# fgvieira/ngsLD

Measured on AMD Instinct MI355X. Metric: SNP-pair EM-LD computations/sec @ n_ind=500, higher is better.
Workload: dtype f64

## Files before the change

include/ngsld.h:

```cpp
#ifndef NGSLD_H
#define NGSLD_H

#include <stddef.h>
#include <stdint.h>

#ifdef __cplusplus
extern "C" {
#endif

typedef struct ngsld_ctx ngsld_ctx;

enum {
  NGSLD_OK = 0,
  NGSLD_ERR_INVALID = -1,
  NGSLD_ERR_DEVICE = -2,
  NGSLD_ERR_NOMEM = -3,
  NGSLD_ERR_NAN = -4,
  NGSLD_ERR_MAF_RANGE = -5,
  NGSLD_ERR_SINK = -6,
  NGSLD_ERR_UNSUPPORTED = -7
};

typedef struct {
  uint64_t max_kb_dist;
  uint64_t max_snp_dist;
  double min_maf;
  int32_t ignore_miss_data;
  int32_t extend_out;
  double rnd_sample;
  uint64_t seed;
  uint64_t first_row;
} ngsld_params;

typedef struct {
  double r2_ExpG;
  double D;
  double Dp;
  double r2;
} ngsld_rec_std;

typedef struct {
  double hap[4];
  uint32_t n_ind_data;
  uint32_t n_iter;
} ngsld_rec_ext;

typedef struct {
  uint32_t s1, s2_begin, count, reserved;
  uint64_t mask;
  uint64_t first_record;
} ngsld_item;

typedef struct {
  uint64_t s1_begin, s1_end;
  uint64_t n_pairs;
  uint64_t n_items;
  const ngsld_item *items;
  const ngsld_rec_std *std;
  const ngsld_rec_ext *ext;
  const char *text;
  uint64_t text_len;
} ngsld_batch;

typedef int (*ngsld_sink_fn)(void *user, const ngsld_batch *batch);

typedef int (*ngsld_read_sites_fn)(void *user, uint64_t site_begin, uint64_t n_sites, double *dst);

const char *ngsld_version(void);

int ngsld_create(int device, ngsld_ctx **ctx);
void ngsld_destroy(ngsld_ctx *ctx);
const char *ngsld_last_error(const ngsld_ctx *ctx);

int ngsld_set_geno_raw(ngsld_ctx *ctx, const double *gl_raw, uint64_t n_sites, uint64_t n_ind, int log_scale,
                       int ignore_miss_data, int on_device);
typedef struct {
  int32_t log_scale;
  int32_t ignore_miss_data;
  int32_t on_device;
  int32_t text_semantics;
  int32_t call_geno;
  int32_t per_individual_only;
  double N_thresh;
  double call_thresh;
} ngsld_geno_opts;
int ngsld_set_geno_raw_opts(ngsld_ctx *ctx, const double *gl_raw, uint64_t n_sites, uint64_t n_ind,
                            const ngsld_geno_opts *opts);
int ngsld_set_geno_lkl(ngsld_ctx *ctx, const double *geno_lkl, const double *maf, uint64_t n_sites, uint64_t n_ind,
                       int on_device);
int ngsld_get_maf(ngsld_ctx *ctx, double *maf_out);
int ngsld_set_pos_dist(ngsld_ctx *ctx, const double *pos_dist);

int ngsld_plan(ngsld_ctx *ctx, const ngsld_params *params, uint64_t *n_pairs);
int ngsld_plan_rows(ngsld_ctx *ctx, const uint64_t **row_off, const uint32_t **row_end);

int ngsld_run(ngsld_ctx *ctx, uint64_t s1_begin, uint64_t s1_end, ngsld_sink_fn sink, void *user);

int ngsld_set_text_output(ngsld_ctx *ctx, const char *const *labels, int enable);

int ngsld_reserve_text_buffers(ngsld_ctx *ctx, uint64_t bytes_per_row);

int ngsld_set_replay_source(ngsld_ctx *ctx, ngsld_read_sites_fn read, void *user);
int ngsld_set_replay_matrix(ngsld_ctx *ctx, const double *values);
int ngsld_set_replay(ngsld_ctx *ctx, int enable);
int ngsld_replay_stats(ngsld_ctx *ctx, uint64_t *pairs, uint64_t *sites);

int ngsld_set_exact_store(ngsld_ctx *ctx, int mode);
typedef struct {
  uint64_t pairs_flagged;
  uint64_t pairs_replayed;
  uint64_t pairs_on_device;
  uint64_t pairs_on_host;
  uint64_t sites_reevaluated;
  int32_t exact_store;
  int32_t text_rows_patched;
  double exact_store_build_s;
  uint64_t sites_degenerate;
} ngsld_replay_stats_t;
int ngsld_replay_info(ngsld_ctx *ctx, ngsld_replay_stats_t *out);

int ngsld_run_device(ngsld_ctx *ctx, uint64_t s1_begin, uint64_t s1_end, void *d_std, void *d_ext, void *hip_stream);
int ngsld_finish_device(ngsld_ctx *ctx);

int ngsld_last_kernel_time(ngsld_ctx *ctx, double *total_ms, uint64_t *n_launches, uint64_t *n_pairs);

const char *ngsld_pair_kernel(const ngsld_ctx *ctx);
int ngsld_describe_dispatch(uint64_t n_ind, int ignore_miss_data, char *buf, size_t buf_len);

int ngsld_set_tuning(ngsld_ctx *ctx, uint32_t pairs_per_item, uint64_t batch_pairs);

int ngsld_selftest(ngsld_ctx *ctx);

int ngsld_selftest_format(ngsld_ctx *ctx, uint64_t n, const ngsld_rec_std *std, const ngsld_rec_ext *ext, const double *dist,
                          const double *maf1, const double *maf2, char *text, uint64_t text_cap, uint64_t *row_len,
                          int32_t *needs_host);
int ngsld_selftest_printed(ngsld_ctx *ctx, uint64_t n, const double *x, int32_t precision, int32_t weight_type,
                           double min_weight, int64_t *micro, int32_t *micro_ok, int64_t *label, int32_t *label_rc);

typedef struct {
  uint64_t row_begin, row_end;
  uint64_t site_end;
} ngsld_slab;

int ngsld_window_ends(const double *pos_dist, uint64_t n_sites, const ngsld_params *params, uint32_t *row_end);

int ngsld_plan_slabs(const double *pos_dist, uint64_t n_sites, const ngsld_params *params, uint64_t max_slab_sites,
                     ngsld_slab *slabs, uint64_t cap, uint64_t *n_slabs);

uint64_t ngsld_slab_sites_for_budget(uint64_t n_ind, uint64_t budget_bytes);
uint64_t ngsld_sites_for_budget(uint64_t n_ind, uint64_t budget_bytes, int matrix_copies);

int ngsld_streamed_replay_info(ngsld_replay_stats_t *out);

int ngsld_set_memory_budget(int device, uint64_t bytes);

int ngsld_device_memory(int device, uint64_t *free_bytes, uint64_t *total_bytes);


int ngsld_run_streamed(int device, uint64_t n_sites, uint64_t n_ind, const double *pos_dist,
                       const ngsld_params *params, const ngsld_geno_opts *opts, uint64_t max_slab_sites,
                       ngsld_read_sites_fn read, void *read_user, double *maf_out, ngsld_sink_fn sink,
                       void *sink_user, uint64_t *n_pairs, uint64_t *n_slabs, char *err, size_t errlen);

int ngsld_run_streamed_text(int device, uint64_t n_sites, uint64_t n_ind, const double *pos_dist,
                            const ngsld_params *params, const ngsld_geno_opts *opts, uint64_t max_slab_sites,
                            ngsld_read_sites_fn read, void *read_user, double *maf_out, ngsld_sink_fn sink,
                            void *sink_user, uint64_t *n_pairs, uint64_t *n_slabs, char *err, size_t errlen,
                            const char *const *labels, int text_output);


int ngsld_plan_parts(const double *pos_dist, uint64_t n_sites, const ngsld_params *params, int n_parts, ngsld_slab *parts);

typedef int (*ngsld_multi_sink_fn)(void *user, int part, const ngsld_batch *batch);

int ngsld_run_multi(const int *devices, int n_devices, uint64_t n_sites, uint64_t n_ind, const double *pos_dist,
                    const ngsld_params *params, const ngsld_geno_opts *opts, const double *gl_raw,
                    ngsld_read_sites_fn read, void *read_user, double *maf_out, ngsld_multi_sink_fn sink, void *sink_user,
                    const char *const *labels, int text_output, uint64_t *pairs_per_part, char *err, size_t errlen);

enum { NGSLD_DIST_NONE = 0, NGSLD_DIST_UPLOAD = 1, NGSLD_DIST_PEER_COPY = 2, NGSLD_DIST_RCCL = 3 };
int ngsld_multi_last_distribution(void);

int ngsld_rccl_selftest(int device, uint64_t bytes, char *err, size_t errlen);

typedef struct {
  uint32_t struct_size;
  int32_t field;
  double max_kb_dist;
  double min_weight;
  int32_t weight_type;
  int32_t keep_heavy;
  int32_t precision;
  int32_t reserved;
  const char *const *subset;
  uint64_t n_subset;
} ngsld_prune_params;

typedef struct {
  uint32_t struct_size;
  uint32_t reserved;
  uint64_t pairs;
  uint64_t nodes, edges;
  uint64_t kept, excluded;
  uint64_t rounds;
  uint64_t host_nodes, host_edges, host_steps;
  double pairs_ms, edges_ms, graph_ms, rounds_ms, host_ms, total_ms;
} ngsld_prune_stats;

int ngsld_prune(ngsld_ctx *ctx, const ngsld_prune_params *params, const char *const *labels, uint8_t *site_state,
                ngsld_prune_stats *stats);

typedef struct {
  uint32_t struct_size;
  uint32_t fields;
  double bin_size;
  double max_kb_dist;
  double min_maf;
} ngsld_decay_params;

typedef struct {
  uint32_t struct_size;
  uint32_t lds;
  uint64_t pairs;
  uint64_t pairs_counted;
  uint64_t bins;
  uint64_t bin_slots;
  uint64_t chunks;
  double pairs_ms, bin_ms, total_ms;
} ngsld_decay_stats;

int ngsld_decay(ngsld_ctx *ctx, const ngsld_decay_params *params, ngsld_decay_stats *stats);
int ngsld_decay_bins(ngsld_ctx *ctx, uint64_t cap, double *dist, uint64_t *count, double *mean, uint64_t *n_bins);

typedef struct {
  uint32_t struct_size;
  uint32_t fields;
  const char *chr;
  uint64_t start, end;
} ngsld_blocks_params;

typedef struct {
  uint32_t struct_size;
  uint32_t reserved;
  uint64_t members, sites;
  uint64_t pairs, pairs_in_region;
  uint64_t cells_na, host_rows, chunks;
  double pairs_ms, scatter_ms, format_ms, total_ms;
} ngsld_blocks_stats;

int ngsld_blocks(ngsld_ctx *ctx, const ngsld_blocks_params *params, const char *const *labels, ngsld_blocks_stats *stats);
int ngsld_blocks_sites(ngsld_ctx *ctx, uint64_t cap, uint64_t *site, uint64_t *n_sites);
int ngsld_blocks_matrix(ngsld_ctx *ctx, int field, double *values, uint8_t *present);
typedef int (*ngsld_text_fn)(void *user, const char *text, uint64_t len);
int ngsld_blocks_text(ngsld_ctx *ctx, int field, ngsld_text_fn sink, void *user, ngsld_blocks_stats *stats);

typedef struct {
  uint32_t struct_size;
  uint32_t fields;
  double max_kb_dist;
  double min_maf;
  double linked_min;
  int32_t abs_value;
  int32_t reserved;
} ngsld_site_ld_params;

typedef struct {
  uint32_t struct_size;
  uint32_t lds;
  uint64_t pairs;
  uint64_t pairs_counted;
  uint64_t sites_with_pairs;
  uint64_t chunks;
  double pairs_ms, site_ms, total_ms;
} ngsld_site_ld_stats;

int ngsld_site_ld(ngsld_ctx *ctx, const ngsld_site_ld_params *params, ngsld_site_ld_stats *stats);
int ngsld_site_ld_get(ngsld_ctx *ctx, int field, uint64_t *n, int64_t *sum_micro, int64_t *max_micro, uint64_t *linked,
                      double *mean);

// ... 127 lines not shown
```

ngsld_amd/capi.py:

```python
from __future__ import annotations

import ctypes as C
import os
import subprocess

import numpy as np

PKG_DIR = os.path.dirname(os.path.abspath(__file__))
REPO_DIR = os.path.dirname(PKG_DIR)
LIB_PATH = os.environ.get("NGSLD_LIB") or os.path.join(PKG_DIR, "libngsld.so")
CLI_PATH = os.path.join(PKG_DIR, "bin", "ngsLD")

OK, ERR_INVALID, ERR_DEVICE, ERR_NOMEM, ERR_NAN, ERR_MAF_RANGE, ERR_SINK, ERR_UNSUPPORTED = 0, -1, -2, -3, -4, -5, -6, -7


class Params(C.Structure):
    _fields_ = [("max_kb_dist", C.c_uint64), ("max_snp_dist", C.c_uint64), ("min_maf", C.c_double),
                ("ignore_miss_data", C.c_int32), ("extend_out", C.c_int32), ("rnd_sample", C.c_double),
                ("seed", C.c_uint64), ("first_row", C.c_uint64)]


class GenoOpts(C.Structure):
    _fields_ = [("log_scale", C.c_int32), ("ignore_miss_data", C.c_int32), ("on_device", C.c_int32),
                ("text_semantics", C.c_int32), ("call_geno", C.c_int32), ("per_individual_only", C.c_int32),
                ("N_thresh", C.c_double), ("call_thresh", C.c_double)]


REC_STD = np.dtype([("r2_ExpG", "<f8"), ("D", "<f8"), ("Dp", "<f8"), ("r2", "<f8")])
REC_EXT = np.dtype([("hap", "<f8", (4,)), ("n_ind_data", "<u4"), ("n_iter", "<u4")])


ITEM = np.dtype([("s1", "<u4"), ("s2_begin", "<u4"), ("count", "<u4"), ("reserved", "<u4"), ("mask", "<u8"),
                 ("first_record", "<u8")])


class Batch(C.Structure):
    _fields_ = [("s1_begin", C.c_uint64), ("s1_end", C.c_uint64), ("n_pairs", C.c_uint64), ("n_items", C.c_uint64),
                ("items", C.c_void_p), ("std", C.c_void_p), ("ext", C.c_void_p), ("text", C.c_void_p),
                ("text_len", C.c_uint64)]


def items_to_pairs(items: np.ndarray) -> tuple[np.ndarray, np.ndarray]:
    if len(items) == 0:
        return np.zeros(0, dtype=np.uint64), np.zeros(0, dtype=np.uint64)
    bits = (items["mask"][:, None] >> np.arange(64, dtype=np.uint64)[None, :]) & np.uint64(1)
    bits &= (np.arange(64)[None, :] < items["count"][:, None]).astype(np.uint64)
    idx, c = np.nonzero(bits)
    return items["s1"][idx].astype(np.uint64), (items["s2_begin"][idx].astype(np.uint64) + c.astype(np.uint64))


def items_from_pairs(s1: np.ndarray, s2: np.ndarray, span: int = 64) -> np.ndarray:
    s1, s2 = np.asarray(s1, dtype=np.int64), np.asarray(s2, dtype=np.int64)
    chunk = (s2 - s1 - 1) // span
    key = s1 * (1 << 32) + chunk
    uniq, first, inv = np.unique(key, return_index=True, return_inverse=True)
    items = np.zeros(len(uniq), dtype=ITEM)
    items["s1"] = s1[first]
    items["s2_begin"] = s1[first] + 1 + chunk[first] * span
    items["first_record"] = first
    np.bitwise_or.at(items["mask"], inv, np.uint64(1) << (s2 - items["s2_begin"][inv]).astype(np.uint64))
    last = np.zeros(len(uniq), dtype=np.int64)
    np.maximum.at(last, inv, s2 - items["s2_begin"][inv].astype(np.int64))
    items["count"] = last + 1
    return items


SINK_FN = C.CFUNCTYPE(C.c_int, C.c_void_p, C.POINTER(Batch))
MULTI_SINK_FN = C.CFUNCTYPE(C.c_int, C.c_void_p, C.c_int, C.POINTER(Batch))
READ_FN = C.CFUNCTYPE(C.c_int, C.c_void_p, C.c_uint64, C.c_uint64, C.c_void_p)
SLAB = np.dtype([("row_begin", "<u8"), ("row_end", "<u8"), ("site_end", "<u8")])

SYMBOLS = [
    "ngsld_version", "ngsld_create", "ngsld_destroy", "ngsld_last_error", "ngsld_set_geno_raw",
    "ngsld_set_geno_raw_opts", "ngsld_set_geno_lkl",
    "ngsld_get_maf", "ngsld_set_pos_dist", "ngsld_plan", "ngsld_plan_rows", "ngsld_run", "ngsld_run_device", "ngsld_set_text_output",
    "ngsld_set_replay_source", "ngsld_set_replay_matrix", "ngsld_set_replay", "ngsld_replay_stats", "ngsld_finish_device",
    "ngsld_set_exact_store", "ngsld_replay_info",
    "ngsld_plan_parts", "ngsld_run_multi", "ngsld_multi_last_distribution", "ngsld_rccl_selftest",
    "ngsld_last_kernel_time", "ngsld_pair_kernel", "ngsld_describe_dispatch", "ngsld_set_tuning", "ngsld_selftest", "ngsld_selftest_format",
    "ngsld_selftest_printed", "ngsld_reserve_text_buffers",
    "ngsld_window_ends", "ngsld_plan_slabs", "ngsld_slab_sites_for_budget", "ngsld_sites_for_budget", "ngsld_streamed_replay_info", "ngsld_set_memory_budget", "ngsld_device_memory", "ngsld_run_streamed", "ngsld_run_streamed_text",
    "ngsld_host_read_geno_bin_range",
    "ngsld_host_set_threads", "ngsld_host_read_pos", "ngsld_host_pos_dist", "ngsld_host_label", "ngsld_host_free_pos", "ngsld_host_pos_slice",
    "ngsld_host_geno_size_ok", "ngsld_host_read_geno_bin", "ngsld_host_read_geno_text", "ngsld_host_format_header", "ngsld_host_format_pair",
    "ngsld_host_format_double", "ngsld_host_write_batch", "ngsld_host_replay_pair", "ngsld_host_missing_call_log",
    "ngsld_host_gz_open", "ngsld_host_gz_close",
    "ngsld_prune", "ngsld_host_prune_graph", "ngsld_host_prune_label",
    "ngsld_decay", "ngsld_decay_bins", "ngsld_host_decay_fit",
    "ngsld_blocks", "ngsld_blocks_sites", "ngsld_blocks_matrix", "ngsld_blocks_text",
    "ngsld_site_ld", "ngsld_site_ld_get",
    "ngsld_clusters", "ngsld_clusters_sites", "ngsld_clusters_table",
    "ngsld_grid", "ngsld_grid_cells", "ngsld_grid_chromosomes", "ngsld_grid_get",
    "ngsld_linked_pairs",
    "ngsld_scan", "ngsld_scan_get",
]


class ReplayStats(C.Structure):
    _fields_ = [("pairs_flagged", C.c_uint64), ("pairs_replayed", C.c_uint64), ("pairs_on_device", C.c_uint64),
                ("pairs_on_host", C.c_uint64), ("sites_reevaluated", C.c_uint64), ("exact_store", C.c_int32),
                ("text_rows_patched", C.c_int32), ("exact_store_build_s", C.c_double), ("sites_degenerate", C.c_uint64)]


class PruneParams(C.Structure):
    _fields_ = [("struct_size", C.c_uint32), ("field", C.c_int32), ("max_kb_dist", C.c_double), ("min_weight", C.c_double),
                ("weight_type", C.c_int32), ("keep_heavy", C.c_int32), ("precision", C.c_int32), ("reserved", C.c_int32),
                ("subset", C.POINTER(C.c_char_p)), ("n_subset", C.c_uint64)]


class PruneStats(C.Structure):
    _fields_ = [("struct_size", C.c_uint32), ("reserved", C.c_uint32), ("pairs", C.c_uint64), ("nodes", C.c_uint64),
                ("edges", C.c_uint64), ("kept", C.c_uint64), ("excluded", C.c_uint64), ("rounds", C.c_uint64),
                ("host_nodes", C.c_uint64), ("host_edges", C.c_uint64), ("host_steps", C.c_uint64),
                ("pairs_ms", C.c_double), ("edges_ms", C.c_double), ("graph_ms", C.c_double), ("rounds_ms", C.c_double),
                ("host_ms", C.c_double), ("total_ms", C.c_double)]


class DecayParams(C.Structure):
    _fields_ = [("struct_size", C.c_uint32), ("fields", C.c_uint32), ("bin_size", C.c_double), ("max_kb_dist", C.c_double),
                ("min_maf", C.c_double)]


class DecayStats(C.Structure):
    _fields_ = [("struct_size", C.c_uint32), ("lds", C.c_uint32), ("pairs", C.c_uint64), ("pairs_counted", C.c_uint64),
                ("bins", C.c_uint64), ("bin_slots", C.c_uint64), ("chunks", C.c_uint64), ("pairs_ms", C.c_double),
                ("bin_ms", C.c_double), ("total_ms", C.c_double)]


class BlocksParams(C.Structure):
    _fields_ = [("struct_size", C.c_uint32), ("fields", C.c_uint32), ("chr", C.c_char_p), ("start", C.c_uint64),
                ("end", C.c_uint64)]


class BlocksStats(C.Structure):
    _fields_ = [("struct_size", C.c_uint32), ("reserved", C.c_uint32), ("members", C.c_uint64), ("sites", C.c_uint64),
                ("pairs", C.c_uint64), ("pairs_in_region", C.c_uint64), ("cells_na", C.c_uint64), ("host_rows", C.c_uint64),
                ("chunks", C.c_uint64), ("pairs_ms", C.c_double), ("scatter_ms", C.c_double), ("format_ms", C.c_double),
                ("total_ms", C.c_double)]


class SiteLdParams(C.Structure):
    _fields_ = [("struct_size", C.c_uint32), ("fields", C.c_uint32), ("max_kb_dist", C.c_double), ("min_maf", C.c_double),
                ("linked_min", C.c_double), ("abs_value", C.c_int32), ("reserved", C.c_int32)]


class SiteLdStats(C.Structure):
    _fields_ = [("struct_size", C.c_uint32), ("lds", C.c_uint32), ("pairs", C.c_uint64), ("pairs_counted", C.c_uint64),
                ("sites_with_pairs", C.c_uint64), ("chunks", C.c_uint64), ("pairs_ms", C.c_double), ("site_ms", C.c_double),
                ("total_ms", C.c_double)]


class ClustersParams(C.Structure):
    _fields_ = [("struct_size", C.c_uint32), ("field", C.c_int32), ("max_kb_dist", C.c_double), ("min_maf", C.c_double),
                ("min_weight", C.c_double), ("abs_value", C.c_int32), ("reserved", C.c_int32)]


class ClustersStats(C.Structure):
    _fields_ = [("struct_size", C.c_uint32), ("reserved", C.c_uint32), ("pairs", C.c_uint64), ("nodes", C.c_uint64),
                ("edges", C.c_uint64), ("clusters", C.c_uint64), ("clusters_multi", C.c_uint64), ("largest", C.c_uint64),
                ("chunks", C.c_uint64), ("union_launches", C.c_uint64), ("pairs_ms", C.c_double), ("union_ms", C.c_double),
                ("finish_ms", C.c_double), ("total_ms", C.c_double)]


class GridParams(C.Structure):
    _fields_ = [("struct_size", C.c_uint32), ("fields", C.c_uint32), ("bin_size", C.c_uint64), ("max_kb_dist", C.c_double),
                ("min_maf", C.c_double), ("linked_min", C.c_double), ("abs_value", C.c_int32), ("reserved", C.c_int32)]


class GridStats(C.Structure):
    _fields_ = [("struct_size", C.c_uint32), ("lds", C.c_uint32), ("pairs", C.c_uint64), ("pairs_counted", C.c_uint64),
                ("cells", C.c_uint64), ("bins", C.c_uint64), ("band", C.c_uint64), ("chunks", C.c_uint64),
                ("pairs_ms", C.c_double), ("grid_ms", C.c_double), ("total_ms", C.c_double)]


class LinkedParams(C.Structure):
    _fields_ = [("struct_size", C.c_uint32), ("field", C.c_int32), ("min_weight", C.c_double), ("max_kb_dist", C.c_double),
                ("min_maf", C.c_double), ("abs_value", C.c_int32), ("want", C.c_int32)]


class ScanParams(C.Structure):
    _fields_ = [("struct_size", C.c_uint32), ("fields", C.c_uint32), ("half_window", C.c_uint64), ("max_kb_dist", C.c_double),
                ("min_maf", C.c_double), ("reserved", C.c_uint64)]


class ScanStats(C.Structure):
    _fields_ = [("struct_size", C.c_uint32), ("reserved", C.c_uint32), ("pairs", C.c_uint64), ("pairs_counted", C.c_uint64),
                ("largest_window", C.c_uint64), ("chunks", C.c_uint64), ("pairs_ms", C.c_double), ("scan_ms", C.c_double),
                ("total_ms", C.c_double)]


class LinkedBatch(C.Structure):
    _fields_ = [("n", C.c_uint64), ("s1", C.c_void_p), ("s2", C.c_void_p), ("std", C.c_void_p), ("ext", C.c_void_p),
                ("text", C.c_void_p), ("text_len", C.c_uint64)]


class LinkedStats(C.Structure):
    _fields_ = [("struct_size", C.c_uint32), ("reserved", C.c_uint32), ("pairs", C.c_uint64), ("rows", C.c_uint64),
                ("text_bytes", C.c_uint64), ("host_rows", C.c_uint64), ("chunks", C.c_uint64), ("pairs_ms", C.c_double),
                ("kernel_ms", C.c_double), ("total_ms", C.c_double), ("count_ms", C.c_double), ("scan_ms", C.c_double),
                ("write_ms", C.c_double)]


LINKED_RECORDS, LINKED_TEXT = 1, 2
LINKED_FN = C.CFUNCTYPE(C.c_int, C.c_void_p, C.POINTER(LinkedBatch))
TEXT_FN = C.CFUNCTYPE(C.c_int, C.c_void_p, C.c_void_p, C.c_uint64)


class DecayFitResult(C.Structure):
    _fields_ = [("rate", C.c_double), ("ld_max", C.c_double), ("ld_min", C.c_double), ("sse", C.c_double),
                ("n_bins", C.c_uint64)]


DECAY_FIELDS = ("r2_ExpG", "D", "Dp", "r2")


class NgsldError(RuntimeError):
    def __init__(self, code: int, msg: str):
        super().__init__(f"ngsld error {code}: {msg}")
        self.code = code
        self.msg = msg


def build(force: bool = False, jobs: int = 8) -> None:
    csrc = os.path.join(PKG_DIR, "csrc")
    if force:
        subprocess.check_call(["make", "-s", "-C", csrc, "clean"])
    subprocess.check_call(["make", "-s", f"-j{jobs}", "-C", csrc, "all"])


_lib = None


def lib() -> C.CDLL:
    global _lib
    if _lib is None:
        if not os.path.exists(LIB_PATH):
            raise FileNotFoundError(f"{LIB_PATH} is missing: run ngsld_amd.capi.build() (or make -C ngsld_amd/csrc); "
                                    "there is no fallback implementation")
        L = C.CDLL(LIB_PATH)
        vp, u64, dbl = C.c_void_p, C.c_uint64, C.c_double
        L.ngsld_version.restype = C.c_char_p
        L.ngsld_create.argtypes = [C.c_int, C.POINTER(vp)]
        L.ngsld_destroy.argtypes = [vp]
        L.ngsld_destroy.restype = None
        L.ngsld_last_error.argtypes = [vp]
        L.ngsld_last_error.restype = C.c_char_p
        L.ngsld_set_geno_raw.argtypes = [vp, vp, u64, u64, C.c_int, C.c_int, C.c_int]
        L.ngsld_set_geno_raw_opts.argtypes = [vp, vp, u64, u64, C.POINTER(GenoOpts)]
        L.ngsld_set_geno_lkl.argtypes = [vp, vp, vp, u64, u64, C.c_int]
        L.ngsld_get_maf.argtypes = [vp, vp]
        L.ngsld_set_pos_dist.argtypes = [vp, vp]
        L.ngsld_plan.argtypes = [vp, C.POINTER(Params), C.POINTER(u64)]
        L.ngsld_plan_rows.argtypes = [vp, C.POINTER(C.POINTER(C.c_uint64)), C.POINTER(C.POINTER(C.c_uint32))]
        L.ngsld_run.argtypes = [vp, u64, u64, SINK_FN, vp]
        L.ngsld_run_device.argtypes = [vp, u64, u64, vp, vp, vp]
        if hasattr(L, "ngsld_set_replay_source"):
            L.ngsld_set_replay_source.argtypes = [vp, READ_FN, vp]
            if hasattr(L, "ngsld_set_replay_matrix"):
                L.ngsld_set_replay_matrix.argtypes = [vp, vp]
            L.ngsld_set_replay.argtypes = [vp, C.c_int]
            L.ngsld_replay_stats.argtypes = [vp, C.POINTER(u64), C.POINTER(u64)]
        if hasattr(L, "ngsld_replay_info"):
            L.ngsld_set_exact_store.argtypes = [vp, C.c_int]
            L.ngsld_replay_info.argtypes = [vp, C.POINTER(ReplayStats)]
            L.ngsld_finish_device.argtypes = [vp]
        if hasattr(L, "ngsld_set_text_output"):
            L.ngsld_set_text_output.argtypes = [vp, C.POINTER(C.c_char_p), C.c_int]
        L.ngsld_last_kernel_time.argtypes = [vp, C.POINTER(dbl), C.POINTER(u64), C.POINTER(u64)]
        L.ngsld_set_tuning.argtypes = [vp, C.c_uint32, u64]
        if hasattr(L, "ngsld_pair_kernel"):
            L.ngsld_pair_kernel.argtypes = [vp]
            L.ngsld_pair_kernel.restype = C.c_char_p
        L.ngsld_selftest.argtypes = [vp]
        if hasattr(L, "ngsld_selftest_format"):
            L.ngsld_selftest_format.argtypes = [vp, u64, vp, vp, vp, vp, vp, C.c_char_p, u64, vp, C.POINTER(C.c_int32)]
            L.ngsld_selftest_printed.argtypes = [vp, u64, vp, C.c_int32, C.c_int32, dbl, vp, vp, vp, vp]
        L.ngsld_window_ends.argtypes = [vp, u64, C.POINTER(Params), vp]
        L.ngsld_plan_slabs.argtypes = [vp, u64, C.POINTER(Params), u64, vp, u64, C.POINTER(u64)]
        L.ngsld_slab_sites_for_budget.argtypes = [u64, u64]
        L.ngsld_slab_sites_for_budget.restype = u64
        if hasattr(L, "ngsld_sites_for_budget"):
            L.ngsld_sites_for_budget.argtypes = [u64, u64, C.c_int]
            L.ngsld_sites_for_budget.restype = u64
        L.ngsld_device_memory.argtypes = [C.c_int, C.POINTER(u64), C.POINTER(u64)]
        L.ngsld_run_streamed.argtypes = [C.c_int, u64, u64, vp, C.POINTER(Params), C.POINTER(GenoOpts), u64, READ_FN, vp,
                                         vp, SINK_FN, vp, C.POINTER(u64), C.POINTER(u64), C.c_char_p, C.c_size_t]
        if hasattr(L, "ngsld_run_multi"):
            L.ngsld_plan_parts.argtypes = [vp, u64, C.POINTER(Params), C.c_int, vp]
            L.ngsld_run_multi.argtypes = [C.POINTER(C.c_int), C.c_int, u64, u64, vp, C.POINTER(Params), C.POINTER(GenoOpts),
                                          vp, READ_FN, vp, vp, MULTI_SINK_FN, vp, C.POINTER(C.c_char_p), C.c_int,
                                          C.POINTER(u64), C.c_char_p, C.c_size_t]
        if hasattr(L, "ngsld_multi_last_distribution"):
            L.ngsld_multi_last_distribution.argtypes = []
        if hasattr(L, "ngsld_rccl_selftest"):
            L.ngsld_rccl_selftest.argtypes = [C.c_int, u64, C.c_char_p, C.c_size_t]
        L.ngsld_host_read_geno_bin_range.argtypes = [C.c_char_p, u64, u64, u64, vp, C.c_char_p, C.c_size_t]
        L.ngsld_host_set_threads.argtypes = [C.c_int]
        L.ngsld_host_set_threads.restype = None
        L.ngsld_host_read_pos.argtypes = [C.c_char_p, C.c_int, u64, C.POINTER(vp), C.c_char_p, C.c_size_t]
        L.ngsld_host_pos_dist.argtypes = [vp]
        L.ngsld_host_pos_dist.restype = C.POINTER(dbl)
        L.ngsld_host_label.argtypes = [vp, u64]
        L.ngsld_host_label.restype = C.c_char_p
        L.ngsld_host_free_pos.argtypes = [vp]
        L.ngsld_host_free_pos.restype = None
        L.ngsld_host_pos_slice.argtypes = [vp, u64, u64]
        L.ngsld_host_pos_slice.restype = vp
        L.ngsld_host_geno_size_ok.argtypes = [u64, u64, u64]
        L.ngsld_host_read_geno_bin.argtypes = [C.c_char_p, u64, u64, vp, C.c_char_p, C.c_size_t]
        L.ngsld_host_read_geno_text.argtypes = [C.c_char_p, C.c_int, C.c_int, u64, u64, vp, C.POINTER(C.c_int),
                                                C.c_char_p, C.c_size_t]
        L.ngsld_host_format_header.argtypes = [C.c_char_p, C.c_size_t, C.c_int]
        L.ngsld_host_format_header.restype = C.c_size_t
        L.ngsld_host_format_pair.argtypes = [C.c_char_p, C.c_size_t, C.c_char_p, C.c_char_p, dbl, vp, vp, dbl, dbl]
        L.ngsld_host_format_pair.restype = C.c_size_t
        L.ngsld_host_format_double.argtypes = [C.c_char_p, C.c_size_t, dbl, C.c_int]
        L.ngsld_host_format_double.restype = C.c_size_t
        L.ngsld_host_write_batch.argtypes = [C.POINTER(Batch), vp, vp, vp, C.c_int, C.c_int]
        L.ngsld_host_replay_pair.argtypes = [vp, vp, u64, C.POINTER(GenoOpts), vp, vp, vp]
        if hasattr(L, "ngsld_host_gz_open"):
            L.ngsld_host_gz_open.argtypes = [C.c_char_p, C.c_int, C.POINTER(vp), C.POINTER(C.c_int)]
            L.ngsld_host_gz_close.argtypes = [vp]
        if hasattr(L, "ngsld_prune"):
            L.ngsld_prune.argtypes = [vp, C.POINTER(PruneParams), C.POINTER(C.c_char_p), vp, C.POINTER(PruneStats)]
            L.ngsld_host_prune_graph.argtypes = [u64, vp, u64, vp, vp, vp, C.c_int, vp, C.POINTER(u64)]
            L.ngsld_host_prune_label.argtypes = [dbl, C.c_int, C.c_char, C.POINTER(C.c_int64)]
        if hasattr(L, "ngsld_decay"):
            L.ngsld_decay.argtypes = [vp, C.POINTER(DecayParams), C.POINTER(DecayStats)]
            L.ngsld_decay_bins.argtypes = [vp, u64, vp, vp, vp, C.POINTER(u64)]
            L.ngsld_host_decay_fit.argtypes = [u64, vp, vp, C.c_int, dbl, dbl, C.POINTER(DecayFitResult)]
        if hasattr(L, "ngsld_blocks"):
            L.ngsld_blocks.argtypes = [vp, C.POINTER(BlocksParams), C.POINTER(C.c_char_p), C.POINTER(BlocksStats)]
            L.ngsld_blocks_sites.argtypes = [vp, u64, vp, C.POINTER(u64)]
            L.ngsld_blocks_matrix.argtypes = [vp, C.c_int, vp, vp]
            L.ngsld_blocks_text.argtypes = [vp, C.c_int, TEXT_FN, vp, C.POINTER(BlocksStats)]
        if hasattr(L, "ngsld_site_ld"):
            L.ngsld_site_ld.argtypes = [vp, C.POINTER(SiteLdParams), C.POINTER(SiteLdStats)]
            L.ngsld_site_ld_get.argtypes = [vp, C.c_int, vp, vp, vp, vp, vp]
        if hasattr(L, "ngsld_clusters"):
            L.ngsld_clusters.argtypes = [vp, C.POINTER(ClustersParams), C.POINTER(ClustersStats)]
            L.ngsld_clusters_sites.argtypes = [vp, vp]
            L.ngsld_clusters_table.argtypes = [vp, u64, u64, vp, vp, vp, vp, vp, vp, vp, vp, vp, C.POINTER(u64)]
        if hasattr(L, "ngsld_grid"):
            L.ngsld_grid.argtypes = [vp, C.POINTER(GridParams), C.POINTER(C.c_char_p), C.POINTER(GridStats)]
            L.ngsld_grid_cells.argtypes = [vp, u64, vp, vp, vp, vp, C.POINTER(u64)]
            L.ngsld_grid_chromosomes.argtypes = [vp, u64, C.POINTER(C.c_char_p), C.POINTER(u64)]
            L.ngsld_grid_get.argtypes = [vp, C.c_int, u64, vp, vp, vp, vp]
        if hasattr(L, "ngsld_linked_pairs"):
            L.ngsld_linked_pairs.argtypes = [vp, C.POINTER(LinkedParams), C.POINTER(C.c_char_p), LINKED_FN, vp, C.POINTER(LinkedStats)]
        if hasattr(L, "ngsld_scan"):
            L.ngsld_scan.argtypes = [vp, C.POINTER(ScanParams), C.POINTER(ScanStats)]
            L.ngsld_scan_get.argtypes = [vp, C.c_int, vp, vp, vp, vp, vp, vp, vp, vp, vp, vp]
        _lib = L
    return _lib


def prune_label(x: float, prec: int = 4, weight_type: str = "a") -> int | None:
    out = C.c_int64()
    rc = lib().ngsld_host_prune_label(float(x), prec, weight_type.encode(), C.byref(out))
    if rc == ERR_INVALID:
        return None
    if rc != OK:
        raise NgsldError(rc, "label out of range")
    return out.value


def decay_fit(dist, values, field: str = "r2", n_ind: float = 0, recomb_rate: float = 1.0) -> dict:
    d = np.ascontiguousarray(dist, dtype=np.float64)
    v = np.ascontiguousarray(values, dtype=np.float64)
    if d.shape != v.shape or d.ndim != 1:
        raise ValueError("dist and values must be 1-D arrays of one length")
    if field not in DECAY_FIELDS:
        raise ValueError(f"field must be one of {DECAY_FIELDS}")
    out = DecayFitResult()
    rc = lib().ngsld_host_decay_fit(len(d), d.ctypes.data, v.ctypes.data, 4 + DECAY_FIELDS.index(field), float(n_ind),
                                    float(recomb_rate), C.byref(out))
    if rc != OK:
        raise NgsldError(rc, f"ngsld_host_decay_fit refused the {field} fit")
    return {k: getattr(out, k) for k, _ in DecayFitResult._fields_}


def prune_graph(n_nodes: int, a, b, label, keep_heavy: bool = False, rank=None) -> tuple[np.ndarray, int]:
    a = np.ascontiguousarray(a, dtype=np.uint32)
    b = np.ascontiguousarray(b, dtype=np.uint32)
    lab = np.ascontiguousarray(label, dtype=np.int64)
    rk = None if rank is None else np.ascontiguousarray(rank, dtype=np.uint64)
    excl = np.zeros(max(n_nodes, 1), dtype=np.uint8)
    steps = C.c_uint64()
    rc = lib().ngsld_host_prune_graph(n_nodes, None if rk is None else rk.ctypes.data, len(a), a.ctypes.data, b.ctypes.data,
                                      lab.ctypes.data, int(keep_heavy), excl.ctypes.data, C.byref(steps))
    if rc != OK:
        raise NgsldError(rc, "ngsld_host_prune_graph failed")
    return excl[:n_nodes].astype(bool), steps.value


def read_pos(path: str, header: bool, n_sites: int) -> tuple[np.ndarray, list[str]]:
    L = lib()
    h = C.c_void_p()
    err = C.create_string_buffer(512)
    rc = L.ngsld_host_read_pos(path.encode(), int(header), n_sites, C.byref(h), err, len(err))
    if rc != OK:
        raise NgsldError(rc, err.value.decode())
    try:
        pd = np.ctypeslib.as_array(L.ngsld_host_pos_dist(h), shape=(n_sites,)).copy()
        labels = [L.ngsld_host_label(h, s).decode() for s in range(n_sites)]
    finally:
        L.ngsld_host_free_pos(h)
    return pd, labels


def read_geno_bin(path: str, n_ind: int, n_sites: int) -> np.ndarray:
    L = lib()
    out = np.empty((n_sites, n_ind, 3), dtype=np.float64)
    err = C.create_string_buffer(512)
    rc = L.ngsld_host_read_geno_bin(path.encode(), n_ind, n_sites, out.ctypes.data, err, len(err))
    if rc != OK:
        raise NgsldError(rc, err.value.decode())
    return out


def read_geno_bin_range(path: str, n_ind: int, site_begin: int, n_sites: int) -> np.ndarray:
    L = lib()
    out = np.empty((n_sites, n_ind, 3), dtype=np.float64)
    err = C.create_string_buffer(512)
    rc = L.ngsld_host_read_geno_bin_range(path.encode(), n_ind, site_begin, n_sites, out.ctypes.data, err, len(err))
# ... 431 lines not shown
        a, b = C.c_uint64(), C.c_uint64()
        self._check(self._L.ngsld_replay_stats(self._h, C.byref(a), C.byref(b)))
        return a.value, b.value

    def set_exact_store(self, mode: int) -> None:
        self._check(self._L.ngsld_set_exact_store(self._h, int(mode)))

    def replay_info(self) -> dict:
        st = ReplayStats()
        self._check(self._L.ngsld_replay_info(self._h, C.byref(st)))
        return {k: getattr(st, k) for k, _ in ReplayStats._fields_}

    def finish_device(self) -> None:
        self._check(self._L.ngsld_finish_device(self._h))

    def maf(self) -> np.ndarray:
        out = np.empty(self.n_sites, dtype=np.float64)
        self._check(self._L.ngsld_get_maf(self._h, out.ctypes.data))
        return out

    def set_pos_dist(self, pos_dist: np.ndarray | None) -> None:
        if pos_dist is None:
            self._check(self._L.ngsld_set_pos_dist(self._h, None))
        else:
            pd = np.ascontiguousarray(pos_dist, dtype=np.float64)
            assert pd.shape[0] == self.n_sites
            self._check(self._L.ngsld_set_pos_dist(self._h, pd.ctypes.data))

    def set_tuning(self, pairs_per_item: int = 0, batch_pairs: int = 0) -> None:
        self._check(self._L.ngsld_set_tuning(self._h, pairs_per_item, batch_pairs))

    def plan(self, max_kb_dist: int = 0, max_snp_dist: int = 0, min_maf: float = 0.0, ignore_miss_data: bool = False,
             extend_out: bool = True, rnd_sample: float = 1.0, seed: int = 0, first_row: int = 0) -> int:
        p = Params(max_kb_dist, max_snp_dist, min_maf, int(ignore_miss_data), int(extend_out), rnd_sample, seed,
                   first_row)
        n = C.c_uint64()
        self._check(self._L.ngsld_plan(self._h, C.byref(p), C.byref(n)))
        self.extend_out = extend_out
        return n.value

    def plan_rows(self) -> tuple[np.ndarray, np.ndarray]:
        ro, re = C.POINTER(C.c_uint64)(), C.POINTER(C.c_uint32)()
        self._check(self._L.ngsld_plan_rows(self._h, C.byref(ro), C.byref(re)))
        return (np.ctypeslib.as_array(ro, shape=(self.n_sites + 1,)).copy(),
                np.ctypeslib.as_array(re, shape=(self.n_sites,)).copy())

    def run(self, s1_begin: int = 0, s1_end: int | None = None):
        s1_end = self.n_sites if s1_end is None else s1_end
        s1s, s2s, stds, exts = [], [], [], []

        def sink(_user, bp):
            b = bp.contents
            n = b.n_pairs
            if n:
                stds.append(np.frombuffer(C.string_at(b.std, n * REC_STD.itemsize), dtype=REC_STD).copy())
                if b.ext:
                    exts.append(np.frombuffer(C.string_at(b.ext, n * REC_EXT.itemsize), dtype=REC_EXT).copy())
            items = np.frombuffer(C.string_at(b.items, b.n_items * ITEM.itemsize), dtype=ITEM) if b.n_items else \
                np.zeros(0, dtype=ITEM)
            a, bb = items_to_pairs(items)
            assert len(a) == n
            if len(items):
                assert np.array_equal(items["first_record"], np.concatenate([[0], np.cumsum(
                    [bin(int(m)).count("1") for m in items["mask"]])[:-1]]).astype(np.uint64))
            s1s.append(a)
            s2s.append(bb)
            return 0

        cb = SINK_FN(sink)
        self._check(self._L.ngsld_run(self._h, s1_begin, s1_end, cb, None))
        cat = lambda xs, dt: np.concatenate(xs) if xs else np.zeros(0, dtype=dt)
        return (cat(s1s, np.uint64), cat(s2s, np.uint64), cat(stds, REC_STD),
                cat(exts, REC_EXT) if self.extend_out else None)

    def items(self, s1_begin: int = 0, s1_end: int | None = None) -> np.ndarray:
        s1_end = self.n_sites if s1_end is None else s1_end
        got = []

        def sink(_user, bp):
            b = bp.contents
            if b.n_items:
                got.append(np.frombuffer(C.string_at(b.items, b.n_items * ITEM.itemsize), dtype=ITEM).copy())
            return 0

        self.set_text_output(None, False)
        self._check(self._L.ngsld_run(self._h, s1_begin, s1_end, SINK_FN(sink), None))
        return np.concatenate(got) if got else np.zeros(0, dtype=ITEM)

    def run_to_fd(self, s1_begin: int, s1_end: int, fd: int, pos_handle, pos_dist: np.ndarray | None, maf: np.ndarray,
                  n_threads: int) -> int:
        maf = np.ascontiguousarray(maf, dtype=np.float64)
        pd_ptr = None if pos_dist is None else np.ascontiguousarray(pos_dist, dtype=np.float64).ctypes.data
        total, rc_box = [0], [0]

        libc = C.CDLL(None, use_errno=True)
        libc.write.argtypes = [C.c_int, C.c_void_p, C.c_size_t]
        libc.write.restype = C.c_ssize_t

        def sink(_user, bp):
            b = bp.contents
            total[0] += b.n_pairs
            if b.text:
                off = 0
                while off < b.text_len:
                    w = libc.write(fd, b.text + off, min(b.text_len - off, 1 << 30))
                    if w <= 0:
                        return 1
                    off += w
                return 0
            rc_box[0] = self._L.ngsld_host_write_batch(bp, pos_handle, pd_ptr, maf.ctypes.data, n_threads, fd)
            return 0 if rc_box[0] == OK else 1

        self._check(self._L.ngsld_run(self._h, s1_begin, s1_end, SINK_FN(sink), None))
        return total[0]

    def set_text_output(self, labels: list[str] | None, enable: bool = True) -> None:
        arr = None
        if labels is not None:
            arr = (C.c_char_p * len(labels))(*[l.encode() for l in labels])
        self._check(self._L.ngsld_set_text_output(self._h, arr, int(enable)))

    def run_text(self, s1_begin: int = 0, s1_end: int | None = None) -> tuple[bytes, int]:
        s1_end = self.n_sites if s1_end is None else s1_end
        parts, fallbacks = [], [0]

        def sink(_user, bp):
            b = bp.contents
            if b.text:
                parts.append(C.string_at(b.text, b.text_len))
            else:
                fallbacks[0] += 1
            return 0

        self._check(self._L.ngsld_run(self._h, s1_begin, s1_end, SINK_FN(sink), None))
        return b"".join(parts), fallbacks[0]

    def run_discard(self, s1_begin: int = 0, s1_end: int | None = None) -> int:
        s1_end = self.n_sites if s1_end is None else s1_end
        total = [0]

        def sink(_user, bp):
            total[0] += bp.contents.n_pairs
            return 0

        self._check(self._L.ngsld_run(self._h, s1_begin, s1_end, SINK_FN(sink), None))
        return total[0]

    def run_device(self, s1_begin: int, s1_end: int, d_std: int, d_ext: int | None, stream: int | None = None) -> None:
        self._check(self._L.ngsld_run_device(self._h, s1_begin, s1_end, d_std, d_ext, stream))

    def pair_kernel(self) -> str:
        return self._L.ngsld_pair_kernel(self._h).decode()

    def last_kernel_time(self) -> tuple[float, int, int]:
        ms, nl, npairs = C.c_double(), C.c_uint64(), C.c_uint64()
        self._check(self._L.ngsld_last_kernel_time(self._h, C.byref(ms), C.byref(nl), C.byref(npairs)))
        return ms.value, nl.value, npairs.value

    def prune(self, labels: list[str] | None, field: int = 7, max_kb_dist: float = float("inf"), min_weight: float = 0.0,
              weight_type: str = "a", keep_heavy: bool = False, subset: list[str] | None = None,
              precision: int = 4) -> tuple[np.ndarray, dict]:
        arr = None if labels is None else (C.c_char_p * len(labels))(*[l.encode() for l in labels])
        sub = None if subset is None else (C.c_char_p * max(len(subset), 1))(*[l.encode() for l in subset])
        p = PruneParams(C.sizeof(PruneParams), field, float(max_kb_dist), float(min_weight), ord(weight_type), int(keep_heavy),
                        precision, 0, sub, 0 if subset is None else len(subset))
        st = PruneStats()
        st.struct_size = C.sizeof(PruneStats)
        state = np.zeros(max(self.n_sites, 1), dtype=np.uint8)
        self._check(self._L.ngsld_prune(self._h, C.byref(p), arr, state.ctypes.data, C.byref(st)))
        return state[:self.n_sites], {k: getattr(st, k) for k, _ in PruneStats._fields_ if k not in ("struct_size", "reserved")}

    def decay(self, ld=("r2",), bin_size: float = 250, max_kb_dist: float = float("inf"),
              min_maf: float = 0.0) -> tuple[dict, dict]:
        ld = (ld,) if isinstance(ld, str) else tuple(ld)
        bad = [f for f in ld if f not in DECAY_FIELDS]
        if bad or not ld:
            raise ValueError(f"ld must name some of {DECAY_FIELDS}: {bad}")
        mask = sum(1 << DECAY_FIELDS.index(f) for f in set(ld))
        names = [f for k, f in enumerate(DECAY_FIELDS) if (mask >> k) & 1]
        p = DecayParams(C.sizeof(DecayParams), mask, float(bin_size), float(max_kb_dist), float(min_maf))
        st = DecayStats()
        st.struct_size = C.sizeof(DecayStats)
        self._check(self._L.ngsld_decay(self._h, C.byref(p), C.byref(st)))
        nb = st.bins
        dist = np.zeros(max(nb, 1))
        cnt = np.zeros(max(nb, 1), dtype=np.uint64)
        mean = np.zeros((max(nb, 1), len(names)))
        got = C.c_uint64()
        self._check(self._L.ngsld_decay_bins(self._h, nb, dist.ctypes.data, cnt.ctypes.data, mean.ctypes.data, C.byref(got)))
        assert got.value == nb
        bins = {"dist": dist[:nb], "n": cnt[:nb]}
        for k, f in enumerate(names):
            bins[f] = mean[:nb, k].copy()
        return bins, {k: getattr(st, k) for k, _ in DecayStats._fields_ if k != "struct_size"}

    def site_ld(self, ld=("r2",), max_kb_dist: float = float("inf"), min_maf: float = 0.0, linked_min: float = 0.5,
                abs_value: bool = True) -> tuple[dict, dict]:
        ld = (ld,) if isinstance(ld, str) else tuple(ld)
        bad = [f for f in ld if f not in DECAY_FIELDS]
        if bad or not ld:
            raise ValueError(f"ld must name some of {DECAY_FIELDS}: {bad}")
        mask = sum(1 << DECAY_FIELDS.index(f) for f in set(ld))
        p = SiteLdParams(C.sizeof(SiteLdParams), mask, float(max_kb_dist), float(min_maf), float(linked_min), int(bool(abs_value)), 0)
        st = SiteLdStats()
        st.struct_size = C.sizeof(SiteLdStats)
        self._check(self._L.ngsld_site_ld(self._h, C.byref(p), C.byref(st)))
        m = max(self.n_sites, 1)
        sites = {"n": np.zeros(m, dtype=np.uint64)}
        for k, f in enumerate(DECAY_FIELDS):
            if not (mask >> k) & 1:
                continue
            sites[f"sum_{f}"], sites[f"max_{f}"] = np.zeros(m, dtype=np.int64), np.zeros(m, dtype=np.int64)
            sites[f"linked_{f}"], sites[f"mean_{f}"] = np.zeros(m, dtype=np.uint64), np.zeros(m)
            self._check(self._L.ngsld_site_ld_get(self._h, 4 + k, sites["n"].ctypes.data, sites[f"sum_{f}"].ctypes.data,
                                                  sites[f"max_{f}"].ctypes.data, sites[f"linked_{f}"].ctypes.data,
                                                  sites[f"mean_{f}"].ctypes.data))
        sites = {k: v[:self.n_sites] for k, v in sites.items()}
        return sites, {k: getattr(st, k) for k, _ in SiteLdStats._fields_ if k != "struct_size"}

    def scan(self, half_window: int, ld=("r2",), max_kb_dist: float = float("inf"), min_maf: float = 0.0) -> tuple[dict, dict]:
        ld = (ld,) if isinstance(ld, str) else tuple(ld)
        bad = [f for f in ld if f not in DECAY_FIELDS]
        if bad or not ld:
            raise ValueError(f"ld must name some of {DECAY_FIELDS}: {bad}")
        if not 0 <= int(half_window) < 2 ** 64:
            raise ValueError("half_window must be a non-negative integer")
        mask = sum(1 << DECAY_FIELDS.index(f) for f in set(ld))
        p = ScanParams(C.sizeof(ScanParams), mask, int(half_window), float(max_kb_dist), float(min_maf), 0)
        st = ScanStats()
        st.struct_size = C.sizeof(ScanStats)
        self._check(self._L.ngsld_scan(self._h, C.byref(p), C.byref(st)))
        m = max(self.n_sites, 1)
        win = {"win_first": np.zeros(m, dtype=np.uint32), "win_last": np.zeros(m, dtype=np.uint32)}
        for cl in ("ll", "rr", "lr"):
            win[f"n_{cl}"] = np.zeros(m, dtype=np.uint64)
        for k, f in enumerate(DECAY_FIELDS):
            if not (mask >> k) & 1:
                continue
            for cl in ("ll", "rr", "lr"):
                win[f"sum_{cl}_{f}"] = np.zeros(m, dtype=np.int64)
            win[f"zns_{f}"], win[f"omega_{f}"] = np.zeros(m), np.zeros(m)
            self._check(self._L.ngsld_scan_get(self._h, 4 + k, win["win_first"].ctypes.data, win["win_last"].ctypes.data,
                                               win["n_ll"].ctypes.data, win["n_rr"].ctypes.data, win["n_lr"].ctypes.data,
                                               win[f"sum_ll_{f}"].ctypes.data, win[f"sum_rr_{f}"].ctypes.data,
                                               win[f"sum_lr_{f}"].ctypes.data, win[f"zns_{f}"].ctypes.data,
                                               win[f"omega_{f}"].ctypes.data))
        win = {k: v[:self.n_sites] for k, v in win.items()}
        return win, {k: getattr(st, k) for k, _ in ScanStats._fields_ if k not in ("struct_size", "reserved")}

    def clusters(self, field: int = 7, min_weight: float = 0.5, max_kb_dist: float = float("inf"), min_maf: float = 0.0,
                 abs_value: bool = True, min_size: int = 2) -> tuple[np.ndarray, dict, dict]:
        p = ClustersParams(C.sizeof(ClustersParams), int(field), float(max_kb_dist), float(min_maf), float(min_weight),
                           int(bool(abs_value)), 0)
        st = ClustersStats()
        st.struct_size = C.sizeof(ClustersStats)
        self._check(self._L.ngsld_clusters(self._h, C.byref(p), C.byref(st)))
        ids = np.zeros(max(self.n_sites, 1), dtype=np.uint32)
        self._check(self._L.ngsld_clusters_sites(self._h, ids.ctypes.data))
        rows = C.c_uint64(0)
        self._check(self._L.ngsld_clusters_table(self._h, int(min_size), 0, None, None, None, None, None, None, None, None, None,
                                                 C.byref(rows)))
        m = max(int(rows.value), 1)
        kinds = dict(id=np.uint32, size=np.uint32, first=np.uint32, last=np.uint32, span=np.uint64, edges=np.uint64, sum=np.int64,
                     mean=np.float64, density=np.float64)
        table = {k: np.zeros(m, dtype=t) for k, t in kinds.items()}
        self._check(self._L.ngsld_clusters_table(self._h, int(min_size), m, *(table[k].ctypes.data for k in kinds), C.byref(rows)))
        table = {k: v[:int(rows.value)] for k, v in table.items()}
        return ids[:self.n_sites], table, {k: getattr(st, k) for k, _ in ClustersStats._fields_ if k not in ("struct_size", "reserved")}

    def grid(self, labels: list[str] | None, bin_size: int, ld=("r2",), max_kb_dist: float = float("inf"), min_maf: float = 0.0,
             linked_min: float = 0.5, abs_value: bool = True) -> tuple[dict, dict]:
        ld = (ld,) if isinstance(ld, str) else tuple(ld)
        bad = [f for f in ld if f not in DECAY_FIELDS]
        if bad or not ld:
            raise ValueError(f"ld must name some of {DECAY_FIELDS}: {bad}")
        mask = sum(1 << DECAY_FIELDS.index(f) for f in set(ld))
        arr = None if labels is None else (C.c_char_p * max(len(labels), 1))(*[l.encode() for l in labels])
        p = GridParams(C.sizeof(GridParams), mask, int(bin_size), float(max_kb_dist), float(min_maf), float(linked_min),
                       int(bool(abs_value)), 0)
        st = GridStats()
        st.struct_size = C.sizeof(GridStats)
        self._check(self._L.ngsld_grid(self._h, C.byref(p), arr, C.byref(st)))
        nc = int(st.cells)
        m = max(nc, 1)
        n_chr = C.c_uint64(0)
        self._check(self._L.ngsld_grid_chromosomes(self._h, 0, None, C.byref(n_chr)))
        names = (C.c_char_p * max(int(n_chr.value), 1))()
        self._check(self._L.ngsld_grid_chromosomes(self._h, int(n_chr.value), names, None))
        names = np.array([names[k].decode() for k in range(int(n_chr.value))] or [""])
        idx, b1, b2 = np.zeros(m, dtype=np.uint32), np.zeros(m, dtype=np.uint64), np.zeros(m, dtype=np.uint64)
        cells = {"n": np.zeros(m, dtype=np.uint64)}
        got = C.c_uint64(0)
        self._check(self._L.ngsld_grid_cells(self._h, m, idx.ctypes.data, b1.ctypes.data, b2.ctypes.data, cells["n"].ctypes.data,
                                             C.byref(got)))
        assert got.value == nc
        cells = {"chr": names[idx], "bin1": b1 * np.uint64(int(bin_size)), "bin2": b2 * np.uint64(int(bin_size)), **cells}
        for k, f in enumerate(DECAY_FIELDS):
            if not (mask >> k) & 1:
                continue
            cells[f"sum_{f}"], cells[f"max_{f}"] = np.zeros(m, dtype=np.int64), np.zeros(m, dtype=np.int64)
            cells[f"linked_{f}"], cells[f"mean_{f}"] = np.zeros(m, dtype=np.uint64), np.zeros(m)
            self._check(self._L.ngsld_grid_get(self._h, 4 + k, m, cells[f"sum_{f}"].ctypes.data, cells[f"max_{f}"].ctypes.data,
                                               cells[f"linked_{f}"].ctypes.data, cells[f"mean_{f}"].ctypes.data))
        cells = {k: v[:nc] for k, v in cells.items()}
        return cells, {k: getattr(st, k) for k, _ in GridStats._fields_ if k != "struct_size"}

# ... 82 lines not shown
```

ngsld_amd/csrc/engine.h:

```cpp
#pragma once

#include "knobs.h"

#include <hip/hip_runtime.h>
#include <sched.h>
#include <dlfcn.h>
#include <sys/mman.h>

#include <algorithm>
#include <atomic>
#include <chrono>
#include <cmath>
#include <condition_variable>
#include <functional>
#include <cstdio>
#include <cstdlib>
#include <cstring>
#include <limits>
#include <mutex>
#include <new>
#include <string>
#include <thread>
#include <unordered_map>
#include <vector>
// ... 60 lines not shown
    if (count == 0) return hipSuccess;
    hipError_t e = hipMalloc((void **)&p, count * sizeof(T));
    if (e == hipSuccess) n = count;
    return e;
  }
  void release() {
    if (p) (void)hipFree(p);
    p = nullptr;
    n = 0;
  }
};

template <typename T>
struct PinBuf {
  T *p = nullptr;
  size_t n = 0;
  void *map_base = nullptr;
  size_t map_len = 0;
  PinBuf() = default;
  PinBuf(const PinBuf &) = delete;
  PinBuf &operator=(const PinBuf &) = delete;
  ~PinBuf() { release(); }
  hipError_t resize(size_t count) {
    if (count <= n && p != nullptr) return hipSuccess;
    release();
    if (count == 0) return hipSuccess;
    const size_t huge = (size_t)2 << 20, want = count * sizeof(T);
    static const bool use_register = [] {
      const char *e = std::getenv("NGSLD_PIN_REGISTER");
      return e != nullptr && std::strcmp(e, "1") == 0;
    }();
    if (use_register && want >= huge) {
      const size_t bytes = (want + huge - 1) / huge * huge, len = bytes + huge;
      void *m = mmap(nullptr, len, PROT_READ | PROT_WRITE, MAP_PRIVATE | MAP_ANONYMOUS, -1, 0);
      if (m != MAP_FAILED) {
        void *q = reinterpret_cast<void *>((reinterpret_cast<uintptr_t>(m) + huge - 1) / huge * huge);
        (void)madvise(q, bytes, MADV_HUGEPAGE);
        if (madvise(q, bytes, MADV_DONTFORK) == 0 && hipHostRegister(q, bytes, hipHostRegisterMapped) == hipSuccess) {
          p = static_cast<T *>(q);
          n = count;
          map_base = m;
          map_len = len;
          return hipSuccess;
        }
        (void)hipGetLastError();
        (void)munmap(m, len);
      }
    }
    hipError_t e = hipHostMalloc((void **)&p, want, hipHostMallocDefault);
    if (e == hipSuccess) n = count;
    return e;
  }
  void release() {
    if (p && map_base) {
      (void)hipHostUnregister(p);
      (void)munmap(map_base, map_len);
    } else if (p) {
      (void)hipHostFree(p);
    }
    p = nullptr;
    n = 0;
    map_base = nullptr;
    map_len = 0;
  }
};
class ReplayPool {
 public:
  ~ReplayPool() {
    {
      std::lock_guard<std::mutex> lk(mu_);
      stop_ = true;
    }
    cv_.notify_all();
    for (auto &t : threads_) t.join();
  }
  template <typename F>
  void run(int T, F &&fn) {
    if (T <= 1) {
      fn(0);
      return;
    }
    while ((int)threads_.size() < T - 1) {
      const int id = (int)threads_.size() + 1;
      threads_.emplace_back([this, id] { loop(id); });
    }
    {
      std::lock_guard<std::mutex> lk(mu_);
      job_ = [&fn](int t) { fn(t); };
      n_ = T;
      left_ = T - 1;
      ++epoch_;
    }
    cv_.notify_all();
    fn(0);
    std::unique_lock<std::mutex> lk(mu_);
    done_.wait(lk, [this] { return left_ == 0; });
    job_ = nullptr;
  }

 private:
  void loop(int id) {
    uint64_t seen = 0;
    for (;;) {
      std::function<void(int)> job;
      {
        std::unique_lock<std::mutex> lk(mu_);
        cv_.wait(lk, [&] { return stop_ || epoch_ != seen; });
        if (stop_) return;
        seen = epoch_;
        if (id >= n_) continue;
        job = job_;
      }
      job(id);
      std::lock_guard<std::mutex> lk(mu_);
      if (--left_ == 0) done_.notify_all();
    }
  }
  std::vector<std::thread> threads_;
  std::mutex mu_;
  std::condition_variable cv_, done_;
  std::function<void(int)> job_;
  int n_ = 0, left_ = 0;
  uint64_t epoch_ = 0;
  bool stop_ = false;
};

}
}

using namespace ngsld;
using namespace ngsld::eng;

#include "exact_store.h"

struct FlagRow {
  uint64_t rec, off;
  uint32_t len, s1, s2, pad;
};
constexpr uint32_t kFlagRowsCap = 1024;

struct ngsld_ctx {
  int device = 0;
  hipStream_t stream = nullptr, stream2 = nullptr, copy_stream = nullptr;
  hipStream_t text_stream = nullptr;
  hipEvent_t ev_scan_done[3] = {nullptr, nullptr, nullptr};
  std::string err;

  uint64_t n_sites = 0, n_ind = 0;
  uint32_t np = 0;
  PairConfig cfg{};
  bool have_geno = false;
  DevBuf<double> d_planes, d_maf, d_mean, d_rsx, d_sc4;
  DevBuf<double> d_dose_sum;
  bool first_step_on = true;
  static constexpr int kMomentStreams = 4;
  DevBuf<double> d_moments[kMomentStreams];
  hipStream_t moments_stream[kMomentStreams] = {nullptr, nullptr, nullptr, nullptr};
  hipEvent_t moments_done[kMomentStreams] = {nullptr, nullptr, nullptr, nullptr};
  int moments_used = 0;
  DevBuf<int> d_status;
  std::vector<double> h_maf, h_pos_dist;
  DevBuf<uint64_t> d_hard_masks;
  DevBuf<double> d_hard_u;
  DevBuf<int> d_all_hard, d_odd_missing;
  int h_odd_missing = 0;
  bool missing_canonical = false;
  int h_all_hard = 0, h_prep_status = 0;
  uint32_t mask_words = 0;
  DevBuf<uint8_t> d_skip;
  DevBuf<uint32_t> d_skip_count;
  uint32_t h_skip_count = 0;
  bool skip_on = true;
  bool skip_kernels = false;

  bool planned = false;
  ngsld_params params{};
  std::vector<uint64_t> h_row_off, h_item_off;
  std::vector<uint32_t> h_row_end;
  std::vector<uint8_t> h_keep;
  std::vector<Item> h_items;
  std::vector<uint64_t> h_run_off;
  uint64_t run_len = 0;
  std::vector<uint64_t> run_ends;
  int n_cus = 256;
  DevBuf<Run> d_runs;
  DevBuf<uint64_t> d_row_off, d_item_off, d_row_seed, d_row_count;
  DevBuf<uint32_t> d_row_end;
  DevBuf<uint8_t> d_keep;
  DevBuf<Item> d_items;
  uint64_t n_items = 0;

  int kernel_choice = kChooseAuto;
  uint32_t pairs_per_item = 16;
  uint64_t batch_pairs = 1ull << 23;
  bool batch_pairs_set = false;

  static constexpr int kSlots = 3;
  DevBuf<ngsld_rec_std> d_std[kSlots];
  DevBuf<ngsld_rec_ext> d_ext[kSlots];
  PinBuf<ngsld_rec_std> h_std[kSlots];
  PinBuf<ngsld_rec_ext> h_ext[kSlots];
  hipEvent_t ev_kernel_done[kSlots] = {nullptr, nullptr, nullptr}, ev_copy_done[kSlots] = {nullptr, nullptr, nullptr};
  bool run_direct = true, run_taper = true;
  int run_streams = 1;
  bool timed_overlap = false;

  bool text_mode = false, have_labels = false;
  uint64_t max_label = 6;
  DevBuf<char> d_labels, d_text[kSlots], d_scan_tmp, d_scan_tmp_b;
  DevBuf<uint64_t> d_label_off, d_lens[kSlots], d_offs[kSlots], d_text_meta[kSlots];
  DevBuf<double> d_cum;
  DevBuf<uint32_t> d_infc;
  PinBuf<char> h_text[kSlots];
  PinBuf<uint64_t> h_text_meta[kSlots];
  std::thread reserve_thread;

  bool replay_on = true;
  ngsld_read_sites_fn replay_read = nullptr;
  void *replay_user = nullptr;
  const double *replay_matrix = nullptr;
  std::mutex replay_mu;
  hipStream_t replay_stream = nullptr;
  std::mutex replay_stream_mu;
  ngsld_geno_opts gopts{};
  bool normalised = false;
  DevBuf<uint32_t> d_flags[kSlots], d_flags_dev;
  PinBuf<uint32_t> h_flags[kSlots], h_flags_dev;
  PinBuf<uint32_t> h_flag_bits;
  PinBuf<FlagRow> h_flag_rows[kSlots];
  uint32_t flag_cap[kSlots] = {0, 0, 0}, flag_cap_dev = 0;
  bool replay_device = true;
  uint64_t replayed_on_device = 0;
  uint64_t text_rows_patched = 0;
  ExactStore store;
  int exact_mode = 1;
  struct LaneScratch {
    DevBuf<ReplayEntry> list;
    DevBuf<uint64_t> keys_a, keys_b;
    DevBuf<uint32_t> vals_a, vals_b;
    DevBuf<char> temp;
    size_t temp_bytes = 0;
    void release() { list.release(); keys_a.release(); keys_b.release(); vals_a.release(); vals_b.release(); temp.release(); }
    bool reserve(uint64_t list_cap, uint64_t n_sites) {
      temp_bytes = replay_sort_temp_bytes(list_cap, (uint32_t)n_sites);
      if (list.resize(list_cap) == hipSuccess && keys_a.resize(list_cap) == hipSuccess && keys_b.resize(list_cap) == hipSuccess &&
          vals_a.resize(list_cap) == hipSuccess && vals_b.resize(list_cap) == hipSuccess && temp.resize(temp_bytes ? temp_bytes : 1) == hipSuccess)
        return true;
      (void)hipGetLastError();
      release();
      return false;
    }
  } lane_scratch[kSlots], lane_scratch_dev;
  uint64_t host_replayed_total = 0;
  uint64_t flagged_pairs = 0;
  bool slot_dev_applied[kSlots] = {false, false, false};
  PinBuf<double> h_site_stage;
  DevBuf<uint64_t> d_patch_idx;
  DevBuf<ngsld_rec_std> d_patch_std;
  DevBuf<ngsld_rec_ext> d_patch_ext;
  DevBuf<char> d_scan_tmp2;
  DevBuf<uint32_t> d_patch_s1, d_patch_s2;
  uint64_t replayed_pairs = 0, replayed_sites = 0;
  int replay_threads = 0;
  ReplayPool replay_pool;
  struct {
    bool pending = false;
    uint64_t s1_begin = 0, s1_end = 0;
    ngsld_rec_std *d_std = nullptr;
    ngsld_rec_ext *d_ext = nullptr;
    hipStream_t st = nullptr;
    bool dev_applied = false;
  } dev_run;
  bool dev_run_flag_text = false;
  DevBuf<ngsld_rec_std> d_group_std[2];
  DevBuf<ngsld_rec_ext> d_group_ext[2];
  DevBuf<uint64_t> d_group_lens, d_group_offs, d_group_meta, d_group_first;
  DevBuf<int> d_group_needs;
  DevBuf<char> d_group_text;
  PinBuf<uint64_t> h_group_bounds;
  PinBuf<int> h_group_needs;

  std::vector<std::pair<hipEvent_t, hipEvent_t>> ev_pool;
  size_t ev_used = 0;
  hipStream_t timed_stream = nullptr;
  uint64_t timed_pairs = 0;

  uint32_t decay_fields = 0;
  std::vector<double> decay_dist, decay_mean;
  std::vector<uint64_t> decay_count;

  uint32_t site_fields = 0;
  std::vector<uint64_t> site_n, site_linked;
  std::vector<int64_t> site_sum, site_max;
  std::vector<double> site_mean;
  void clear_sites() {
    site_fields = 0;
    site_n.clear();
    site_linked.clear();
    site_sum.clear();
    site_max.clear();
    site_mean.clear();
  }

  struct Clusters {
    bool valid = false;
    std::vector<uint32_t> id, size, first, last;
    std::vector<uint64_t> span, edges;
    std::vector<int64_t> sum;
    std::vector<double> mean, density;
  } clusters;
  void clear_clusters() { clusters = Clusters(); }

  struct Grid {
    uint32_t fields = 0;
    std::vector<std::string> chr_name;
    std::vector<uint32_t> chr;
    std::vector<uint64_t> b1, b2, n, linked;
    std::vector<int64_t> sum, max;
    std::vector<double> mean;
  } grid;
  void clear_grid() { grid = Grid(); }

  struct Scan {
    uint32_t fields = 0;
    std::vector<uint32_t> first, last;
    std::vector<uint64_t> n;
    std::vector<int64_t> sum;
    std::vector<double> zns, omega;
  } scan;
  void clear_scan() { scan = Scan(); }

  uint32_t blocks_fields = 0;
  uint64_t blocks_members = 0;
  DevBuf<double> d_blocks_val;
  DevBuf<uint8_t> d_blocks_present;
  DevBuf<uint32_t> d_blocks_col;
  std::vector<uint64_t> blocks_site;
  std::vector<std::string> blocks_label;
  DevBuf<char> d_blocks_label;
  DevBuf<uint64_t> d_blocks_label_off;
  void clear_blocks() {
    clear_sites();
    clear_clusters();
    clear_grid();
    clear_scan();
    blocks_fields = 0;
    blocks_members = 0;
    d_blocks_val.release();
    d_blocks_present.release();
    d_blocks_col.release();
    d_blocks_label.release();
    d_blocks_label_off.release();
    blocks_site.clear();
    blocks_label.clear();
  }
};

namespace ngsld {
namespace eng {


inline int fail(ngsld_ctx *c, int code, const std::string &msg) {
  if (c) c->err = msg;
  return code;
}

inline int hip_fail(ngsld_ctx *c, hipError_t e, const char *what) {
  return fail(c, e == hipErrorOutOfMemory ? NGSLD_ERR_NOMEM : NGSLD_ERR_DEVICE,
              std::string(what) + ": " + hipGetErrorString(e));
}

#define HIP_TRY(c, call)                                \
  do {                                                  \
    hipError_t e_ = (call);                             \
    if (e_ != hipSuccess) return hip_fail(c, e_, #call); \
  } while (0)

#define RC_TRY(call)                     \
  do {                                   \
    const int rc_ = (call);              \
    if (rc_ != NGSLD_OK) return rc_;     \
  } while (0)

inline int caught(ngsld_ctx *c, bool nomem) {
  if (c) {
    (void)hipSetDevice(c->device);
    (void)hipDeviceSynchronize();
    c->planned = false;
  }
  return nomem ? fail(c, NGSLD_ERR_NOMEM, "out of host memory") : fail(c, NGSLD_ERR_INVALID, "unexpected C++ exception");
}
#define NGSLD_CATCH(ctx)                                        \
  catch (const std::bad_alloc &) { return caught(ctx, true); }  \
  catch (...) { return caught(ctx, false); }

inline int check_status(ngsld_ctx *c) {
  int status = 0;
  HIP_TRY(c, hipMemcpy(&status, c->d_status.p, sizeof(int), hipMemcpyDeviceToHost));
  if (status == NGSLD_ERR_MAF_RANGE) return fail(c, NGSLD_ERR_MAF_RANGE, "invalid allele frequencies");
  return NGSLD_OK;
}

constexpr uint64_t kTextBatchPairs = 1ull << 19;

inline uint32_t flag_cap_for(uint64_t n) { return (uint32_t)std::min<uint64_t>(1ull << 20, std::max<uint64_t>(4096, n / 256)); }
inline size_t flag_head_bytes(uint32_t cap) { return (size_t)flag_head_words(cap) * sizeof(uint32_t); }
inline size_t flag_bitmap_words(uint64_t n) { return (size_t)((n + 31) / 32); }
inline size_t flag_words(uint64_t n, uint32_t cap) { return (size_t)flag_head_words(cap) + 2 * flag_bitmap_words(n); }

void plan_rows(const std::vector<double> &pos_dist, const std::vector<double> &maf, const ngsld_params &p, uint64_t n,
               std::vector<uint32_t> &row_end);
int build_runs(ngsld_ctx *c, uint64_t run_len, const std::vector<uint64_t> &launch_ends);

inline uint64_t rows_within(const std::vector<uint64_t> &off, uint64_t r0, uint64_t end, uint64_t target) {
  uint64_t r1 = r0 + 1;
  while (r1 < end && off[r1 + 1] - off[r0] <= target) ++r1;
  return r1;
}
hipError_t timed_launch(ngsld_ctx *c, const PairArgs &a, hipStream_t stream);
PairArgs make_args(ngsld_ctx *c, uint64_t r0, uint64_t r1, ngsld_rec_std *d_std, ngsld_rec_ext *d_ext,
                   uint32_t *d_flags = nullptr, uint32_t flag_cap = 0, uint64_t flag_n = 0);

bool dist_prefix(const ngsld_ctx *c, std::vector<double> &cum, std::vector<uint32_t> &infc);

inline unsigned blocks_for(uint64_t threads, unsigned per_block = 256) { return (unsigned)((threads + per_block - 1) / per_block); }
inline double ms_since(std::chrono::steady_clock::time_point t0) {
  return std::chrono::duration<double, std::milli>(std::chrono::steady_clock::now() - t0).count();
}
template <class P, class S>
int check_struct_sizes(ngsld_ctx *c, const P *p, const char *p_name, const S *stats, const char *s_name) {
  if (p == nullptr || p->struct_size != sizeof(P))
    return fail(c, NGSLD_ERR_INVALID, std::string(p_name) + ": struct_size must be sizeof(" + p_name + ")");
  if (stats != nullptr && stats->struct_size < sizeof(uint32_t)) return fail(c, NGSLD_ERR_INVALID, std::string(s_name) + ": struct_size not set");
  return NGSLD_OK;
}
template <class S>
void copy_stats(S *out, const S &s) {
  if (out == nullptr) return;
  const uint32_t want = out->struct_size;
  std::memcpy(out, &s, std::min<size_t>(want, sizeof(S)));
  out->struct_size = want;
}
inline int field_list(uint32_t mask, int field[4]) {
  int ns = 0;
  for (int f = 0; f < 4; ++f)
    if ((mask >> f) & 1u) field[ns++] = f;
  return ns;
}

int send_flag_rows(ngsld_ctx *c, const uint32_t *d_flags, uint32_t cap, bool dev_applied, const uint64_t *d_offs, const uint64_t *d_lens,
                   uint64_t n_records, uint64_t base, FlagRow *h_rows, hipStream_t st);
int replay_pairs_on_host(ngsld_ctx *c, const uint32_t *s1, const uint32_t *s2, size_t n, ngsld_rec_std *out_std, ngsld_rec_ext *out_ext);
unsigned usable_threads();
hipStream_t replay_stream_of(ngsld_ctx *c);
int ensure_host_items(ngsld_ctx *c);
int fetch_replay_site(ngsld_ctx *c, uint64_t s, std::vector<double> &tmp, ReplaySite *out);
int flagged_records(ngsld_ctx *c, const uint32_t *h_head, const uint32_t *d_flags, uint32_t cap, uint64_t n,
                    std::vector<uint64_t> &recs, bool dev_applied = false);
bool room_for(uint64_t need_bytes, uint64_t device_margin, uint64_t budget_margin);
bool lkl_device_eligible(const ngsld_ctx *c);
bool lkl_device_ready(const ngsld_ctx *c);
int reserve_device_run(ngsld_ctx *c, uint64_t n_records);
inline uint64_t exact_sites_needed(const ngsld_ctx *c, uint64_t r0, uint64_t r1) {
  uint64_t need = r1;
  for (uint64_t r = r0; r < r1 && r < c->h_row_end.size(); ++r) need = std::max<uint64_t>(need, c->h_row_end[r]);
  return std::min<uint64_t>(need, c->n_sites);
}
struct ReplayLaunch {
  uint32_t *d_flags;
  uint32_t cap;
  uint64_t out_base, n;
  ngsld_rec_std *d_std;
  ngsld_rec_ext *d_ext;
  hipStream_t st;
  bool flag_text;
  int slot;
};
int try_device_replay_lkl(ngsld_ctx *c, const ReplayLaunch &l, bool *applied, uint64_t need_sites);
int device_replay_lkl(ngsld_ctx *c, const ReplayLaunch &l);
int device_replay(ngsld_ctx *c, const ReplayLaunch &l);
int replay_flagged(ngsld_ctx *c, const std::vector<uint64_t> &recs, uint64_t base, ngsld_rec_std *h_std,
                   ngsld_rec_ext *h_ext, ngsld_rec_std *d_std, ngsld_rec_ext *d_ext, hipStream_t st,
                   std::vector<uint32_t> *sites1 = nullptr, std::vector<uint32_t> *sites2 = nullptr);
int reset_flags(ngsld_ctx *c, DevBuf<uint32_t> &buf, uint64_t n, uint32_t cap, hipStream_t stream);
int send_flag_head(ngsld_ctx *c, const uint32_t *d_flags, uint32_t *h_head, uint32_t cap, hipStream_t st, bool with_list = true);
int finish_device_run(ngsld_ctx *c);

}
}
```

ngsld_amd/csrc/engine.hip:

```cpp
#include "engine.h"

#include <atomic>

namespace ngsld {
namespace eng {

thread_local std::string g_create_error;

int set_geno_common(ngsld_ctx *c, const double *gl, const double *maf, uint64_t n_sites, uint64_t n_ind,
                    const ngsld_geno_opts &o, bool normalised) {
  if (c == nullptr) return NGSLD_ERR_INVALID;
  const int log_scale = o.log_scale, ignore_miss = o.ignore_miss_data, on_device = o.on_device;
  Range range_("ngsld:set_geno (upload + per-site prep)");
  if (o.call_geno && o.N_thresh > o.call_thresh)
    return fail(c, NGSLD_ERR_INVALID, "missing data threshold must be smaller than calling genotype threshold!");
  if (gl == nullptr || n_sites == 0 || n_ind == 0) return fail(c, NGSLD_ERR_INVALID, "empty genotype matrix");
  if (normalised && maf == nullptr) return fail(c, NGSLD_ERR_INVALID, "maf missing");
  if (n_sites >= 0xffffffffull) return fail(c, NGSLD_ERR_UNSUPPORTED, "n_sites must be below 2^32 - 1");
  PairConfig cfg;
  if (!pair_config(n_ind, &cfg, c->kernel_choice, ignore_miss != 0))
    return fail(c, NGSLD_ERR_UNSUPPORTED, "n_ind is outside the supported range");
  HIP_TRY(c, hipSetDevice(c->device));
  (void)hipGetLastError();
  {
    const int rcp = finish_device_run(c);
    if (rcp != NGSLD_OK) return rcp;
  }
  c->store.reset();
  c->have_geno = false;
  c->planned = false;
  c->clear_blocks();
  c->text_mode = false;
  c->replay_read = nullptr;
  c->replay_user = nullptr;
  c->replay_matrix = nullptr;
  c->host_replayed_total = 0;
  for (int k = 0; k < 2; ++k) {
    c->d_group_std[k].release();
    c->d_group_ext[k].release();
  }
  c->d_group_lens.release();
  c->d_group_offs.release();
  c->d_group_text.release();
  c->gopts = o;
  c->normalised = normalised;
  c->n_sites = n_sites;
  c->n_ind = n_ind;
  c->cfg = cfg;
  c->np = cfg.np;
  const bool trace = std::getenv("NGSLD_TRACE") != nullptr;
  const auto t_0 = std::chrono::steady_clock::now();
  auto ms_since = [&]() { return std::chrono::duration<double, std::milli>(std::chrono::steady_clock::now() - t_0).count(); };
  const size_t plane_elems = (size_t)n_sites * 3 * c->np;
  HIP_TRY(c, c->d_planes.resize(plane_elems));
  HIP_TRY(c, c->d_maf.resize(n_sites));
  HIP_TRY(c, c->d_mean.resize(n_sites));
  HIP_TRY(c, c->d_rsx.resize(n_sites));
  HIP_TRY(c, c->d_sc4.resize(4 * n_sites));
  HIP_TRY(c, c->d_status.resize(1));
  HIP_TRY(c, hipMemsetAsync(c->d_status.p, 0, sizeof(int), c->stream));

  PrepArgs a{};
  a.planes = c->d_planes.p;
  a.site_stride = 3ull * c->np;
  a.np = c->np;
  a.n_ind = (uint32_t)n_ind;
  a.log_scale = log_scale;
  a.ignore_miss = ignore_miss;
  a.normalised_input = normalised ? 1 : 0;
  a.text_semantics = o.text_semantics;
  a.call_geno = o.call_geno;
  {
    const char *pe = test_knob("PREP_EXACT");
    a.exact_chain = (pe != nullptr && std::strcmp(pe, "0") != 0) ? 1 : 0;
  }
  a.N_thresh = o.N_thresh;
  a.call_thresh = o.call_thresh;
  a.maf = c->d_maf.p;
  a.mean_e = c->d_mean.p;
  a.rsx = c->d_rsx.p;
  a.status = c->d_status.p;
  c->missing_canonical = false;
  const bool look_for_odd_missing = o.text_semantics && log_scale && !o.call_geno && !normalised;
  if (look_for_odd_missing) {
    HIP_TRY(c, c->d_odd_missing.resize(1));
    HIP_TRY(c, hipMemsetAsync(c->d_odd_missing.p, 0, sizeof(int), c->stream));
    a.odd_missing = c->d_odd_missing.p;
    a.missing_canon = replay_missing_raw_text();
  }
  if (on_device) {
    a.raw = gl;
    a.maf_in = maf;
    a.site0 = 0;
    a.n_sites = n_sites;
    HIP_TRY(c, launch_prep(a, c->stream));
  } else {
    const uint64_t site_bytes = n_ind * 3 * sizeof(double);
    uint64_t stage_bytes = 64ull << 20;
    if (const char *e = test_knob("STAGE_BYTES")) stage_bytes = std::strtoull(e, nullptr, 10);
    uint64_t chunk = stage_bytes / site_bytes;
    if (chunk < 1) chunk = 1;
    if (chunk > n_sites) chunk = n_sites;
    DevBuf<double> stage[2], maf_stage[2];
    hipEvent_t prepped[2] = {nullptr, nullptr};
    for (int k = 0; k < 2; ++k) {
      HIP_TRY(c, stage[k].resize(chunk * n_ind * 3));
      if (normalised) HIP_TRY(c, maf_stage[k].resize(chunk));
      HIP_TRY(c, hipEventCreateWithFlags(&prepped[k], hipEventDisableTiming));
    }
    int rc = NGSLD_OK;
    uint64_t k = 0;
    if (trace) std::fprintf(stderr, "[trace] set_geno: device buffers + staging allocated at %.2f ms\n", ms_since());
    for (uint64_t s0 = 0; s0 < n_sites && rc == NGSLD_OK; s0 += chunk, ++k) {
      const int b = (int)(k & 1);
      const uint64_t m = std::min(chunk, n_sites - s0);
      hipError_t e = hipSuccess;
      if (k >= 2) e = hipEventSynchronize(prepped[b]);
      if (e == hipSuccess)
        e = hipMemcpyAsync(stage[b].p, gl + s0 * n_ind * 3, m * site_bytes, hipMemcpyHostToDevice, c->copy_stream);
      if (e == hipSuccess && normalised)
        e = hipMemcpyAsync(maf_stage[b].p, maf + s0, m * sizeof(double), hipMemcpyHostToDevice, c->copy_stream);
      if (e == hipSuccess) e = hipStreamSynchronize(c->copy_stream);
      if (trace) std::fprintf(stderr, "[trace] set_geno: chunk %llu (%llu sites) on the device at %.2f ms\n", (unsigned long long)k, (unsigned long long)m, ms_since());
      a.raw = stage[b].p;
      a.maf_in = normalised ? maf_stage[b].p : nullptr;
      a.site0 = s0;
      a.n_sites = m;
      if (e == hipSuccess) e = launch_prep(a, c->stream);
      if (e == hipSuccess) e = hipEventRecord(prepped[b], c->stream);
      if (e != hipSuccess) rc = hip_fail(c, e, "chunked genotype upload");
    }
    hipError_t e = hipStreamSynchronize(c->stream);
    if (trace) std::fprintf(stderr, "[trace] set_geno: last prep kernel done at %.2f ms\n", ms_since());
    for (int q = 0; q < 2; ++q) {
      stage[q].release();
      maf_stage[q].release();
      if (prepped[q]) (void)hipEventDestroy(prepped[q]);
    }
    if (trace) std::fprintf(stderr, "[trace] set_geno: staging buffers freed at %.2f ms\n", ms_since());
    if (rc != NGSLD_OK) return rc;
    if (e != hipSuccess) return hip_fail(c, e, "chunked genotype upload");
  }
  c->h_skip_count = 0;
  const bool look_for_skip = c->skip_on && c->replay_on && c->replay_device && c->exact_mode != 0;
  c->skip_kernels = cfg.kernel == kRun || (cfg.kernel == kMulti && cfg.form == 0 && cfg.waves == 2);
  if (look_for_skip) {
    HIP_TRY(c, c->d_skip.resize(n_sites));
    HIP_TRY(c, c->d_skip_count.resize(1));
    HIP_TRY(c, hipMemsetAsync(c->d_skip_count.p, 0, sizeof(uint32_t), c->stream));
    HIP_TRY(c, launch_site_skip(c->d_planes.p, 3ull * c->np, c->np, (uint32_t)n_ind, ignore_miss, c->d_maf.p, n_sites, c->d_skip.p,
                                c->d_skip_count.p, c->stream));
    HIP_TRY(c, hipMemcpyAsync(&c->h_skip_count, c->d_skip_count.p, sizeof(uint32_t), hipMemcpyDeviceToHost, c->stream));
  } else {
    c->d_skip.release();
  }
  HIP_TRY(c, launch_pack_scalars(c->d_maf.p, c->d_mean.p, c->d_rsx.p, c->d_skip.p, c->d_sc4.p, n_sites, c->stream));
  if (cfg.kernel == kRun && !ignore_miss && cfg.slots >= 2 && cfg.slots <= 8) {
    c->first_step_on = !test_knob_is("FIRST_STEP", "0");
    HIP_TRY(c, c->d_dose_sum.resize(n_sites));
    HIP_TRY(c, launch_site_dose(c->d_planes.p, 3ull * c->np, c->np, (uint32_t)n_ind, c->d_maf.p, c->d_skip.p, n_sites, c->d_dose_sum.p,
                                c->stream));
  } else {
    c->d_dose_sum.release();
  }
  int &all_hard = c->h_all_hard;
  all_hard = 0;
  const char *hk = test_knob("HARD_KERNEL");
  const bool try_hard = n_ind <= kHardMaxInd && !o.per_individual_only && !(hk != nullptr && std::strcmp(hk, "0") == 0);
  if (try_hard) {
    c->mask_words = (uint32_t)((n_ind + 63) / 64);
    HIP_TRY(c, c->d_hard_masks.resize((size_t)n_sites * 4 * c->mask_words));
    HIP_TRY(c, c->d_hard_u.resize(n_sites));
    HIP_TRY(c, c->d_all_hard.resize(1));
    all_hard = 1;
    HIP_TRY(c, hipMemcpyAsync(c->d_all_hard.p, &all_hard, sizeof(int), hipMemcpyHostToDevice, c->stream));
    HIP_TRY(c, launch_classify_hard(c->d_planes.p, 3ull * c->np, c->np, (uint32_t)n_ind, n_sites, c->d_hard_masks.p,
                                    c->d_hard_u.p, c->d_all_hard.p, c->stream));
    HIP_TRY(c, hipMemcpyAsync(&all_hard, c->d_all_hard.p, sizeof(int), hipMemcpyDeviceToHost, c->stream));
    if (trace) std::fprintf(stderr, "[trace] set_geno: called-genotype check enqueued at %.2f ms\n", ms_since());
  }
  c->h_maf.resize(n_sites);
  int &status = c->h_prep_status;
  status = 0;
  HIP_TRY(c, hipMemcpyAsync(c->h_maf.data(), c->d_maf.p, n_sites * sizeof(double), hipMemcpyDeviceToHost, c->stream));
  HIP_TRY(c, hipMemcpyAsync(&status, c->d_status.p, sizeof(int), hipMemcpyDeviceToHost, c->stream));
  c->h_odd_missing = 1;
  if (look_for_odd_missing)
    HIP_TRY(c, hipMemcpyAsync(&c->h_odd_missing, c->d_odd_missing.p, sizeof(int), hipMemcpyDeviceToHost, c->stream));
  HIP_TRY(c, hipStreamSynchronize(c->stream));
  c->missing_canonical = look_for_odd_missing && c->h_odd_missing == 0;
  if (trace) std::fprintf(stderr, "[trace] set_geno: scalars packed, called-genotype check, maf on the host at %.2f ms\n", ms_since());
  if (status == NGSLD_ERR_NAN) return fail(c, NGSLD_ERR_NAN, "NaN found! Is the file format correct?");
  if (try_hard && all_hard) {
    c->cfg.kernel = kHard;
    c->cfg.group = 16;
    c->cfg.slots = 1;
    c->cfg.waves = 1;
    c->d_dose_sum.release();
  } else {
    c->d_hard_masks.release();
    c->d_hard_u.release();
  }
  c->have_geno = true;
  return NGSLD_OK;
}
}
}

extern "C" {

const char *ngsld_version(void) { return "ngsld-amd 0.13.0 (gfx950; reference ngsLD 1.2.1)"; }

int ngsld_create(int device, ngsld_ctx **out) {
  if (out == nullptr) return NGSLD_ERR_INVALID;
  *out = nullptr;
  int n_dev = 0;
  hipError_t e = hipGetDeviceCount(&n_dev);
  if (e != hipSuccess || n_dev == 0) {
    g_create_error = std::string("no HIP device available (") + hipGetErrorString(e) +
                     "); this library has no CPU fallback";
    return NGSLD_ERR_DEVICE;
  }
  if (device < 0 || device >= n_dev) {
    g_create_error = "device index out of range";
    return NGSLD_ERR_INVALID;
  }
  hipDeviceProp_t prop;
  e = hipGetDeviceProperties(&prop, device);
  if (e != hipSuccess) {
    g_create_error = std::string("hipGetDeviceProperties: ") + hipGetErrorString(e);
    return NGSLD_ERR_DEVICE;
  }
  if (std::strncmp(prop.gcnArchName, "gfx950", 6) != 0) {
    g_create_error = std::string("device is ") + prop.gcnArchName + ", this build targets gfx950 (MI355X) only";
    return NGSLD_ERR_DEVICE;
  }
  ngsld_ctx *c = new (std::nothrow) ngsld_ctx();
  if (c == nullptr) return NGSLD_ERR_NOMEM;
  c->device = device;
  if (prop.multiProcessorCount > 0) c->n_cus = prop.multiProcessorCount;
  if (const char *k = std::getenv("NGSLD_PAIR_KERNEL")) {
    c->kernel_choice = std::strcmp(k, "multi") == 0 ? kChooseMulti
                       : (std::strcmp(k, "ab") == 0 ? kChooseAB
                          : (std::strcmp(k, "stream") == 0 ? kChoosePlainStream : (std::strcmp(k, "abm") == 0 ? kChooseABMulti
                                                               : (std::strcmp(k, "bres") == 0 ? kChooseResidentStream : kChooseAuto))));
  }
  if (const char *k = test_knob("BATCH_PAIRS")) {
    const uint64_t v = std::strtoull(k, nullptr, 10);
    if (v > 0) {
      c->batch_pairs = v;
      c->batch_pairs_set = true;
    }
  }
  if (const char *k = std::getenv("NGSLD_REPLAY")) c->replay_on = std::strcmp(k, "0") != 0;
  if (const char *k = std::getenv("NGSLD_REPLAY_THREADS")) c->replay_threads = std::atoi(k);
  if (const char *k = std::getenv("NGSLD_REPLAY_DEVICE")) c->replay_device = std::strcmp(k, "0") != 0;
  if (const char *k = std::getenv("NGSLD_REPLAY_SKIP")) c->skip_on = std::strcmp(k, "0") != 0;
  if (const char *k = std::getenv("NGSLD_EXACT_STORE")) c->exact_mode = std::max(0, std::min(2, std::atoi(k)));
  if (const char *k = test_knob("RUN_DIRECT")) c->run_direct = std::strcmp(k, "0") != 0;
  if (const char *k = test_knob("RUN_TAPER")) c->run_taper = std::strcmp(k, "0") != 0;
  if (const char *k = test_knob("RUN_STREAMS")) c->run_streams = std::atoi(k) >= 2 ? 2 : 1;
  if ((e = hipSetDevice(device)) != hipSuccess || (e = hipStreamCreate(&c->stream)) != hipSuccess ||
      (e = hipStreamCreate(&c->stream2)) != hipSuccess || (e = hipStreamCreate(&c->copy_stream)) != hipSuccess) {
    g_create_error = std::string("stream setup: ") + hipGetErrorString(e);
    delete c;
    return NGSLD_ERR_DEVICE;
  }
  for (int k = 0; k < ngsld_ctx::kSlots; ++k) {
    (void)hipEventCreateWithFlags(&c->ev_kernel_done[k], hipEventDisableTiming);
    (void)hipEventCreateWithFlags(&c->ev_copy_done[k], hipEventDisableTiming);
  }
  *out = c;
  return NGSLD_OK;
}

void ngsld_destroy(ngsld_ctx *c) {
  if (c == nullptr) return;
  if (c->reserve_thread.joinable()) c->reserve_thread.join();
  c->store.destroy();
  (void)hipSetDevice(c->device);
  (void)hipDeviceSynchronize();
  c->d_planes.release(); c->d_maf.release(); c->d_mean.release(); c->d_rsx.release(); c->d_sc4.release(); c->d_dose_sum.release(); c->d_runs.release(); c->d_skip.release(); c->d_skip_count.release();
  for (auto &b : c->d_moments) b.release();
  for (auto &e : c->moments_done)
    if (e) (void)hipEventDestroy(e);
  c->d_hard_masks.release(); c->d_hard_u.release(); c->d_all_hard.release();
  c->lane_scratch_dev.release();
  for (int k = 0; k < ngsld_ctx::kSlots; ++k) c->lane_scratch[k].release();
  c->d_labels.release(); c->d_scan_tmp.release(); c->d_scan_tmp_b.release(); c->d_label_off.release(); c->d_cum.release(); c->d_infc.release();
  for (int k = 0; k < ngsld_ctx::kSlots; ++k) {
    c->d_text[k].release(); c->d_lens[k].release(); c->d_offs[k].release(); c->d_text_meta[k].release();
    c->h_text[k].release(); c->h_text_meta[k].release();
  }
  c->d_status.release(); c->d_row_off.release(); c->d_item_off.release(); c->d_row_end.release();
  c->d_row_seed.release(); c->d_row_count.release(); c->d_keep.release(); c->d_items.release();
  for (int k = 0; k < ngsld_ctx::kSlots; ++k) {
    c->d_std[k].release(); c->d_ext[k].release(); c->h_std[k].release(); c->h_ext[k].release();
    if (c->ev_kernel_done[k]) (void)hipEventDestroy(c->ev_kernel_done[k]);
    if (c->ev_copy_done[k]) (void)hipEventDestroy(c->ev_copy_done[k]);
  }
  for (auto &ev : c->ev_pool) {
    (void)hipEventDestroy(ev.first);
    (void)hipEventDestroy(ev.second);
  }
  if (c->stream) (void)hipStreamDestroy(c->stream);
  if (c->stream2) (void)hipStreamDestroy(c->stream2);
  if (c->copy_stream) (void)hipStreamDestroy(c->copy_stream);
  if (c->text_stream) (void)hipStreamDestroy(c->text_stream);
  for (int k = 0; k < 3; ++k)
    if (c->ev_scan_done[k]) (void)hipEventDestroy(c->ev_scan_done[k]);
  if (c->replay_stream) (void)hipStreamDestroy(c->replay_stream);
  delete c;
}

const char *ngsld_last_error(const ngsld_ctx *c) { return c ? c->err.c_str() : g_create_error.c_str(); }

int ngsld_set_geno_raw(ngsld_ctx *c, const double *gl_raw, uint64_t n_sites, uint64_t n_ind, int log_scale,
                       int ignore_miss_data, int on_device) try {
  ngsld_geno_opts o{};
  o.log_scale = log_scale;
  o.ignore_miss_data = ignore_miss_data;
  o.on_device = on_device;
  return set_geno_common(c, gl_raw, nullptr, n_sites, n_ind, o, false);
} NGSLD_CATCH(c)

int ngsld_set_geno_raw_opts(ngsld_ctx *c, const double *gl_raw, uint64_t n_sites, uint64_t n_ind,
                            const ngsld_geno_opts *opts) try {
  if (opts == nullptr) return c ? fail(c, NGSLD_ERR_INVALID, "opts is NULL") : NGSLD_ERR_INVALID;
  return set_geno_common(c, gl_raw, nullptr, n_sites, n_ind, *opts, false);
} NGSLD_CATCH(c)

int ngsld_set_geno_lkl(ngsld_ctx *c, const double *geno_lkl, const double *maf, uint64_t n_sites, uint64_t n_ind,
                       int on_device) try {
  ngsld_geno_opts o{};
  o.on_device = on_device;
  return set_geno_common(c, geno_lkl, maf, n_sites, n_ind, o, true);
} NGSLD_CATCH(c)

int ngsld_get_maf(ngsld_ctx *c, double *maf_out) try {
  if (c == nullptr || maf_out == nullptr) return NGSLD_ERR_INVALID;
  if (!c->have_geno) return fail(c, NGSLD_ERR_INVALID, "no genotype data set");
  std::memcpy(maf_out, c->h_maf.data(), c->n_sites * sizeof(double));
  return NGSLD_OK;
} NGSLD_CATCH(c)

int ngsld_set_pos_dist(ngsld_ctx *c, const double *pos_dist) try {
  if (c == nullptr) return NGSLD_ERR_INVALID;
  if (!c->have_geno) return fail(c, NGSLD_ERR_INVALID, "set the genotype data before the positions");
  c->planned = false;
  c->clear_blocks();
  if (pos_dist == nullptr)
    c->h_pos_dist.assign(c->n_sites, std::numeric_limits<double>::infinity());
  else
    c->h_pos_dist.assign(pos_dist, pos_dist + c->n_sites);
  return NGSLD_OK;
} NGSLD_CATCH(c)
const char *ngsld_pair_kernel(const ngsld_ctx *c) {
  if (c == nullptr || !c->have_geno) return "";
  switch (effective_kernel(c->cfg, c->params.ignore_miss_data != 0)) {
    case kGroup: return "group";
    case kMulti: return c->cfg.form == 1 ? "multi-ab" : "multi";
    case kStream: return "stream";
    case kRun: return "run";
    case kHard: return "hard";
    case kRunAB: return "ab";
    default: return "";
  }
}

int ngsld_describe_dispatch(uint64_t n_ind, int ignore_miss_data, char *buf, size_t buf_len) {
  if (buf == nullptr || buf_len == 0) return NGSLD_ERR_INVALID;
  buf[0] = 0;
  PairConfig cfg;
  const bool masked = ignore_miss_data != 0;
  if (!pair_config(n_ind, &cfg, kChooseAuto, masked)) return NGSLD_ERR_UNSUPPORTED;
  const char *family = "";
  int slots = cfg.slots, waves = cfg.waves;
  switch (effective_kernel(cfg, masked)) {
    case kGroup: family = "group"; break;
    case kMulti:
      family = cfg.form == 1 ? "multi-ab" : "multi";
      if (cfg.form == 0) multi_shape(cfg, masked, &slots, &waves);
      break;
    case kStream: family = "stream"; break;
    case kRun: family = "run"; break;
    case kRunAB: family = "ab"; break;
    default: return NGSLD_ERR_UNSUPPORTED;
  }
  const int n = std::snprintf(buf, buf_len, "%s %dx%d lanes=%d np=%u", family, waves, slots, cfg.group, cfg.np);
  return (n < 0 || (size_t)n >= buf_len) ? NGSLD_ERR_INVALID : NGSLD_OK;
}

int ngsld_set_tuning(ngsld_ctx *c, uint32_t pairs_per_item, uint64_t batch_pairs) {
  if (c == nullptr) return NGSLD_ERR_INVALID;
  c->clear_blocks();
  if (pairs_per_item) {
    c->pairs_per_item = pairs_per_item;
    c->planned = false;
  }
  if (batch_pairs) {
    c->batch_pairs = batch_pairs;
    c->batch_pairs_set = true;
  }
  return NGSLD_OK;
}

int ngsld_selftest(ngsld_ctx *c) try {
  if (c == nullptr) return NGSLD_ERR_INVALID;
  HIP_TRY(c, hipSetDevice(c->device));
  (void)hipGetLastError();
  std::vector<double> in(320), out(71, 0.0);
  uint64_t st = 0x9E3779B97F4A7C15ull;
  for (auto &v : in) {
    st = st * 6364136223846793005ull + 1442695040888963407ull;
    v = (double)(st >> 11) / 9007199254740992.0 + 1e-3;
  }
  for (int l = 0; l < 64; ++l) in[256 + l] *= std::pow(10.0, -(l % 30));
  DevBuf<double> d_in, d_out;
  HIP_TRY(c, d_in.resize(in.size()));
  HIP_TRY(c, d_out.resize(out.size()));
  HIP_TRY(c, hipMemcpy(d_in.p, in.data(), in.size() * sizeof(double), hipMemcpyHostToDevice));
  HIP_TRY(c, launch_selftest(d_in.p, d_out.p, c->stream));
  HIP_TRY(c, hipStreamSynchronize(c->stream));
  HIP_TRY(c, hipMemcpy(out.data(), d_out.p, out.size() * sizeof(double), hipMemcpyDeviceToHost));
  d_in.release();
  d_out.release();
  for (int k = 0; k < 7; ++k) {
    const int v = k < 4 ? k : k - 4;
    const double got = k < 4 ? out[k] : out[68 + v];
    long double ref = 0;
    for (int l = 0; l < 64; ++l) ref += in[v * 64 + l];
    if (!(std::fabs((double)(got - ref)) <= 1e-14 * std::fabs((double)ref))) {
      char buf[160];
      std::snprintf(buf, sizeof(buf), "%s value %d: got %.17g expected %.17Lg", k < 4 ? "wave_sum4" : "wave_sum3", v, got, ref);
      return fail(c, NGSLD_ERR_DEVICE, buf);
    }
  }
  for (int l = 0; l < 64; ++l) {
    const double ref = 1.0 / in[256 + l];
    if (std::fabs(out[4 + l] - ref) > 4.5e-16 * ref) {
      char buf[160];
      std::snprintf(buf, sizeof(buf), "rcp_refined lane %d: got %.17g expected %.17g", l, out[4 + l], ref);
      return fail(c, NGSLD_ERR_DEVICE, buf);
    }
  }
  return NGSLD_OK;
} NGSLD_CATCH(c)

int ngsld_selftest_format(ngsld_ctx *c, uint64_t n, const ngsld_rec_std *std_rec, const ngsld_rec_ext *ext_rec, const double *dist,
                          const double *maf1, const double *maf2, char *text, uint64_t text_cap, uint64_t *row_len,
                          int32_t *needs_host) try {
  if (c == nullptr) return NGSLD_ERR_INVALID;
  if (n == 0 || n > (1ull << 24) || std_rec == nullptr || dist == nullptr || maf1 == nullptr || maf2 == nullptr ||
      text == nullptr || row_len == nullptr || needs_host == nullptr)
    return fail(c, NGSLD_ERR_INVALID, "ngsld_selftest_format: 1 <= n <= 2^24 rows and every pointer but ext set");
  HIP_TRY(c, hipSetDevice(c->device));
  (void)hipGetLastError();
  std::vector<ngsld_item> items(n);
  std::vector<double> cum(2 * n, 0.0), maf(2 * n);
  std::vector<uint32_t> infc(2 * n, 0);
  for (uint64_t i = 0; i < n; ++i) {
    items[i] = ngsld_item{(uint32_t)(2 * i), (uint32_t)(2 * i + 1), 1, 0, 1ull, i};
    if (dist[i] == std::numeric_limits<double>::infinity())
      infc[2 * i + 1] = 1;
    else
      cum[2 * i + 1] = dist[i];
    maf[2 * i] = maf1[i];
    maf[2 * i + 1] = maf2[i];
  }
  DevBuf<ngsld_item> d_items;
  DevBuf<ngsld_rec_std> d_std;
  DevBuf<ngsld_rec_ext> d_ext;
  DevBuf<double> d_cum, d_maf;
  DevBuf<uint32_t> d_infc;
  DevBuf<uint64_t> d_lens, d_offs, d_meta;
  DevBuf<int> d_host;
  DevBuf<char> d_text, d_tmp;
  const size_t tmp_bytes = text_scan_temp_bytes(n);
  HIP_TRY(c, d_items.resize(n));
  HIP_TRY(c, d_std.resize(n));
  if (ext_rec != nullptr) HIP_TRY(c, d_ext.resize(n));
  HIP_TRY(c, d_cum.resize(2 * n));
  HIP_TRY(c, d_maf.resize(2 * n));
  HIP_TRY(c, d_infc.resize(2 * n));
  HIP_TRY(c, d_lens.resize(n));
  HIP_TRY(c, d_offs.resize(n));
  HIP_TRY(c, d_meta.resize(2));
  HIP_TRY(c, d_host.resize(1));
  HIP_TRY(c, d_text.resize(text_cap ? text_cap : 1));
  HIP_TRY(c, d_tmp.resize(tmp_bytes ? tmp_bytes : 1));
  HIP_TRY(c, hipMemcpy(d_items.p, items.data(), n * sizeof(ngsld_item), hipMemcpyHostToDevice));
  HIP_TRY(c, hipMemcpy(d_std.p, std_rec, n * sizeof(ngsld_rec_std), hipMemcpyHostToDevice));
  if (ext_rec != nullptr) HIP_TRY(c, hipMemcpy(d_ext.p, ext_rec, n * sizeof(ngsld_rec_ext), hipMemcpyHostToDevice));
  HIP_TRY(c, hipMemcpy(d_cum.p, cum.data(), 2 * n * sizeof(double), hipMemcpyHostToDevice));
  HIP_TRY(c, hipMemcpy(d_maf.p, maf.data(), 2 * n * sizeof(double), hipMemcpyHostToDevice));
  HIP_TRY(c, hipMemcpy(d_infc.p, infc.data(), 2 * n * sizeof(uint32_t), hipMemcpyHostToDevice));
  HIP_TRY(c, hipMemset(d_meta.p, 0, 2 * sizeof(uint64_t)));
  HIP_TRY(c, hipMemset(d_host.p, 0, sizeof(int)));
  TextArgs t{};
  t.items = d_items.p;
  t.n_items = n;
  t.out_base = 0;
  t.n_pairs = n;
  t.std_rec = d_std.p;
  t.ext_rec = ext_rec != nullptr ? d_ext.p : nullptr;
  t.maf = d_maf.p;
  t.cum = d_cum.p;
  t.infc = d_infc.p;
  t.labels = nullptr;
  t.label_off = nullptr;
  t.lens = d_lens.p;
  t.offs = d_offs.p;
  t.text = d_text.p;
  t.text_cap = text_cap;
  t.overflow = d_meta.p + 1;
  t.needs_host = d_host.p;
  HIP_TRY(c, launch_text_lengths(t, c->stream));
  HIP_TRY(c, text_scan(d_tmp.p, tmp_bytes, d_lens.p, d_offs.p, n, d_meta.p, c->stream));
  if (text_cap > 0) HIP_TRY(c, launch_text_write(t, c->stream));
  HIP_TRY(c, hipStreamSynchronize(c->stream));
  uint64_t meta[2];
  int host = 0;
  HIP_TRY(c, hipMemcpy(meta, d_meta.p, sizeof(meta), hipMemcpyDeviceToHost));
  HIP_TRY(c, hipMemcpy(&host, d_host.p, sizeof(int), hipMemcpyDeviceToHost));
  HIP_TRY(c, hipMemcpy(row_len, d_lens.p, n * sizeof(uint64_t), hipMemcpyDeviceToHost));
  *needs_host = host;
  if (meta[0] > text_cap || meta[1] != 0)
    return fail(c, NGSLD_ERR_INVALID, "ngsld_selftest_format: the rows take " + std::to_string(meta[0]) + " bytes, text_cap is " +
                                          std::to_string(text_cap));
  HIP_TRY(c, hipMemcpy(text, d_text.p, meta[0], hipMemcpyDeviceToHost));
  return NGSLD_OK;
} NGSLD_CATCH(c)

uint64_t ngsld_slab_sites_for_budget(uint64_t n_ind, uint64_t budget_bytes) { return ngsld_sites_for_budget(n_ind, budget_bytes, 3); }

uint64_t ngsld_sites_for_budget(uint64_t n_ind, uint64_t budget_bytes, int matrix_copies) {
  PairConfig cfg, cfg_masked;
  if (!pair_config(n_ind, &cfg) || !pair_config(n_ind, &cfg_masked, kChooseAuto, true)) return 0;
  if (cfg_masked.np > cfg.np) cfg.np = cfg_masked.np;
  const uint64_t fixed = ((uint64_t)ngsld_ctx::kSlots * (1ull << 23) * (sizeof(ngsld_rec_std) + sizeof(ngsld_rec_ext))) + (768ull << 20);
  const uint64_t per_ctx = budget_bytes / 2;
  if (per_ctx <= fixed) return 0;
  const uint64_t copies = matrix_copies < 1 ? 1 : (matrix_copies > 3 ? 3 : (uint64_t)matrix_copies);
  return (per_ctx - fixed) / (24ull * copies * cfg.np + 64ull);
}

}

namespace ngsld {
namespace eng {
static std::atomic<uint64_t> g_mem_budget{0}, g_mem_base_free{0};
bool room_for(uint64_t need_bytes, uint64_t device_margin, uint64_t budget_margin) {
  size_t free_b = 0, total_b = 0;
  if (hipMemGetInfo(&free_b, &total_b) != hipSuccess) {
    (void)hipGetLastError();
    return false;
  }
  if ((uint64_t)free_b < need_bytes + device_margin) return false;
  const uint64_t budget = g_mem_budget.load();
  if (budget == 0) return true;
  const uint64_t base = g_mem_base_free.load(), used = base > (uint64_t)free_b ? base - (uint64_t)free_b : 0;
  return used + need_bytes + budget_margin <= budget;
}
}
}

extern "C" {

int ngsld_set_memory_budget(int device, uint64_t bytes) {
  uint64_t free_b = 0;
  if (ngsld_device_memory(device, &free_b, nullptr) != NGSLD_OK) return NGSLD_ERR_DEVICE;
  ngsld::eng::g_mem_base_free.store(free_b);
  ngsld::eng::g_mem_budget.store(bytes);
  return NGSLD_OK;
}

int ngsld_device_memory(int device, uint64_t *free_bytes, uint64_t *total_bytes) {
  if (hipSetDevice(device) != hipSuccess) {
    (void)hipGetLastError();
    return NGSLD_ERR_DEVICE;
  }
  size_t f = 0, t = 0;
  if (hipMemGetInfo(&f, &t) != hipSuccess) {
    (void)hipGetLastError();
    return NGSLD_ERR_DEVICE;
  }
  if (free_bytes) *free_bytes = f;
  if (total_bytes) *total_bytes = t;
  return NGSLD_OK;
}

}
```

ngsld_amd/csrc/engine_plan.hip:

```cpp
#include "engine.h"

namespace ngsld {
namespace eng {

void plan_rows(const std::vector<double> &pos_dist, const std::vector<double> &maf, const ngsld_params &p,
               uint64_t n, std::vector<uint32_t> &row_end) {
  row_end.assign(n, 0);
  const bool use_dist = p.max_kb_dist > 0;
  const double limit = (double)(p.max_kb_dist * 1000);
  bool exact = true;
  std::vector<double> cum;
  std::vector<uint32_t> seg;
  if (use_dist) {
    cum.assign(n, 0.0);
    seg.assign(n, 0);
    double run = 0.0;
    uint32_t sg = 0;
    for (uint64_t s = 0; s < n; ++s) {
      const double g = pos_dist[s];
      if (std::isinf(g) && g > 0) {
        if (s > 0) ++sg;
      } else if (s > 0) {
        if (!(g >= 1.0) || g != std::floor(g) || run + g > 9.0e15) exact = false;
        run += g;
      }
      cum[s] = run;
      seg[s] = sg;
    }
  }
  uint64_t e = 0;
  for (uint64_t s1 = 0; s1 < n; ++s1) {
    uint64_t end;
    if (maf[s1] < p.min_maf) {
      end = s1 + 1;
    } else if (!use_dist) {
      end = n;
    } else if (exact) {
      if (e < s1 + 1) e = s1 + 1;
      while (e < n && seg[e] == seg[s1] && !(limit < cum[e] - cum[s1])) ++e;
      end = e;
    } else {
      double dist = 0.0;
      end = s1 + 1;
      while (end < n) {
        dist += pos_dist[end];
        if (limit < dist) break;
        ++end;
      }
    }
    if (p.max_snp_dist > 0 && end > s1 + 1 + p.max_snp_dist) end = s1 + 1 + p.max_snp_dist;
    if (end > n) end = n;
    row_end[s1] = (uint32_t)end;
  }
}

int build_runs(ngsld_ctx *c, uint64_t run_len, const std::vector<uint64_t> &launch_ends) {
  run_len = std::max<uint64_t>(1, std::min<uint64_t>(run_len, kRunItems));
  if (c->run_len == run_len && c->run_ends == launch_ends) return NGSLD_OK;
  const uint64_t n = c->n_sites;
  uint64_t tail_len = std::max<uint64_t>(1, run_len / 8);
  uint64_t tail_pairs = (uint64_t)c->n_cus * run_len * item_span(c->cfg, c->pairs_per_item);
  if (const char *e = test_knob("TAIL_LEN")) tail_len = (uint64_t)std::max(0l, atol(e));
  if (const char *e = test_knob("TAIL_PAIRS")) tail_pairs = std::strtoull(e, nullptr, 10);
  std::vector<uint8_t> in_tail(n, 0);
  if (tail_len > 0 && tail_len < run_len) {
    uint64_t begin = 0;
    for (const uint64_t end : launch_ends) {
      if (end > n || end < begin) continue;
      for (uint64_t s1 = end; s1 > begin && c->h_row_off[end] - c->h_row_off[s1 - 1] <= tail_pairs; --s1) in_tail[s1 - 1] = 1;
      begin = end;
    }
  }
  std::vector<Run> runs;
  c->h_run_off.assign(n + 1, 0);
  for (uint64_t s1 = 0; s1 < n; ++s1) {
    const uint64_t i0 = c->h_item_off[s1], m = c->h_item_off[s1 + 1] - i0;
    const uint64_t len = in_tail[s1] ? tail_len : run_len;
    const uint64_t parts = (m + len - 1) / len;
    for (uint64_t q = 0; q < parts; ++q) {
      const uint64_t b = i0 + m * q / parts, e = i0 + m * (q + 1) / parts;
      runs.push_back(Run{(uint32_t)b, (uint32_t)(e - b)});
    }
    c->h_run_off[s1 + 1] = runs.size();
  }
  if (c->run_len != 0) HIP_TRY(c, hipDeviceSynchronize());
  HIP_TRY(c, c->d_runs.resize(runs.empty() ? 1 : runs.size()));
  if (!runs.empty())
    HIP_TRY(c, hipMemcpy(c->d_runs.p, runs.data(), runs.size() * sizeof(Run), hipMemcpyHostToDevice));
  c->run_len = run_len;
  c->run_ends = launch_ends;
  return NGSLD_OK;
}
}
}

extern "C" {

int ngsld_plan(ngsld_ctx *c, const ngsld_params *p, uint64_t *n_pairs) try {
  if (c == nullptr || p == nullptr) return NGSLD_ERR_INVALID;
  if (!c->have_geno) return fail(c, NGSLD_ERR_INVALID, "no genotype data set");
  if (c->h_pos_dist.size() != c->n_sites) {
    if (p->max_kb_dist > 0)
      return fail(c, NGSLD_ERR_INVALID, "position file necessary in order to filter by maximum distance!");
    c->h_pos_dist.assign(c->n_sites, std::numeric_limits<double>::infinity());
  }
  if (p->min_maf < 0 || p->min_maf > 1)
    return fail(c, NGSLD_ERR_INVALID, "minimum allele frequency must be in [0,1]!");
  HIP_TRY(c, hipSetDevice(c->device));
  (void)hipGetLastError();
  Range range_("ngsld:plan");
  {
    const int rcp = finish_device_run(c);
    if (rcp != NGSLD_OK) return rcp;
  }
  const uint64_t n = c->n_sites;
  c->params = *p;
  c->planned = false;
  c->clear_blocks();
  if (!(p->rnd_sample >= 0 && p->rnd_sample <= 1))
    return fail(c, NGSLD_ERR_INVALID, "proportion of comparisons to sample must be in ]0,1]!");
  const bool sampling = p->rnd_sample > 0 && p->rnd_sample < 1;
  c->replayed_sites = 0;
  if (c->replay_on && (c->replay_read != nullptr || c->replay_matrix != nullptr) && !c->normalised) {
    bool changed = false;
    std::vector<double> tmp;
    ReplaySite site;
    for (uint64_t s = 0; s < n; ++s) {
      const double m = c->h_maf[s], t = std::fabs(m) * 1e6;
      const bool tie = p->min_maf > 0 && std::fabs(m - p->min_maf) <= 1e-12;
      const bool edge = p->extend_out && std::fabs((t - std::floor(t)) - 0.5) < 1e-6;
      if (!tie && !edge) continue;
      const int rcs = fetch_replay_site(c, s, tmp, &site);
      if (rcs != NGSLD_OK) return fail(c, rcs, "the replay source callback failed");
      ++c->replayed_sites;
      if (site.maf != m && !(site.maf != site.maf && m != m)) {
        c->h_maf[s] = site.maf;
        changed = true;
      }
    }
    if (changed) {
      HIP_TRY(c, hipMemcpy(c->d_maf.p, c->h_maf.data(), n * sizeof(double), hipMemcpyHostToDevice));
      HIP_TRY(c, launch_pack_scalars(c->d_maf.p, c->d_mean.p, c->d_rsx.p, c->d_skip.p, c->d_sc4.p, n, c->stream));
      if (c->d_dose_sum.p != nullptr)
        HIP_TRY(c, launch_site_dose(c->d_planes.p, 3ull * c->np, c->np, (uint32_t)c->n_ind, c->d_maf.p, c->d_skip.p, n, c->d_dose_sum.p,
                                    c->stream));
    }
  }
  plan_rows(c->h_pos_dist, c->h_maf, *p, n, c->h_row_end);
  c->h_keep.resize(n);
  for (uint64_t s = 0; s < n; ++s) c->h_keep[s] = (c->h_maf[s] < p->min_maf) ? 0 : 1;
  const uint64_t ch = item_span(c->cfg, c->pairs_per_item);
  c->h_item_off.resize(n + 1);
  c->h_item_off[0] = 0;
  for (uint64_t s1 = 0; s1 < n; ++s1) {
    const uint64_t end = c->h_row_end[s1];
    const uint64_t span = end > s1 + 1 ? end - (s1 + 1) : 0;
    c->h_item_off[s1 + 1] = c->h_item_off[s1] + (span + ch - 1) / ch;
  }
  c->n_items = c->h_item_off[n];
  if (uses_runs(c->cfg.kernel)) {
    if (c->n_items > 0xffffffffull) return fail(c, NGSLD_ERR_UNSUPPORTED, "more than 2^32 work items in one plan");
    c->run_len = 0;
  }
  HIP_TRY(c, c->d_row_end.resize(n));
  HIP_TRY(c, c->d_keep.resize(n));
  HIP_TRY(c, c->d_row_off.resize(n + 1));
  HIP_TRY(c, c->d_item_off.resize(n + 1));
  HIP_TRY(c, c->d_row_count.resize(n));
  HIP_TRY(c, c->d_items.resize(c->n_items ? c->n_items : 1));
  HIP_TRY(c, hipMemcpyAsync(c->d_row_end.p, c->h_row_end.data(), n * sizeof(uint32_t), hipMemcpyHostToDevice, c->stream));
  HIP_TRY(c, hipMemcpyAsync(c->d_keep.p, c->h_keep.data(), n, hipMemcpyHostToDevice, c->stream));
  HIP_TRY(c, hipMemcpyAsync(c->d_item_off.p, c->h_item_off.data(), (n + 1) * sizeof(uint64_t), hipMemcpyHostToDevice, c->stream));
  std::vector<uint64_t> seeds;
  if (sampling) {
    seeds.resize(n);
    Taus master;
    master.set(p->seed);
    for (uint64_t k = 0; k < p->first_row; ++k) master.get();
    for (uint64_t s = 0; s < n; ++s) seeds[s] = master.row_seed();
    HIP_TRY(c, c->d_row_seed.resize(n));
    HIP_TRY(c, hipMemcpyAsync(c->d_row_seed.p, seeds.data(), n * sizeof(uint64_t), hipMemcpyHostToDevice, c->stream));
  }
  ItemArgs ia{};
  ia.row_end = c->d_row_end.p;
  ia.keep = c->d_keep.p;
  ia.row_seed = sampling ? c->d_row_seed.p : nullptr;
  ia.row_off = c->d_row_off.p;
  ia.item_off = c->d_item_off.p;
  ia.row_count = c->d_row_count.p;
  ia.items = c->d_items.p;
  ia.n_sites = (uint32_t)n;
  ia.span = (uint32_t)ch;
  ia.rnd_sample = p->rnd_sample;
  ia.count_only = 1;
  HIP_TRY(c, launch_items(ia, c->stream));
  std::vector<uint64_t> counts(n);
  HIP_TRY(c, hipMemcpyAsync(counts.data(), c->d_row_count.p, n * sizeof(uint64_t), hipMemcpyDeviceToHost, c->stream));
  HIP_TRY(c, hipStreamSynchronize(c->stream));
  c->h_row_off.resize(n + 1);
  c->h_row_off[0] = 0;
  for (uint64_t s1 = 0; s1 < n; ++s1) c->h_row_off[s1 + 1] = c->h_row_off[s1] + counts[s1];
  HIP_TRY(c, hipMemcpyAsync(c->d_row_off.p, c->h_row_off.data(), (n + 1) * sizeof(uint64_t), hipMemcpyHostToDevice, c->stream));
  ia.count_only = 0;
  HIP_TRY(c, launch_items(ia, c->stream));
  c->h_items.clear();
  HIP_TRY(c, hipStreamSynchronize(c->stream));
  if (uses_runs(c->cfg.kernel)) {
    const int rcr = build_runs(c, kRunItems, std::vector<uint64_t>{n});
    if (rcr != NGSLD_OK) return rcr;
  }
  c->planned = true;
  if (n_pairs) *n_pairs = c->h_row_off[n];
  return NGSLD_OK;
} NGSLD_CATCH(c)

int ngsld_plan_rows(ngsld_ctx *c, const uint64_t **row_off, const uint32_t **row_end) {
  if (c == nullptr) return NGSLD_ERR_INVALID;
  if (!c->planned) return fail(c, NGSLD_ERR_INVALID, "ngsld_plan has not been called");
  if (row_off) *row_off = c->h_row_off.data();
  if (row_end) *row_end = c->h_row_end.data();
  return NGSLD_OK;
}
int ngsld_window_ends(const double *pos_dist, uint64_t n_sites, const ngsld_params *p, uint32_t *row_end) try {
  if (p == nullptr || row_end == nullptr || n_sites == 0 || n_sites >= 0xffffffffull) return NGSLD_ERR_INVALID;
  std::vector<double> pd;
  if (pos_dist == nullptr)
    pd.assign(n_sites, std::numeric_limits<double>::infinity());
  else
    pd.assign(pos_dist, pos_dist + n_sites);
  ngsld_params q = *p;
  q.min_maf = 0.0;
  const std::vector<double> maf(n_sites, 0.5);
  std::vector<uint32_t> ends;
  plan_rows(pd, maf, q, n_sites, ends);
  std::memcpy(row_end, ends.data(), n_sites * sizeof(uint32_t));
  return NGSLD_OK;
} NGSLD_CATCH((ngsld_ctx *)nullptr)

}
```

ngsld_amd/csrc/engine_run.hip:

```cpp
#include "engine.h"
#include "../../include/ngsld_host.h"

namespace ngsld {
namespace eng {

static hipError_t launch_run_with_moments(ngsld_ctx *c, const PairArgs &a, hipStream_t stream) {
  const std::vector<uint64_t> &ro = c->h_row_off;
  const uint64_t total = ro[a.row1] - ro[a.row0];
  if (total == 0) return hipSuccess;
  uint64_t longest = 0;
  for (uint64_t r = a.row0; r < a.row1; ++r) longest = std::max(longest, ro[r + 1] - ro[r]);
  int k = 0;
  while (k < c->moments_used && c->moments_stream[k] != stream) ++k;
  if (k == c->moments_used) {
    if (k == ngsld_ctx::kMomentStreams) {
      k = ngsld_ctx::kMomentStreams - 1;
      const hipError_t e = hipEventSynchronize(c->moments_done[k]);
      if (e != hipSuccess) return e;
    } else {
      ++c->moments_used;
      const hipError_t e = hipEventCreateWithFlags(&c->moments_done[k], hipEventDisableTiming);
      if (e != hipSuccess) {
        --c->moments_used;
        return e;
      }
    }
    c->moments_stream[k] = stream;
  }
  DevBuf<double> &buf = c->d_moments[k];
  uint64_t want = total;
  if (const char *e = test_knob("MOMENTS_PAIRS")) want = std::min<uint64_t>(want, std::max<uint64_t>(1, std::strtoull(e, nullptr, 10)));
  want = std::max(want, longest);
  uint64_t cap = buf.n / 2;
  if (cap < want) {
    const uint64_t floor = std::max(std::max(longest, cap), std::min<uint64_t>(want, 1ull << 22));
    uint64_t grow = want;
    while (grow > floor && !room_for(grow * 16, 2ull << 30, 256ull << 20)) grow = std::max(floor, grow / 2);
    if (grow > cap) {
      const hipError_t e = buf.resize(2 * grow);
      if (e != hipSuccess) return e;
      cap = grow;
    }
  }
  cap = std::min(cap, want);
  const bool masked = false;
  for (uint64_t r0 = a.row0; r0 < a.row1;) {
    const uint64_t r1 = rows_within(ro, r0, a.row1, cap);
    if (ro[r1] > ro[r0]) {
      MomentArgs m{};
      m.planes = a.planes;
      m.site_stride = a.site_stride;
      m.np = a.np;
      m.n_ind = a.n_ind;
      m.maf = a.maf;
      m.n_sites = c->n_sites;
      m.items_all = a.items_all;
      m.item_off = a.item_off;
      m.row_end = c->d_row_end.p;
      m.row0 = (uint32_t)r0;
      m.row1 = (uint32_t)r1;
      m.dose = (a.dose_sum != nullptr && c->cfg.slots >= 2 && c->cfg.slots <= 8) ? 1 : 0;
      m.rec0 = ro[r0];
      m.out = buf.p;
      hipError_t e = launch_pair_moments(m, c->h_row_end.data(), stream);
      if (e != hipSuccess) return e;
      PairArgs b = a;
      b.row0 = (uint32_t)r0;
      b.row1 = (uint32_t)r1;
      b.items = c->d_items.p + c->h_item_off[r0];
      b.n_items = c->h_item_off[r1] - c->h_item_off[r0];
      b.runs = c->d_runs.p + c->h_run_off[r0];
      b.n_runs = c->h_run_off[r1] - c->h_run_off[r0];
      b.moments = reinterpret_cast<const double *>(reinterpret_cast<uintptr_t>(buf.p) - 16 * (ro[r0] - a.out_base));
      e = launch_pair_kernel(c->cfg, masked, b, stream);
      if (e != hipSuccess) return e;
    }
    r0 = r1;
  }
  return hipEventRecord(c->moments_done[k], stream);
}

hipError_t timed_launch(ngsld_ctx *c, const PairArgs &a, hipStream_t stream) {
  if (c->ev_used == c->ev_pool.size()) {
    hipEvent_t b, e;
    hipError_t r = hipEventCreate(&b);
    if (r != hipSuccess) return r;
    r = hipEventCreate(&e);
    if (r != hipSuccess) return r;
    c->ev_pool.emplace_back(b, e);
  }
  auto &ev = c->ev_pool[c->ev_used++];
  hipError_t r = hipEventRecord(ev.first, stream);
  if (r != hipSuccess) return r;
  if (c->cfg.kernel == kRun && c->params.ignore_miss_data == 0 && a.row1 > a.row0 && !test_knob_is("PAIR_MOMENTS", "0"))
    r = launch_run_with_moments(c, a, stream);
  else
    r = launch_pair_kernel(c->cfg, c->params.ignore_miss_data != 0, a, stream);
  if (r != hipSuccess) return r;
  return hipEventRecord(ev.second, stream);
}

PairArgs make_args(ngsld_ctx *c, uint64_t r0, uint64_t r1, ngsld_rec_std *d_std, ngsld_rec_ext *d_ext, uint32_t *d_flags,
                   uint32_t flag_cap, uint64_t flag_n) {
  PairArgs a{};
  a.flags = d_flags;
  a.flags_host = d_flags != nullptr ? d_flags + flag_head_words(flag_cap) + flag_bitmap_words(flag_n) : nullptr;
  a.flag_cap = flag_cap;
  a.flag_text = 1;
  a.pearson_on_device = lkl_device_eligible(c) ? 1 : 0;
  a.skip_degenerate = (d_flags != nullptr && c->h_skip_count > 0 && c->skip_on && lkl_device_eligible(c) && !c->store.failed()) ? 1 : 0;
  a.planes = c->d_planes.p;
  a.site_stride = 3ull * c->np;
  a.np = c->np;
  a.n_ind = (uint32_t)c->n_ind;
  a.inv_n = 1.0 / (double)c->n_ind;
  a.maf = c->d_maf.p;
  a.mean_e = c->d_mean.p;
  a.rsx = c->d_rsx.p;
  a.items = c->d_items.p + c->h_item_off[r0];
  a.n_items = c->h_item_off[r1] - c->h_item_off[r0];
  if (uses_runs(c->cfg.kernel)) {
    a.runs = c->d_runs.p + c->h_run_off[r0];
    a.n_runs = c->h_run_off[r1] - c->h_run_off[r0];
  }
  a.hard_masks = c->d_hard_masks.p;
  a.hard_u = c->d_hard_u.p;
  a.mask_words = c->mask_words;
  a.items_all = c->d_items.p;
  a.item_off = c->d_item_off.p;
  a.h_item_off = c->h_item_off.data();
  a.row0 = (uint32_t)r0;
  a.row1 = (uint32_t)r1;
  a.planes_bytes = c->n_sites * 3ull * c->np * sizeof(double);
  a.sc4 = c->d_sc4.p;
  a.dose_ok = c->cfg.kernel == kRun ? c->d_dose_sum.p : nullptr;
  a.dose_sum = c->first_step_on ? a.dose_ok : nullptr;
  a.out_base = c->h_row_off[r0];
  a.out_std = d_std;
  a.out_ext = d_ext;
  a.status = c->d_status.p;
  return a;
}
}
}

extern "C" {

int ngsld_set_text_output(ngsld_ctx *c, const char *const *labels, int enable) try {
  if (c == nullptr) return NGSLD_ERR_INVALID;
  if (!c->have_geno) return fail(c, NGSLD_ERR_INVALID, "set the genotype data before the labels");
  HIP_TRY(c, hipSetDevice(c->device));
  (void)hipGetLastError();
  c->text_mode = false;
  c->clear_blocks();
  if (!enable) return NGSLD_OK;
  c->have_labels = labels != nullptr;
  c->max_label = 6;
  if (labels != nullptr) {
    std::vector<uint64_t> off(c->n_sites + 1, 0);
    for (uint64_t s = 0; s < c->n_sites; ++s) {
      if (labels[s] == nullptr) return fail(c, NGSLD_ERR_INVALID, "a label is NULL");
      const uint64_t n = std::strlen(labels[s]);
      off[s + 1] = off[s] + n;
      c->max_label = std::max<uint64_t>(c->max_label, n);
    }
    std::vector<char> blob(off[c->n_sites] ? off[c->n_sites] : 1);
    for (uint64_t s = 0; s < c->n_sites; ++s) std::memcpy(blob.data() + off[s], labels[s], off[s + 1] - off[s]);
    HIP_TRY(c, c->d_labels.resize(blob.size()));
    HIP_TRY(c, c->d_label_off.resize(c->n_sites + 1));
    HIP_TRY(c, hipMemcpy(c->d_labels.p, blob.data(), blob.size(), hipMemcpyHostToDevice));
    HIP_TRY(c, hipMemcpy(c->d_label_off.p, off.data(), off.size() * sizeof(uint64_t), hipMemcpyHostToDevice));
  }
  c->text_mode = true;
  return NGSLD_OK;
} NGSLD_CATCH(c)

int ngsld_reserve_text_buffers(ngsld_ctx *c, uint64_t bytes_per_row) try {
  if (c == nullptr) return NGSLD_ERR_INVALID;
  if (c->reserve_thread.joinable()) c->reserve_thread.join();
  if (bytes_per_row == 0) return NGSLD_OK;
  const uint64_t bytes_per_batch = bytes_per_row * std::min<uint64_t>(c->batch_pairs, kTextBatchPairs);
  c->reserve_thread = std::thread([c, bytes_per_batch] {
    if (hipSetDevice(c->device) != hipSuccess) return;
    for (int k = 0; k < ngsld_ctx::kSlots; ++k) (void)c->h_text[k].resize(bytes_per_batch);
  });
  return NGSLD_OK;
} NGSLD_CATCH(c)
int ngsld_run_device(ngsld_ctx *c, uint64_t s1_begin, uint64_t s1_end, void *d_std, void *d_ext, void *hip_stream) try {
  if (c == nullptr) return NGSLD_ERR_INVALID;
  if (!c->planned) return fail(c, NGSLD_ERR_INVALID, "ngsld_plan has not been called");
  if (s1_begin > s1_end || s1_end > c->n_sites) return fail(c, NGSLD_ERR_INVALID, "row range out of bounds");
  if (d_std == nullptr) return fail(c, NGSLD_ERR_INVALID, "d_std is NULL");
  HIP_TRY(c, hipSetDevice(c->device));
  (void)hipGetLastError();
  Range range_("ngsld:run_device (pair kernels)");
  {
    const int rcp = finish_device_run(c);
    if (rcp != NGSLD_OK) return rcp;
  }
  hipStream_t st = hip_stream ? (hipStream_t)hip_stream : c->stream;
  c->ev_used = 0;
  c->timed_stream = st;
  c->timed_overlap = false;
  c->timed_pairs = c->h_row_off[s1_end] - c->h_row_off[s1_begin];
  c->replayed_pairs = 0;
  c->replayed_on_device = 0;
  c->flagged_pairs = 0;
// ... 833 lines not shown
```

ngsld_amd/csrc/exact_store.hip:

```cpp
#include "engine.h"

namespace ngsld {
namespace eng {

const double *ExactStore::planes(const ngsld_ctx *c) const { return alias_ ? c->d_planes.p : xplanes_.p; }
const double *ExactStore::maf(const ngsld_ctx *c) const { return alias_ ? c->d_maf.p : xmaf_.p; }

bool ExactStore::is_free(const ngsld_ctx *c) { return c->normalised || (c->replay_matrix == nullptr && c->replay_read == nullptr); }

bool ExactStore::wanted(const ngsld_ctx *c, uint64_t pending) const {
  if (!lkl_device_eligible(c) || failed_) return false;
  if (started() || is_free(c)) return pending > 0;
  if (c->exact_mode >= 2) return pending > 0;
  return c->host_replayed_total + pending > std::max<uint64_t>(4096, c->n_sites / 2);
}

bool ExactStore::alloc_lane_copy(ngsld_ctx *c) {
  xT_ready_ = false;
  const size_t elems = (size_t)c->n_sites * c->n_ind * 3;
  if (!room_for(elems * sizeof(double), 4ull << 30, 512ull << 20)) return false;
  std::vector<uint32_t> perm(c->n_sites);
  {
    uint32_t n_rare = 0;
    auto rare = [&](uint64_t s) {
// ... 21 lines not shown
  hipError_t e = launch_transpose_store(planes(c), 3ull * c->np, c->np, (uint32_t)c->n_ind, c->n_sites, xT_.p, xdepth_.p, xperm_.p, st);
  if (e == hipSuccess) e = hipStreamSynchronize(st);
  if (e != hipSuccess) return e;
  xT_ready_ = true;
  return hipSuccess;
}

__global__ __launch_bounds__(256) void store_chunk_kernel(const double *__restrict__ src, double *__restrict__ dst, uint64_t n,
                                                          const double *__restrict__ src_maf, double *__restrict__ dst_maf, uint64_t n_maf) {
  const uint64_t t = (uint64_t)blockIdx.x * blockDim.x + threadIdx.x, T = (uint64_t)gridDim.x * blockDim.x;
  const double2 *s2 = reinterpret_cast<const double2 *>(src);
  double2 *d2 = reinterpret_cast<double2 *>(dst);
  for (uint64_t i = t; i < n / 2; i += T) d2[i] = s2[i];
  if (t == 0 && (n & 1)) dst[n - 1] = src[n - 1];
  for (uint64_t i = t; i < n_maf; i += T) dst_maf[i] = src_maf[i];
}

struct ExactStore::Builder {
  ngsld_ctx *const c;
  ExactStore &s;
  Range range_{"ngsld:exact store (host libm -> device)"};
  const std::chrono::steady_clock::time_point t0 = std::chrono::steady_clock::now();
  const uint64_t n = c->n_sites, ni = c->n_ind, np = c->np, site_elems = 3 * np;
  uint64_t chunk = std::max<uint64_t>(1, (32ull << 20) / (site_elems * sizeof(double))), slow_us = 0;
  const int T = c->replay_threads > 0 ? c->replay_threads : (int)std::min<unsigned>(32u, usable_threads());
  hipEvent_t up[2] = {nullptr, nullptr};
  std::vector<double> raw_chunk;
  std::string msg;

  int hip(hipError_t e, const char *what) {
    if (e == hipSuccess) return NGSLD_OK;
    (void)hipGetLastError();
    return bad(NGSLD_ERR_DEVICE, (std::string(what) + ": " + hipGetErrorString(e)).c_str());
  }
  int bad(int rc, const char *text) { return msg = text, rc; }

  int setup() {
    if (const char *e = test_knob("EXACT_CHUNK_SITES")) chunk = std::max<uint64_t>(1, std::strtoull(e, nullptr, 10));
    if (const char *e = test_knob("EXACT_SLOW_US")) slow_us = std::strtoull(e, nullptr, 10);
    if (chunk > n) chunk = n;
    RC_TRY(hip(hipSetDevice(c->device), "exact store"));
    if (s.stream_ == nullptr) {
      int least = 0, greatest = 0;
      if (hipDeviceGetStreamPriorityRange(&least, &greatest) != hipSuccess) {
        (void)hipGetLastError();
        least = greatest = 0;
      }
      RC_TRY(hip(hipStreamCreateWithPriority(&s.stream_, hipStreamNonBlocking, greatest), "exact store stream"));
    }
    for (int k = 0; k < 2; ++k) {
      RC_TRY(hip(s.stage_[k].resize((size_t)chunk * (site_elems + 1)), "exact store staging"));
      RC_TRY(hip(hipEventCreateWithFlags(&up[k], hipEventDisableTiming), "exact store event"));
    }
    return NGSLD_OK;
  }

  int fetch_chunk(uint64_t s0, uint64_t m, const double **raw) {
    if (c->replay_matrix != nullptr) {
      *raw = c->replay_matrix + s0 * 3 * ni;
      return NGSLD_OK;
    }
    raw_chunk.resize((size_t)m * 3 * ni);
    std::lock_guard<std::mutex> g(c->replay_mu);
    if (c->replay_read(c->replay_user, s0, m, raw_chunk.data()) != 0) return bad(NGSLD_ERR_SINK, "the replay source callback failed");
    *raw = raw_chunk.data();
    return NGSLD_OK;
  }

  int compute_chunk(const double *raw, uint64_t m, int b) {
    double *stage = s.stage_[b].p, *stage_maf = stage + (size_t)chunk * site_elems;
    const int Tm = (int)std::min<uint64_t>((uint64_t)T, m);
    std::atomic<bool> good{true};
    s.pool_.run(Tm, [&](int t) {
      try {
        for (uint64_t k = m * (uint64_t)t / (uint64_t)Tm; k < m * (uint64_t)(t + 1) / (uint64_t)Tm; ++k)
          replay_site_planes(raw + k * 3 * ni, ni, c->gopts, np, stage + k * site_elems, &stage_maf[k]);
      } catch (...) {
        good = false;
      }
    });
    return good ? NGSLD_OK : bad(NGSLD_ERR_NOMEM, "out of host memory");
  }

  int upload_chunk(uint64_t s0, uint64_t m, int b) {
    double *stage_dev = nullptr;
    RC_TRY(hip(hipHostGetDevicePointer((void **)&stage_dev, s.stage_[b].p, 0), "exact store upload"));
    hipLaunchKernelGGL(store_chunk_kernel, dim3(512), dim3(256), 0, s.stream_, stage_dev, s.xplanes_.p + s0 * site_elems, (uint64_t)m * site_elems,
                       stage_dev + (size_t)chunk * site_elems, s.xmaf_.p + s0, (uint64_t)m);
    RC_TRY(hip(hipGetLastError(), "exact store upload"));
    if (s.xT_ready_.load())
      RC_TRY(hip(launch_transpose_store(s.xplanes_.p, site_elems, (uint32_t)np, (uint32_t)ni, n, s.xT_.p, s.xdepth_.p, s.xperm_.p, s.stream_, s0, s0 + m),
                 "exact store, individual-major copy"));
    return hip(hipEventRecord(up[b], s.stream_), "exact store upload");
  }

  int publish(int b, uint64_t end) {
    RC_TRY(hip(hipEventSynchronize(up[b]), "exact store upload"));
    s.frontier_.store(end);
    s.cv_.notify_all();
    return NGSLD_OK;
  }

  int chunks() try {
    RC_TRY(setup());
    uint64_t k = 0, prev_end = 0;
    for (uint64_t s0 = 0; s0 < n && !s.cancel_.load(); s0 += chunk, ++k) {
      const int b = (int)(k & 1);
      const uint64_t m = std::min(chunk, n - s0);
      const double *raw = nullptr;
      RC_TRY(fetch_chunk(s0, m, &raw));
      if (slow_us) std::this_thread::sleep_for(std::chrono::microseconds(slow_us));
      RC_TRY(compute_chunk(raw, m, b));
      RC_TRY(upload_chunk(s0, m, b));
      if (k >= 1) RC_TRY(publish(b ^ 1, prev_end));
      prev_end = s0 + m;
    }
    return NGSLD_OK;
  } catch (...) {
    return bad(NGSLD_ERR_NOMEM, "out of host memory");
  }

  void finish(int rc) {
    if (s.stream_ != nullptr) {
      const hipError_t e = hipStreamSynchronize(s.stream_);
      if (rc == NGSLD_OK) rc = hip(e, "exact store upload");
    }
    if (rc == NGSLD_OK && !s.cancel_.load()) {
      s.frontier_.store(n);
      s.cv_.notify_all();
    }
    for (auto &b : s.stage_) b.release();
    for (hipEvent_t e : up)
      if (e) (void)hipEventDestroy(e);
    const double secs = std::chrono::duration<double>(std::chrono::steady_clock::now() - t0).count();
    {
      std::lock_guard<std::mutex> g(s.mu_);
      s.rc_ = rc;
      s.msg_ = msg;
      s.build_s_ = secs;
      s.state_.store(rc == NGSLD_OK && !s.cancel_.load() ? 2 : -1);
    }
    s.cv_.notify_all();
    if (std::getenv("NGSLD_TRACE") != nullptr)
      std::fprintf(stderr, "[trace] exact store: %llu sites x %llu individuals through the host's libm in %.3f s (a thread of its own beside the run)\n",
                   (unsigned long long)n, (unsigned long long)ni, secs);
  }

  void run() { finish(chunks()); }
};

int ExactStore::start(ngsld_ctx *c) {
  if (state_.load() != 0 || failed_) return NGSLD_OK;
  HIP_TRY(c, hipSetDevice(c->device));
  if (is_free(c)) {
    alias_ = true;
    frontier_.store(c->n_sites);
    const hipError_t e = fill_lane_copy(c, replay_stream_of(c));
    if (e != hipSuccess) return hip_fail(c, e, "exact store, individual-major copy");
    failed_ = !xT_ready_.load() && replay_lkl_waves((uint32_t)c->n_ind) == 0;
    if (!failed_) state_.store(2);
    return NGSLD_OK;
  }
  const bool pretend = test_knob("EXACT_STORE_NO_ROOM") != nullptr;
  const bool no_room = !room_for((uint64_t)c->n_sites * (3ull * c->np + 1) * sizeof(double), 0, 256ull << 20);
  failed_ = pretend || no_room || xplanes_.resize((size_t)c->n_sites * 3 * c->np) != hipSuccess || xmaf_.resize(c->n_sites) != hipSuccess;
  if (failed_) (void)hipGetLastError();
  if (!failed_) {
    if (thread_.joinable()) thread_.join();
    alias_ = false;
    xT_ready_ = alloc_lane_copy(c);
    failed_ = !xT_ready_.load() && replay_lkl_waves((uint32_t)c->n_ind) == 0;
  }
  if (failed_) {
    xplanes_.release();
    xmaf_.release();
    return NGSLD_OK;
  }
  cancel_.store(false);
  frontier_.store(0);
  state_.store(1);
  try {
    thread_ = std::thread([this, c] { Builder{c, *this}.run(); });
  } catch (...) {
    state_.store(0);
    failed_ = true;
  }
  return NGSLD_OK;
}

int ExactStore::wait(ngsld_ctx *c, uint64_t need_sites, bool *have) {
  *have = false;
  if (failed_ || state_.load() == 0) return NGSLD_OK;
  const bool all = need_sites >= c->n_sites;
  {
    std::unique_lock<std::mutex> lk(mu_);
    while (state_.load() == 1 && (all || frontier_.load() < need_sites)) cv_.wait_for(lk, std::chrono::milliseconds(1));
    if (state_.load() == -1) {
      const int rc = rc_;
      const std::string msg = msg_;
      lk.unlock();
      stop();
      failed_ = true;
      return rc != NGSLD_OK ? fail(c, rc, msg.c_str()) : NGSLD_OK;
    }
  }
  if (state_.load() == 2 && thread_.joinable()) thread_.join();
  *have = true;
  return NGSLD_OK;
}

void ExactStore::wait_idle() {
  std::unique_lock<std::mutex> lk(mu_);
  while (state_.load() == 1) cv_.wait_for(lk, std::chrono::milliseconds(1));
}

void ExactStore::stop() {
  if (thread_.joinable()) {
    cancel_.store(true);
    thread_.join();
  }
  cancel_.store(false);
  state_.store(0);
  frontier_.store(0);
  rc_ = NGSLD_OK;
  msg_.clear();
  release_buffers();
}

void ExactStore::destroy() {
  stop();
  if (stream_) (void)hipStreamDestroy(stream_);
  stream_ = nullptr;
  for (auto &b : stage_) b.release();
}

}
}
```

ngsld_amd/csrc/ld_common.h:

```cpp
#pragma once

#include <hip/hip_runtime.h>
#include <stdint.h>

#include "../../include/ngsld.h"

namespace ngsld {

#ifndef NGSLD_PRIO_S
#define NGSLD_PRIO_S 0
#define NGSLD_PRIO_TREE 3
#define NGSLD_PRIO_R 1
#define NGSLD_PRIO_SERIAL 3
#endif
#ifndef NGSLD_SETPRIO
#define NGSLD_SETPRIO 1
#endif
#ifndef NGSLD_MASK_SLOTS
#define NGSLD_MASK_SLOTS 6
#endif
constexpr int kIterMax = 100;
constexpr double kEpsilon = 1e-5;

constexpr double kHapNoise = 0x1p-49;
// ... 30 lines not shown
  const Item *items;
  uint64_t n_items;
  const struct Run *runs;
  uint64_t n_runs;
  const Item *items_all;
  const double *sc4;
  uint64_t out_base;
  ngsld_rec_std *out_std;
  ngsld_rec_ext *out_ext;
  int *status;
  const uint64_t *hard_masks;
  const double *hard_u;
  uint32_t mask_words;
  uint32_t *flags;
  uint32_t *flags_host;
  uint32_t flag_cap;
  uint32_t flag_text;
  uint32_t pearson_on_device;
  uint32_t skip_degenerate;
  const uint64_t *item_off;
  const uint64_t *h_item_off;
  uint32_t row0, row1, tile_rows, tile_nk;
  uint64_t planes_bytes;
  const double *dose_sum;
  const double *dose_ok;
  const double *moments;
};

typedef unsigned u32x2 __attribute__((ext_vector_type(2)));

__device__ __forceinline__ double mk_double(unsigned lo, unsigned hi) { return __hiloint2double((int)hi, (int)lo); }

__device__ __forceinline__ double ref_nan(double v) { return v != v ? mk_double(0u, 0xfff80000u) : v; }

__device__ __forceinline__ double uniform(double v) {
  return mk_double((unsigned)__builtin_amdgcn_readfirstlane(__double2loint(v)),
                   (unsigned)__builtin_amdgcn_readfirstlane(__double2hiint(v)));
}

__device__ __forceinline__ double read_lane(double v, int lane) {
  return mk_double((unsigned)__builtin_amdgcn_readlane(__double2loint(v), lane),
                   (unsigned)__builtin_amdgcn_readlane(__double2hiint(v), lane));
}

__device__ __forceinline__ double fold32(double x, double y) {
  u32x2 l = __builtin_amdgcn_permlane32_swap((unsigned)__double2loint(x), (unsigned)__double2loint(y), false, false);
  u32x2 h = __builtin_amdgcn_permlane32_swap((unsigned)__double2hiint(x), (unsigned)__double2hiint(y), false, false);
  return mk_double(l[0], h[0]) + mk_double(l[1], h[1]);
}

__device__ __forceinline__ double fold16(double x, double y) {
  u32x2 l = __builtin_amdgcn_permlane16_swap((unsigned)__double2loint(x), (unsigned)__double2loint(y), false, false);
  u32x2 h = __builtin_amdgcn_permlane16_swap((unsigned)__double2hiint(x), (unsigned)__double2hiint(y), false, false);
  return mk_double(l[0], h[0]) + mk_double(l[1], h[1]);
}

template <int CTRL>
__device__ __forceinline__ double dpp_mov(double v) {
  int lo = __double2loint(v), hi = __double2hiint(v);
  lo = __builtin_amdgcn_update_dpp(0, lo, CTRL, 0xf, 0xf, true);
  hi = __builtin_amdgcn_update_dpp(0, hi, CTRL, 0xf, 0xf, true);
  return __hiloint2double(hi, lo);
}

__device__ __forceinline__ void wave_sum4(double &t0, double &t1, double &t2, double &t3) {
  double z01 = fold32(t0, t1);
  double z23 = fold32(t2, t3);
  double w = fold16(z01, z23);
  w += dpp_mov<0x128>(w);
  w += dpp_mov<0x124>(w);
  w += dpp_mov<0x4E>(w);
  w += dpp_mov<0xB1>(w);
  t0 = read_lane(w, 0);
  t2 = read_lane(w, 16);
  t1 = read_lane(w, 32);
  t3 = read_lane(w, 48);
}

template <int CTRL, int ROW_MASK>
__device__ __forceinline__ double dpp_mov_rows(double v) {
  int lo = __double2loint(v), hi = __double2hiint(v);
  lo = __builtin_amdgcn_update_dpp(0, lo, CTRL, ROW_MASK, 0xf, false);
  hi = __builtin_amdgcn_update_dpp(0, hi, CTRL, ROW_MASK, 0xf, false);
  return __hiloint2double(hi, lo);
}

__device__ __forceinline__ double wave_sum3_rows(double t1, double t2, double t3) {
  double z12 = fold32(t1, t2);
  double w = fold16(z12, t3);
  w += dpp_mov<0x128>(w);
  w += dpp_mov<0x124>(w);
  w += dpp_mov<0x4E>(w);
  w += dpp_mov<0xB1>(w);
  w += dpp_mov_rows<0x143, 0x8>(w);
  return w;
}
__device__ __forceinline__ void wave_sum3(double &t1, double &t2, double &t3) {
  double z12 = fold32(t1, t2);
  double w = fold16(z12, t3);
  w += dpp_mov<0x128>(w);
  w += dpp_mov<0x124>(w);
  w += dpp_mov<0x4E>(w);
  w += dpp_mov<0xB1>(w);
  t1 = read_lane(w, 0);
  t2 = read_lane(w, 32);
  int ulo, uhi;
  asm("; undefined" : "=v"(ulo), "=v"(uhi));
  const int lo = __builtin_amdgcn_update_dpp(ulo, __double2loint(w), 0x143, 0x8, 0xf, false);
  const int hi = __builtin_amdgcn_update_dpp(uhi, __double2hiint(w), 0x143, 0x8, 0xf, false);
  t3 = read_lane(w + __hiloint2double(hi, lo), 48);
}

__device__ __forceinline__ double wave_sum1_bcast(double v) {
  v += dpp_mov<0xB1>(v);
  v += dpp_mov<0x4E>(v);
  v += dpp_mov<0x124>(v);
  v += dpp_mov<0x128>(v);
  v += dpp_mov_rows<0x142, 0xa>(v);
  v += dpp_mov_rows<0x143, 0xc>(v);
  return read_lane(v, 63);
}

__device__ __forceinline__ double wave_sum1(double v) {
  double a = v, b = 0.0, c = 0.0, d = 0.0;
  wave_sum4(a, b, c, d);
  return a;
}

__device__ __forceinline__ double rcp_refined(double s) {
  const double r0 = __builtin_amdgcn_rcp(s);
  const double e = fma(-s, r0, 1.0);
  const double t = fma(e, e, e);
  return fma(r0, t, r0);
}

struct DoseWeights {
  double u0, u1, u2, u2x2;
};
__device__ __forceinline__ DoseWeights dose_weights(double m) {
  const double q = 1.0 - m;
  DoseWeights u;
  u.u0 = q * q;
  u.u1 = 2.0 * (m * q);
  u.u2 = m * m;
  u.u2x2 = 2.0 * u.u2;
  return u;
}
__device__ __forceinline__ void dose_terms(const DoseWeights &u, double a0, double a1, double a2, double &den, double &num) {
  const double t = u.u1 * a1;
  den = fma(u.u2, a2, fma(u.u0, a0, t));
  num = fma(u.u2x2, a2, t);
}

__device__ __forceinline__ void lds_barrier() {
  asm volatile("s_waitcnt lgkmcnt(0)" ::: "memory");
  __builtin_amdgcn_s_barrier();
  asm volatile("" ::: "memory");
}

typedef double dbl2 __attribute__((ext_vector_type(2)));
__device__ __forceinline__ uint32_t lds_addr(const void *p) {
  return (uint32_t)(uintptr_t)(__attribute__((address_space(3))) const char *)p;
}
__device__ __forceinline__ void lds_post(uint32_t addr, double v) {
  asm volatile("ds_write_b64 %0, %1" ::"v"(addr), "v"(v) : "memory");
}
__device__ __forceinline__ void lds_post2(uint32_t addr, double a, double b) {
  dbl2 v = {a, b};
  asm volatile("ds_write_b128 %0, %1" ::"v"(addr), "v"(v) : "memory");
}
template <int N>
__device__ __forceinline__ void lds_gather(uint32_t addr, dbl2 (&q)[N]) {
  static_assert(N == 2 || N == 3 || N == 4 || N == 6 || N == 8 || N == 12, "lds_gather: unsupported count");
  if constexpr (N == 2)
    asm volatile("ds_read_b128 %0, %2\n\tds_read_b128 %1, %2 offset:16\n\ts_waitcnt lgkmcnt(0)"
                 : "=&v"(q[0]), "=&v"(q[1]) : "v"(addr) : "memory");
  else if constexpr (N == 3)
    asm volatile("ds_read_b128 %0, %3\n\tds_read_b128 %1, %3 offset:16\n\tds_read_b128 %2, %3 offset:32\n\ts_waitcnt lgkmcnt(0)"
                 : "=&v"(q[0]), "=&v"(q[1]), "=&v"(q[2]) : "v"(addr) : "memory");
  else if constexpr (N == 4)
    asm volatile("ds_read_b128 %0, %4\n\tds_read_b128 %1, %4 offset:16\n\tds_read_b128 %2, %4 offset:32\n\t"
                 "ds_read_b128 %3, %4 offset:48\n\ts_waitcnt lgkmcnt(0)"
                 : "=&v"(q[0]), "=&v"(q[1]), "=&v"(q[2]), "=&v"(q[3]) : "v"(addr) : "memory");
  else if constexpr (N == 6)
    asm volatile("ds_read_b128 %0, %6\n\tds_read_b128 %1, %6 offset:16\n\tds_read_b128 %2, %6 offset:32\n\t"
                 "ds_read_b128 %3, %6 offset:48\n\tds_read_b128 %4, %6 offset:64\n\tds_read_b128 %5, %6 offset:80\n\t"
                 "s_waitcnt lgkmcnt(0)"
                 : "=&v"(q[0]), "=&v"(q[1]), "=&v"(q[2]), "=&v"(q[3]), "=&v"(q[4]), "=&v"(q[5]) : "v"(addr) : "memory");
  else if constexpr (N == 8)
    asm volatile("ds_read_b128 %0, %8\n\tds_read_b128 %1, %8 offset:16\n\tds_read_b128 %2, %8 offset:32\n\t"
                 "ds_read_b128 %3, %8 offset:48\n\tds_read_b128 %4, %8 offset:64\n\tds_read_b128 %5, %8 offset:80\n\t"
                 "ds_read_b128 %6, %8 offset:96\n\tds_read_b128 %7, %8 offset:112\n\ts_waitcnt lgkmcnt(0)"
                 : "=&v"(q[0]), "=&v"(q[1]), "=&v"(q[2]), "=&v"(q[3]), "=&v"(q[4]), "=&v"(q[5]), "=&v"(q[6]), "=&v"(q[7])
                 : "v"(addr) : "memory");
  else
    asm volatile("ds_read_b128 %0, %12\n\tds_read_b128 %1, %12 offset:16\n\tds_read_b128 %2, %12 offset:32\n\t"
                 "ds_read_b128 %3, %12 offset:48\n\tds_read_b128 %4, %12 offset:64\n\tds_read_b128 %5, %12 offset:80\n\t"
                 "ds_read_b128 %6, %12 offset:96\n\tds_read_b128 %7, %12 offset:112\n\tds_read_b128 %8, %12 offset:128\n\t"
                 "ds_read_b128 %9, %12 offset:144\n\tds_read_b128 %10, %12 offset:160\n\tds_read_b128 %11, %12 offset:176\n\t"
                 "s_waitcnt lgkmcnt(0)"
                 : "=&v"(q[0]), "=&v"(q[1]), "=&v"(q[2]), "=&v"(q[3]), "=&v"(q[4]), "=&v"(q[5]), "=&v"(q[6]), "=&v"(q[7]),
                   "=&v"(q[8]), "=&v"(q[9]), "=&v"(q[10]), "=&v"(q[11])
                 : "v"(addr) : "memory");
}

__device__ __forceinline__ bool miss_data(double g0, double g1, double g2) {
  double d01 = g0 - g1, d12 = g1 - g2;
  d01 = d01 >= 0 ? d01 : -d01;
  d12 = d12 >= 0 ? d12 : -d12;
  return d01 < kEpsilon && d12 < kEpsilon;
}

}
```

ngsld_amd/csrc/ld_dispatch.h:

```cpp
#pragma once

#include "ld_common.h"

namespace ngsld {

constexpr int kBresMinSlots = 11, kBresMaxSlots = 20;
constexpr int kBresTailSlots = 20;

enum PairKernel { kGroup = 0, kMulti = 2, kStream = 4, kRun = 5, kHard = 6, kRunAB = 7 };
enum PairChoice { kChooseAuto = 0, kChooseMulti = 1, kChooseAB = 2, kChoosePlainStream = 3, kChooseABMulti = 4, kChooseResidentStream = 5 };
inline bool uses_runs(int kernel) { return kernel == kRun || kernel == kGroup || kernel == kHard || kernel == kRunAB; }
constexpr uint32_t kHardMaxWords = 512;
constexpr uint64_t kHardMaxInd = 64ull * kHardMaxWords;
struct PairConfig {
  int kernel;
  int group;
  int slots;
  int waves;
  int form;
  uint32_t np;
};
bool pair_config(uint64_t n_ind, PairConfig *cfg, int choice = kChooseAuto, bool masked = false);
inline int effective_kernel(const PairConfig &cfg, bool ) { return cfg.kernel; }
inline void multi_shape(const PairConfig &cfg, bool masked, int *slots, int *waves) {
  *slots = cfg.slots;
  *waves = cfg.waves;
  if (masked && cfg.waves == 2 && cfg.slots == 10) {
    *slots = 5;
    *waves = 4;
  }
}
hipError_t launch_pair_kernel(const PairConfig &cfg, bool masked, const PairArgs &args, hipStream_t stream);
hipError_t launch_pair_hard(bool masked, const PairArgs &args, hipStream_t stream);
hipError_t launch_pair_ab(int slots, bool masked, const PairArgs &args, hipStream_t stream);
hipError_t launch_pair_abm(int slots, int waves, bool masked, const PairArgs &args, hipStream_t stream);
hipError_t launch_pair_bres(int slots, bool masked, const PairArgs &args, hipStream_t stream);
hipError_t launch_classify_hard(const double *planes, uint64_t site_stride, uint32_t np, uint32_t n_ind, uint64_t n_sites,
                                uint64_t *masks, double *u, int *all_hard, hipStream_t stream);
struct MomentArgs {
  const double *planes;
  uint64_t site_stride;
  uint32_t np, n_ind;
  const double *maf;
  uint64_t n_sites;
  const Item *items_all;
  const uint64_t *item_off;
  const uint32_t *row_end;
  uint32_t row0, row1;
  uint32_t dose;
  uint64_t rec0;
  double *out;
};
hipError_t launch_pair_moments(const MomentArgs &args, const uint32_t *h_row_end, hipStream_t stream);
inline uint32_t item_span(const PairConfig &cfg, uint32_t pairs_per_item) {
  if (uses_runs(cfg.kernel)) return 64u;
  const uint32_t span = cfg.kernel == kMulti ? 4u * pairs_per_item : pairs_per_item;
  return span > 64u ? 64u : span;
}

}
```

ngsld_amd/csrc/ld_pair_moments.hip:

```cpp
#include <algorithm>

#include "ld_dispatch.h"

namespace ngsld {

namespace {
constexpr uint32_t kTR = 128, kTC = 64, kKc = 16;
constexpr uint32_t kSites = kTR + kTC;
constexpr uint32_t kLd = kSites + 16;
typedef double v4d __attribute__((ext_vector_type(4)));
typedef double v2d __attribute__((ext_vector_type(2)));
}

template <bool DOSE>
__global__ __launch_bounds__(512) void pair_ld_moments_kernel(MomentArgs A) {
  __shared__ double sE[kKc * kLd];
  __shared__ double sD[DOSE ? kKc * kLd : 1];
  __shared__ uint64_t s_ioff[kTR];
  __shared__ uint32_t s_end[kTR];
  __shared__ uint32_t s_cmax;
  const uint32_t t = threadIdx.x, lane = t & 63u;
  const uint32_t wave = (uint32_t)__builtin_amdgcn_readfirstlane((int)(t >> 6));
  const uint32_t rb = A.row0 + blockIdx.y * kTR;
  const uint64_t c0 = (uint64_t)rb + 1u + (uint64_t)blockIdx.x * kTC;
  if (t == 0) s_cmax = 0;
  __syncthreads();
  if (t < kTR) {
    const uint32_t row = rb + t;
    const bool in = row < A.row1;
    const uint32_t e = in ? A.row_end[row] : 0u;
    s_end[t] = e;
    s_ioff[t] = in ? A.item_off[row] : 0ull;
    atomicMax(&s_cmax, e);
  }
  __syncthreads();
  const uint32_t cmax = s_cmax;
  if (c0 >= cmax) return;

  const bool loader = t < 2 * kSites;
  const uint32_t sl = t < kSites ? t : (loader ? t - kSites : 0u), half = t < kSites ? 0u : 1u;
  uint64_t site = sl < kTR ? (uint64_t)rb + sl : c0 + (sl - kTR);
  if (site >= A.n_sites) site = A.n_sites - 1;
  const double m = A.maf[site];
  const bool flip = m > 0.5;
  const DoseWeights u = dose_weights(flip ? 1.0 - m : m);
  const double *pl = A.planes + site * A.site_stride + half * 8u;
  const double *p0 = pl + (flip ? 2u * A.np : 0u), *p1 = pl + A.np, *p2 = pl + (flip ? 0u : 2u * A.np);
  v2d q0[4], q1[4], q2[4];
  auto fetch = [&](uint32_t kc) {
#pragma unroll
    for (int i = 0; i < 4; ++i) {
      q0[i] = reinterpret_cast<const v2d *>(p0 + kc * kKc)[i];
      q1[i] = reinterpret_cast<const v2d *>(p1 + kc * kKc)[i];
      q2[i] = reinterpret_cast<const v2d *>(p2 + kc * kKc)[i];
    }
  };
  auto stage = [&](uint32_t kc) {
#pragma unroll
    for (int i = 0; i < 8; ++i) {
      const double a0 = q0[i >> 1][i & 1], a1 = q1[i >> 1][i & 1], a2 = q2[i >> 1][i & 1];
      const uint32_t k = half * 8u + (uint32_t)i;
      sE[k * kLd + sl] = fma(2.0, a2, a1);
      if (DOSE) {
        double den, num;
        dose_terms(u, a0, a1, a2, den, num);
        sD[k * kLd + sl] = kc * kKc + k < A.n_ind ? num / den : 0.0;
      }
    }
  };

  const uint32_t wr = wave & 3u, wc = wave >> 2;
  bool live[2][2];
#pragma unroll
  for (int ri = 0; ri < 2; ++ri)
#pragma unroll
    for (int cj = 0; cj < 2; ++cj) {
      const uint64_t r_lo = (uint64_t)rb + wr * 32u + ri * 16u, c_lo = c0 + wc * 32u + cj * 16u;
      live[ri][cj] = r_lo < A.row1 && c_lo + 15u > r_lo && c_lo < cmax;
    }
  v4d totE[2][2], totD[2][2];
#pragma unroll
  for (int ri = 0; ri < 2; ++ri)
#pragma unroll
    for (int cj = 0; cj < 2; ++cj) totE[ri][cj] = totD[ri][cj] = v4d{0.0, 0.0, 0.0, 0.0};
  const uint32_t oa = (lane >> 4) * kLd + wr * 32u + (lane & 15u);
  const uint32_t ob = (lane >> 4) * kLd + kTR + wc * 32u + (lane & 15u);

  const uint32_t nk = A.np / kKc;
  if (loader) fetch(0);
  for (uint32_t kc = 0; kc < nk; ++kc) {
    lds_barrier();
    if (loader) {
      stage(kc);
      if (kc + 1 < nk) fetch(kc + 1);
    }
    lds_barrier();
    v4d inE[2][2], inD[2][2];
#pragma unroll
    for (int ks = 0; ks < 4; ++ks) {
      double ae[2], be[2], ad[2], bd[2];
#pragma unroll
      for (int x = 0; x < 2; ++x) {
        ae[x] = sE[ks * 4 * kLd + oa + x * 16];
        be[x] = sE[ks * 4 * kLd + ob + x * 16];
        if (DOSE) {
          ad[x] = sD[ks * 4 * kLd + oa + x * 16];
          bd[x] = sD[ks * 4 * kLd + ob + x * 16];
        }
      }
#pragma unroll
      for (int ri = 0; ri < 2; ++ri)
#pragma unroll
        for (int cj = 0; cj < 2; ++cj) {
          if (!live[ri][cj]) continue;
          const v4d z = {0.0, 0.0, 0.0, 0.0};
          inE[ri][cj] = __builtin_amdgcn_mfma_f64_16x16x4f64(ae[ri], be[cj], ks == 0 ? z : inE[ri][cj], 0, 0, 0);
          if (DOSE) inD[ri][cj] = __builtin_amdgcn_mfma_f64_16x16x4f64(ad[ri], bd[cj], ks == 0 ? z : inD[ri][cj], 0, 0, 0);
        }
    }
#pragma unroll
    for (int ri = 0; ri < 2; ++ri)
#pragma unroll
      for (int cj = 0; cj < 2; ++cj) {
        if (!live[ri][cj]) continue;
        totE[ri][cj] += inE[ri][cj];
        if (DOSE) totD[ri][cj] += inD[ri][cj];
      }
  }

#pragma unroll
  for (int ri = 0; ri < 2; ++ri)
#pragma unroll
    for (int cj = 0; cj < 2; ++cj) {
      if (!live[ri][cj]) continue;
#pragma unroll
      for (int r = 0; r < 4; ++r) {
        const uint32_t lr = wr * 32u + ri * 16u + (lane >> 4) + 4u * r;
        const uint64_t s1 = (uint64_t)rb + lr, s2 = c0 + wc * 32u + cj * 16u + (lane & 15u);
        if (s1 >= A.row1 || s2 <= s1 || s2 >= s_end[lr]) continue;
        const uint64_t off = s2 - s1 - 1;
        const Item *it = A.items_all + s_ioff[lr] + (off >> 6);
        const uint64_t mask = it->mask, bit = 1ull << (off & 63u);
        if (!(mask & bit)) continue;
        const uint64_t idx = it->first_record + (uint64_t)__popcll(mask & (bit - 1)) - A.rec0;
        reinterpret_cast<v2d *>(A.out)[idx] = v2d{totE[ri][cj][r], DOSE ? totD[ri][cj][r] : 0.0};
      }
    }
}

hipError_t launch_pair_moments(const MomentArgs &a, const uint32_t *h_row_end, hipStream_t stream) {
  if (a.row1 <= a.row0) return hipSuccess;
  uint64_t most = 0;
  for (uint32_t rb = a.row0; rb < a.row1; rb += kTR) {
    uint32_t end = 0;
    for (uint32_t r = rb; r < a.row1 && r < rb + kTR; ++r) end = std::max(end, h_row_end[r]);
    if (end > rb + 1) most = std::max<uint64_t>(most, ((uint64_t)end - rb - 1 + kTC - 1) / kTC);
  }
  if (most == 0) return hipSuccess;
  if (most > (1ull << 22)) return hipErrorInvalidValue;
  const uint64_t blocks_y = std::min<uint64_t>(65535, std::max<uint64_t>(1, (1ull << 22) / most));
  for (uint64_t r0 = a.row0; r0 < a.row1; r0 += blocks_y * kTR) {
    MomentArgs b = a;
    b.row0 = (uint32_t)r0;
    const uint64_t by = std::min<uint64_t>(blocks_y, ((uint64_t)a.row1 - r0 + kTR - 1) / kTR);
    const dim3 grid((unsigned)most, (unsigned)by), block(512);
    if (a.dose)
      hipLaunchKernelGGL((pair_ld_moments_kernel<true>), grid, block, 0, stream, b);
    else
      hipLaunchKernelGGL((pair_ld_moments_kernel<false>), grid, block, 0, stream, b);
    const hipError_t e = hipGetLastError();
    if (e != hipSuccess) return e;
  }
  return hipSuccess;
}

}
```

ngsld_amd/csrc/ld_prep.h:

```cpp
#pragma once

#include "ld_common.h"

namespace ngsld {

struct PrepArgs {
  const double *raw;
  uint64_t site0;
  const double *maf_in;
  double *planes;
  uint64_t site_stride;
  uint64_t n_sites;
  uint32_t np, n_ind;
  int log_scale, ignore_miss, normalised_input;
  int text_semantics, call_geno;
  int exact_chain;
  double N_thresh, call_thresh;
  double *maf, *mean_e, *rsx;
  int *status;
  int *odd_missing;
  double missing_canon;
};

hipError_t launch_prep(const PrepArgs &a, hipStream_t stream);
struct ItemArgs {
  const uint32_t *row_end;
  const uint8_t *keep;
  const uint64_t *row_seed;
  const uint64_t *row_off;
  const uint64_t *item_off;
  uint64_t *row_count;
  Item *items;
  uint32_t n_sites, span;
  double rnd_sample;
  int count_only;
};
hipError_t launch_items(const ItemArgs &a, hipStream_t stream);
hipError_t launch_pack_scalars(const double *maf, const double *mean_e, const double *rsx, const uint8_t *skip, double *sc4, uint64_t n,
                               hipStream_t stream);
hipError_t launch_site_skip(const double *planes, uint64_t site_stride, uint32_t np, uint32_t n_ind, int ignore_miss, const double *maf,
                            uint64_t n_sites, uint8_t *skip, uint32_t *count, hipStream_t stream);
hipError_t launch_site_dose(const double *planes, uint64_t site_stride, uint32_t np, uint32_t n_ind, const double *maf, const uint8_t *skip,
                            uint64_t n_sites, double *dose_sum, hipStream_t stream);
hipError_t launch_selftest(const double *in, double *out, hipStream_t stream);

}
```

ngsld_amd/csrc/ld_prep.hip:

```cpp
#include "ld_prep.h"
#include "taus.h"

namespace ngsld {

__device__ __forceinline__ double logsum3(double g0, double g1, double g2) {
  double M = g0;
  M = g1 >= M ? g1 : M;
  M = g2 >= M ? g2 : M;
  if (M == -__builtin_inf()) return -__builtin_inf();
  double sum = 0.0;
  sum += exp(g0 - M);
  sum += exp(g1 - M);
  sum += exp(g2 - M);
  return log(sum) + M;
}

__device__ __forceinline__ double conv_log(double g) {
  g = log(g);
  return g == -__builtin_inf() ? -1e15 : g;
}

__device__ __forceinline__ void call_geno(double &g0, double &g1, double &g2, double N_thresh, double call_thresh) {
  int max_pos = 0;
  double mx = -__builtin_inf();
// ... 257 lines not shown
      if (mn[0] == mx[0] && raw_differs && !A.normalised_input) rsx = -__builtin_inf();
      A.rsx[A.site0 + site] = rsx;
    }
    if (nan_seen) atomicExch(A.status, (int)NGSLD_ERR_NAN);
  }
}

__global__ __launch_bounds__(256) void missing_check_kernel(const double *__restrict__ raw, uint64_t n_triples, double canon, int *odd) {
  const uint64_t T = (uint64_t)gridDim.x * blockDim.x;
  const unsigned long long cb = (unsigned long long)__double_as_longlong(canon);
  bool bad = false;
  for (uint64_t t = (uint64_t)blockIdx.x * blockDim.x + threadIdx.x; t < n_triples; t += T) {
    const double g0 = raw[3 * t], g1 = raw[3 * t + 1], g2 = raw[3 * t + 2];
    const double mn = fmin(g0, fmin(g1, g2)), mx = fmax(g0, fmax(g1, g2));
    if (mx - mn < 1e-9) {
      const bool canonical = (unsigned long long)__double_as_longlong(g0) == cb && (unsigned long long)__double_as_longlong(g1) == cb &&
                             (unsigned long long)__double_as_longlong(g2) == cb;
      bad |= !canonical;
    }
  }
  if (bad) *odd = 1;
}

hipError_t launch_prep(const PrepArgs &a, hipStream_t stream) {
  if (a.n_sites == 0) return hipSuccess;
  if (a.odd_missing != nullptr) {
    const uint64_t n_triples = a.n_sites * (uint64_t)a.n_ind;
    const uint64_t wgs = (n_triples + 255) / 256;
    hipLaunchKernelGGL(missing_check_kernel, dim3((unsigned)(wgs < 4096 ? wgs : 4096)), dim3(256), 0, stream, a.raw, n_triples, a.missing_canon,
                       a.odd_missing);
    const hipError_t e = hipGetLastError();
    if (e != hipSuccess) return e;
  }
  if (a.np <= 2048) {
    const uint64_t wgs = (a.n_sites + 3) / 4;
    const unsigned grid = (unsigned)(wgs < 65536 ? wgs : 65536);
    if (a.np <= 512)
      hipLaunchKernelGGL(prep_sites_wave_kernel<8>, dim3(grid), dim3(256), 0, stream, a);
    else if (a.np <= 1024)
      hipLaunchKernelGGL(prep_sites_wave_kernel<16>, dim3(grid), dim3(256), 0, stream, a);
    else
      hipLaunchKernelGGL(prep_sites_wave_kernel<32>, dim3(grid), dim3(256), 0, stream, a);
    return hipGetLastError();
  }
  const unsigned grid = (unsigned)(a.n_sites < 65536 ? a.n_sites : 65536);
  hipLaunchKernelGGL(prep_sites_kernel, dim3(grid), dim3(256), 0, stream, a);
  return hipGetLastError();
}

constexpr double kSkipBelow = 3e-6;
template <int MAXJ>
__global__ __launch_bounds__(256) void site_skip_kernel(const double *__restrict__ planes, uint64_t site_stride, uint32_t np, uint32_t n_ind,
                                                        int ignore_miss, const double *__restrict__ maf, uint64_t n_sites,
                                                        uint8_t *__restrict__ skip, uint32_t *count) {
  const int lane = threadIdx.x & 63, wave = threadIdx.x >> 6;
  for (uint64_t site = (uint64_t)blockIdx.x * 4 + wave; site < n_sites; site += (uint64_t)gridDim.x * 4) {
    const double *pl = planes + site * site_stride;
    const double m_in = maf[site];
    const bool flip = m_in > 0.5;
    double m = flip ? 1.0 - m_in : m_in;
    const double *p0 = pl + (flip ? 2ull * np : 0ull), *p1 = pl + np, *p2 = pl + (flip ? 0ull : 2ull * np);
    constexpr int kRegs = MAXJ > 0 ? MAXJ : 1;
    double a0[kRegs], a1[kRegs], a2[kRegs];
    uint32_t valid = 0, x = 0;
    const uint32_t n_slots = (n_ind + 63) / 64;
    auto is_valid = [&](uint32_t i, double g0, double g1, double g2) {
      return i < n_ind && !(ignore_miss && miss_data(g0, g1, g2));
    };
    if (MAXJ > 0) {
#pragma unroll
      for (int j = 0; j < kRegs; ++j) {
        const uint32_t i = (uint32_t)lane + 64u * (uint32_t)j;
        const bool in = i < n_ind;
        a0[j] = in ? p0[i] : 0.0;
        a1[j] = in ? p1[i] : 0.0;
        a2[j] = in ? p2[i] : 0.0;
        if (is_valid(i, a0[j], a1[j], a2[j])) valid |= 1u << j;
      }
      x = 0;
#pragma unroll
      for (int j = 0; j < kRegs; ++j) x += (uint32_t)__popcll(__ballot((valid >> j) & 1u));
    }
    bool mark = false;
    for (int iter = 0; iter < kIterMax; ++iter) {
      const double w0 = (1 - m) * (1 - m), w1 = 2 * m * (1 - m), w2 = m * m;
      double acc = 0.0;
      uint32_t cnt = 0;
      auto one = [&](double g0, double g1, double g2) {
        const double s = fma(w2, g2, fma(w1, g1, w0 * g0));
        acc = fma(fma(2.0 * w2, g2, w1 * g1), rcp_refined(s), acc);
      };
      if (MAXJ > 0) {
#pragma unroll
        for (int j = 0; j < kRegs; ++j)
          if ((valid >> j) & 1u) one(a0[j], a1[j], a2[j]);
        cnt = x;
      } else {
        for (uint32_t j = 0; j < n_slots; ++j) {
          const uint32_t i = (uint32_t)lane + 64u * j;
          const double g0 = i < n_ind ? p0[i] : 0.0, g1 = i < n_ind ? p1[i] : 0.0, g2 = i < n_ind ? p2[i] : 0.0;
          const bool ok = is_valid(i, g0, g1, g2);
          if (ok) one(g0, g1, g2);
          cnt += (uint32_t)__popcll(__ballot(ok));
        }
      }
      const double mn = wave_sum1(acc) / (2.0 * (double)cnt);
      const bool stop = !(fabs(mn - m) >= kEpsilon);
      m = mn;
      if (stop) {
        mark = m < kSkipBelow;
        break;
      }
    }
    if (lane == 0) {
      skip[site] = mark ? 1 : 0;
      if (mark) atomicAdd(count, 1u);
    }
  }
}

hipError_t launch_site_skip(const double *planes, uint64_t site_stride, uint32_t np, uint32_t n_ind, int ignore_miss, const double *maf,
                            uint64_t n_sites, uint8_t *skip, uint32_t *count, hipStream_t stream) {
  if (n_sites == 0) return hipSuccess;
  const uint64_t wgs = (n_sites + 3) / 4;
  const dim3 grid((unsigned)(wgs < 65536 ? wgs : 65536)), block(256);
  if (np <= 512)
    hipLaunchKernelGGL(site_skip_kernel<8>, grid, block, 0, stream, planes, site_stride, np, n_ind, ignore_miss, maf, n_sites, skip, count);
  else if (np <= 1024)
    hipLaunchKernelGGL(site_skip_kernel<16>, grid, block, 0, stream, planes, site_stride, np, n_ind, ignore_miss, maf, n_sites, skip, count);
  else
    hipLaunchKernelGGL(site_skip_kernel<0>, grid, block, 0, stream, planes, site_stride, np, n_ind, ignore_miss, maf, n_sites, skip, count);
  return hipGetLastError();
}

__global__ void pack_scalars_kernel(const double *maf, const double *mean_e, const double *rsx, const uint8_t *skip, double *sc4, uint64_t n) {
  const uint64_t s = (uint64_t)blockIdx.x * blockDim.x + threadIdx.x;
  if (s >= n) return;
  sc4[4 * s] = maf[s];
  sc4[4 * s + 1] = mean_e[s];
  sc4[4 * s + 2] = rsx[s];
  sc4[4 * s + 3] = (skip != nullptr && skip[s]) ? 1.0 : 0.0;
}

hipError_t launch_pack_scalars(const double *maf, const double *mean_e, const double *rsx, const uint8_t *skip, double *sc4, uint64_t n,
                               hipStream_t stream) {
  if (n == 0) return hipSuccess;
  hipLaunchKernelGGL(pack_scalars_kernel, dim3((unsigned)((n + 255) / 256)), dim3(256), 0, stream, maf, mean_e, rsx, skip, sc4, n);
  return hipGetLastError();
}

constexpr double kDoseDenMin = 0x1p-500;
__global__ __launch_bounds__(256) void site_dose_kernel(const double *__restrict__ planes, uint64_t site_stride, uint32_t np, uint32_t n_ind,
                                                        const double *__restrict__ maf, const uint8_t *__restrict__ skip, uint64_t n_sites,
                                                        double *__restrict__ dose_sum) {
  const int lane = threadIdx.x & 63, wave = threadIdx.x >> 6;
  for (uint64_t site = (uint64_t)blockIdx.x * 4 + wave; site < n_sites; site += (uint64_t)gridDim.x * 4) {
    const double *pl = planes + site * site_stride;
    const double m_in = maf[site];
    const bool flip = m_in > 0.5;
    const double m = flip ? 1.0 - m_in : m_in;
    const DoseWeights u = dose_weights(m);
    const double *p0 = pl + (flip ? 2ull * np : 0ull), *p1 = pl + np, *p2 = pl + (flip ? 0ull : 2ull * np);
    bool ok = m_in > 0.0 && m_in < 1.0;
    const bool marked = skip != nullptr && skip[site];
    double acc = 0.0, prod = 1.0;
    for (uint32_t i = (uint32_t)lane; i < n_ind; i += 64) {
      const double a0 = p0[i], a1 = p1[i], a2 = p2[i];
      double den, num;
      dose_terms(u, a0, a1, a2, den, num);
      const double d = num / den;
      ok = ok && den >= kDoseDenMin && den < __builtin_inf() && d >= 0.0 && d < __builtin_inf() && !odd_triple(a0, a1, a2);
      acc += d;
      prod *= den;
    }
    ok = ok && prod >= kDoseDenMin * kDoseDenMin;
    const double S = wave_sum1(acc);
    const bool all_ok = __ballot(!ok) == 0 && S >= 0.0 && S < __builtin_inf();
    if (lane == 0) dose_sum[site] = all_ok ? (marked ? -2.0 : S) : -1.0;
  }
}

hipError_t launch_site_dose(const double *planes, uint64_t site_stride, uint32_t np, uint32_t n_ind, const double *maf, const uint8_t *skip,
                            uint64_t n_sites, double *dose_sum, hipStream_t stream) {
  if (n_sites == 0) return hipSuccess;
  const uint64_t wgs = (n_sites + 3) / 4;
  hipLaunchKernelGGL(site_dose_kernel, dim3((unsigned)(wgs < 65536 ? wgs : 65536)), dim3(256), 0, stream, planes, site_stride, np, n_ind, maf,
                     skip, n_sites, dose_sum);
  return hipGetLastError();
}

__global__ void items_kernel(ItemArgs A) {
  const uint32_t s1 = blockIdx.x * blockDim.x + threadIdx.x;
  if (s1 >= A.n_sites) return;
  const uint32_t end = A.row_end[s1];
  const bool sampling = A.row_seed != nullptr;
  Taus rng;
  if (sampling) rng.set(A.row_seed[s1]);
  uint64_t kept = 0;
  uint64_t k = A.count_only ? 0 : A.item_off[s1];
  const uint64_t base = A.count_only ? 0 : A.row_off[s1];
  for (uint32_t b = s1 + 1; b < end; b += A.span) {
    const uint32_t cnt = end - b < A.span ? end - b : A.span;
    uint64_t mask = 0;
    for (uint32_t c = 0; c < cnt; ++c) {
      if (!A.keep[b + c]) continue;
      if (sampling && rng.uniform() > A.rnd_sample) continue;
      mask |= 1ull << c;
    }
    if (!A.count_only) {
      Item it;
      it.s1 = s1;
      it.s2_begin = b;
      it.count = cnt;
      it.reserved = 0;
      it.mask = mask;
      it.first_record = base + kept;
      A.items[k++] = it;
    }
    kept += (uint64_t)__popcll(mask);
  }
  if (A.count_only) A.row_count[s1] = kept;
}

hipError_t launch_items(const ItemArgs &a, hipStream_t stream) {
  if (a.n_sites == 0) return hipSuccess;
  hipLaunchKernelGGL(items_kernel, dim3((a.n_sites + 255) / 256), dim3(256), 0, stream, a);
  return hipGetLastError();
}

__global__ void selftest_kernel(const double *in, double *out) {
  const int lane = threadIdx.x;
  double t0 = in[lane], t1 = in[64 + lane], t2 = in[128 + lane], t3 = in[192 + lane];
  wave_sum4(t0, t1, t2, t3);
  if (lane == 0) {
    out[0] = t0;
    out[1] = t1;
    out[2] = t2;
    out[3] = t3;
  }
  out[4 + lane] = rcp_refined(in[256 + lane]);
  double u1 = in[lane], u2 = in[64 + lane], u3 = in[128 + lane];
  wave_sum3(u1, u2, u3);
  if (lane == 0) {
    out[68] = u1;
    out[69] = u2;
    out[70] = u3;
  }
}

hipError_t launch_selftest(const double *in, double *out, hipStream_t stream) {
  hipLaunchKernelGGL(selftest_kernel, dim3(1), dim3(64), 0, stream, in, out);
  return hipGetLastError();
}

}
```

Baseline: 221.6 million.

## Precompute per-site moment vectors once and stream them into pair-moment kernel

The site-dose kernel now also writes per-individual expected-genotype and dosage values into a chunked, site-major device buffer, laid out to match the 16-wide k-chunks of the pair-moment kernel. A new VEC variant of the moment kernel loads these precomputed vectors directly with all threads and double-buffers them in shared memory, replacing per-tile recomputation from the three genotype planes and one of the two barriers per chunk. The buffer is allocated only when device memory allows and is released when the exact store needs room, trading extra device memory and a prep pass for less arithmetic and traffic in the hot pair kernel.

Measured after the change: 223.7 million (median of 6 runs). No clear change (+0.9%).

```diff
diff --git a/include/ngsld.h b/include/ngsld.h
--- a/include/ngsld.h
+++ b/include/ngsld.h
@@ -125,6 +125,7 @@
 int ngsld_last_kernel_time(ngsld_ctx *ctx, double *total_ms, uint64_t *n_launches, uint64_t *n_pairs);
 
 const char *ngsld_pair_kernel(const ngsld_ctx *ctx);
+uint64_t ngsld_moment_vector_bytes(const ngsld_ctx *ctx);
 int ngsld_describe_dispatch(uint64_t n_ind, int ignore_miss_data, char *buf, size_t buf_len);
 
 int ngsld_set_tuning(ngsld_ctx *ctx, uint32_t pairs_per_item, uint64_t batch_pairs);
diff --git a/ngsld_amd/capi.py b/ngsld_amd/capi.py
--- a/ngsld_amd/capi.py
+++ b/ngsld_amd/capi.py
@@ -77,7 +77,7 @@
     "ngsld_set_replay_source", "ngsld_set_replay_matrix", "ngsld_set_replay", "ngsld_replay_stats", "ngsld_finish_device",
     "ngsld_set_exact_store", "ngsld_replay_info",
     "ngsld_plan_parts", "ngsld_run_multi", "ngsld_multi_last_distribution", "ngsld_rccl_selftest",
-    "ngsld_last_kernel_time", "ngsld_pair_kernel", "ngsld_describe_dispatch", "ngsld_set_tuning", "ngsld_selftest", "ngsld_selftest_format",
+    "ngsld_last_kernel_time", "ngsld_pair_kernel", "ngsld_moment_vector_bytes", "ngsld_describe_dispatch", "ngsld_set_tuning", "ngsld_selftest", "ngsld_selftest_format",
     "ngsld_selftest_printed", "ngsld_reserve_text_buffers",
     "ngsld_window_ends", "ngsld_plan_slabs", "ngsld_slab_sites_for_budget", "ngsld_sites_for_budget", "ngsld_streamed_replay_info", "ngsld_set_memory_budget", "ngsld_device_memory", "ngsld_run_streamed", "ngsld_run_streamed_text",
     "ngsld_host_read_geno_bin_range",
@@ -271,6 +271,9 @@
         if hasattr(L, "ngsld_pair_kernel"):
             L.ngsld_pair_kernel.argtypes = [vp]
             L.ngsld_pair_kernel.restype = C.c_char_p
+        if hasattr(L, "ngsld_moment_vector_bytes"):
+            L.ngsld_moment_vector_bytes.argtypes = [vp]
+            L.ngsld_moment_vector_bytes.restype = u64
         L.ngsld_selftest.argtypes = [vp]
         if hasattr(L, "ngsld_selftest_format"):
             L.ngsld_selftest_format.argtypes = [vp, u64, vp, vp, vp, vp, vp, C.c_char_p, u64, vp, C.POINTER(C.c_int32)]
@@ -1008,6 +1011,9 @@
     def pair_kernel(self) -> str:
         return self._L.ngsld_pair_kernel(self._h).decode()
 
+    def moment_vector_bytes(self) -> int:
+        return int(self._L.ngsld_moment_vector_bytes(self._h))
+
     def last_kernel_time(self) -> tuple[float, int, int]:
         ms, nl, npairs = C.c_double(), C.c_uint64(), C.c_uint64()
         self._check(self._L.ngsld_last_kernel_time(self._h, C.byref(ms), C.byref(nl), C.byref(npairs)))
diff --git a/ngsld_amd/csrc/engine.h b/ngsld_amd/csrc/engine.h
--- a/ngsld_amd/csrc/engine.h
+++ b/ngsld_amd/csrc/engine.h
@@ -236,6 +236,7 @@
   bool have_geno = false;
   DevBuf<double> d_planes, d_maf, d_mean, d_rsx, d_sc4;
   DevBuf<double> d_dose_sum;
+  DevBuf<double> d_moment_vec;
   bool first_step_on = true;
   static constexpr int kMomentStreams = 4;
   DevBuf<double> d_moments[kMomentStreams];
@@ -542,6 +543,8 @@
 int flagged_records(ngsld_ctx *c, const uint32_t *h_head, const uint32_t *d_flags, uint32_t cap, uint64_t n,
                     std::vector<uint64_t> &recs, bool dev_applied = false);
 bool room_for(uint64_t need_bytes, uint64_t device_margin, uint64_t budget_margin);
+bool hold_moment_vectors(ngsld_ctx *c);
+void yield_moment_vectors(ngsld_ctx *c);
 bool lkl_device_eligible(const ngsld_ctx *c);
 bool lkl_device_ready(const ngsld_ctx *c);
 int reserve_device_run(ngsld_ctx *c, uint64_t n_records);
diff --git a/ngsld_amd/csrc/engine.hip b/ngsld_amd/csrc/engine.hip
--- a/ngsld_amd/csrc/engine.hip
+++ b/ngsld_amd/csrc/engine.hip
@@ -159,10 +159,11 @@
     c->first_step_on = !test_knob_is("FIRST_STEP", "0");
     HIP_TRY(c, c->d_dose_sum.resize(n_sites));
     HIP_TRY(c, launch_site_dose(c->d_planes.p, 3ull * c->np, c->np, (uint32_t)n_ind, c->d_maf.p, c->d_skip.p, n_sites, c->d_dose_sum.p,
-                                c->stream));
+                                nullptr, c->stream));
   } else {
     c->d_dose_sum.release();
   }
+  c->d_moment_vec.release();
   int &all_hard = c->h_all_hard;
   all_hard = 0;
   const char *hk = test_knob("HARD_KERNEL");
@@ -200,6 +201,11 @@
   } else {
     c->d_hard_masks.release();
     c->d_hard_u.release();
+    if (c->d_dose_sum.p != nullptr && hold_moment_vectors(c)) {
+      HIP_TRY(c, launch_site_dose(c->d_planes.p, 3ull * c->np, c->np, (uint32_t)n_ind, c->d_maf.p, c->d_skip.p, n_sites, c->d_dose_sum.p,
+                                  c->d_moment_vec.p, c->stream));
+      HIP_TRY(c, hipStreamSynchronize(c->stream));
+    }
   }
   c->have_geno = true;
   return NGSLD_OK;
@@ -209,7 +215,7 @@
 
 extern "C" {
 
-const char *ngsld_version(void) { return "ngsld-amd 0.13.0 (gfx950; reference ngsLD 1.2.1)"; }
+const char *ngsld_version(void) { return "ngsld-amd 0.14.0 (gfx950; reference ngsLD 1.2.1)"; }
 
 int ngsld_create(int device, ngsld_ctx **out) {
   if (out == nullptr) return NGSLD_ERR_INVALID;
@@ -280,7 +286,7 @@
   c->store.destroy();
   (void)hipSetDevice(c->device);
   (void)hipDeviceSynchronize();
-  c->d_planes.release(); c->d_maf.release(); c->d_mean.release(); c->d_rsx.release(); c->d_sc4.release(); c->d_dose_sum.release(); c->d_runs.release(); c->d_skip.release(); c->d_skip_count.release();
+  c->d_planes.release(); c->d_maf.release(); c->d_mean.release(); c->d_rsx.release(); c->d_sc4.release(); c->d_dose_sum.release(); c->d_moment_vec.release(); c->d_runs.release(); c->d_skip.release(); c->d_skip_count.release();
   for (auto &b : c->d_moments) b.release();
   for (auto &e : c->moments_done)
     if (e) (void)hipEventDestroy(e);
@@ -355,6 +361,10 @@
     c->h_pos_dist.assign(pos_dist, pos_dist + c->n_sites);
   return NGSLD_OK;
 } NGSLD_CATCH(c)
+uint64_t ngsld_moment_vector_bytes(const ngsld_ctx *c) {
+  return c != nullptr && c->have_geno && c->d_moment_vec.p != nullptr ? moment_vec_doubles(c->n_sites, c->np) * sizeof(double) : 0;
+}
+
 const char *ngsld_pair_kernel(const ngsld_ctx *c) {
   if (c == nullptr || !c->have_geno) return "";
   switch (effective_kernel(c->cfg, c->params.ignore_miss_data != 0)) {
@@ -550,6 +560,26 @@
 namespace ngsld {
 namespace eng {
 static std::atomic<uint64_t> g_mem_budget{0}, g_mem_base_free{0};
+
+static uint64_t exact_store_bytes(const ngsld_ctx *c) {
+  return c->n_sites * (3ull * c->np + 1) * sizeof(double) + c->n_sites * c->n_ind * 3ull * sizeof(double);
+}
+bool hold_moment_vectors(ngsld_ctx *c) {
+  c->d_moment_vec.release();
+  if (test_knob_is("MOMENT_VECTORS", "0")) return false;
+  const uint64_t n = moment_vec_doubles(c->n_sites, c->np);
+  if (!room_for(n * sizeof(double) + exact_store_bytes(c), 4ull << 30, 512ull << 20)) return false;
+  if (c->d_moment_vec.resize(n) != hipSuccess) {
+    (void)hipGetLastError();
+    return false;
+  }
+  return true;
+}
+void yield_moment_vectors(ngsld_ctx *c) {
+  if (c->d_moment_vec.p == nullptr || room_for(exact_store_bytes(c), 4ull << 30, 512ull << 20)) return;
+  (void)hipDeviceSynchronize();
+  c->d_moment_vec.release();
+}
 bool room_for(uint64_t need_bytes, uint64_t device_margin, uint64_t budget_margin) {
   size_t free_b = 0, total_b = 0;
   if (hipMemGetInfo(&free_b, &total_b) != hipSuccess) {
diff --git a/ngsld_amd/csrc/engine_plan.hip b/ngsld_amd/csrc/engine_plan.hip
--- a/ngsld_amd/csrc/engine_plan.hip
+++ b/ngsld_amd/csrc/engine_plan.hip
@@ -143,7 +143,7 @@
       HIP_TRY(c, launch_pack_scalars(c->d_maf.p, c->d_mean.p, c->d_rsx.p, c->d_skip.p, c->d_sc4.p, n, c->stream));
       if (c->d_dose_sum.p != nullptr)
         HIP_TRY(c, launch_site_dose(c->d_planes.p, 3ull * c->np, c->np, (uint32_t)c->n_ind, c->d_maf.p, c->d_skip.p, n, c->d_dose_sum.p,
-                                    c->stream));
+                                    c->d_moment_vec.p, c->stream));
     }
   }
   plan_rows(c->h_pos_dist, c->h_maf, *p, n, c->h_row_end);
diff --git a/ngsld_amd/csrc/engine_run.hip b/ngsld_amd/csrc/engine_run.hip
--- a/ngsld_amd/csrc/engine_run.hip
+++ b/ngsld_amd/csrc/engine_run.hip
@@ -53,6 +53,7 @@
       m.np = a.np;
       m.n_ind = a.n_ind;
       m.maf = a.maf;
+      m.vec = c->d_moment_vec.p;
       m.n_sites = c->n_sites;
       m.items_all = a.items_all;
       m.item_off = a.item_off;
diff --git a/ngsld_amd/csrc/exact_store.hip b/ngsld_amd/csrc/exact_store.hip
--- a/ngsld_amd/csrc/exact_store.hip
+++ b/ngsld_amd/csrc/exact_store.hip
@@ -197,6 +197,7 @@
 int ExactStore::start(ngsld_ctx *c) {
   if (state_.load() != 0 || failed_) return NGSLD_OK;
   HIP_TRY(c, hipSetDevice(c->device));
+  yield_moment_vectors(c);
   if (is_free(c)) {
     alias_ = true;
     frontier_.store(c->n_sites);
diff --git a/ngsld_amd/csrc/ld_common.h b/ngsld_amd/csrc/ld_common.h
--- a/ngsld_amd/csrc/ld_common.h
+++ b/ngsld_amd/csrc/ld_common.h
@@ -206,6 +206,12 @@
   num = fma(u.u2x2, a2, t);
 }
 
+constexpr uint32_t kMomentVecChunk = 16;
+__host__ __device__ inline uint64_t moment_vec_doubles(uint64_t n_sites, uint32_t np) { return 2ull * n_sites * np; }
+__host__ __device__ inline uint64_t moment_vec_index(uint64_t n_sites, uint64_t site, uint32_t i) {
+  return ((uint64_t)(i / kMomentVecChunk) * n_sites + site) * (2 * kMomentVecChunk) + i % kMomentVecChunk;
+}
+
 __device__ __forceinline__ void lds_barrier() {
   asm volatile("s_waitcnt lgkmcnt(0)" ::: "memory");
   __builtin_amdgcn_s_barrier();
diff --git a/ngsld_amd/csrc/ld_dispatch.h b/ngsld_amd/csrc/ld_dispatch.h
--- a/ngsld_amd/csrc/ld_dispatch.h
+++ b/ngsld_amd/csrc/ld_dispatch.h
@@ -42,6 +42,7 @@
   uint64_t site_stride;
   uint32_t np, n_ind;
   const double *maf;
+  const double *vec;
   uint64_t n_sites;
   const Item *items_all;
   const uint64_t *item_off;
diff --git a/ngsld_amd/csrc/ld_pair_moments.hip b/ngsld_amd/csrc/ld_pair_moments.hip
--- a/ngsld_amd/csrc/ld_pair_moments.hip
+++ b/ngsld_amd/csrc/ld_pair_moments.hip
@@ -8,14 +8,19 @@
 constexpr uint32_t kTR = 128, kTC = 64, kKc = 16;
 constexpr uint32_t kSites = kTR + kTC;
 constexpr uint32_t kLd = kSites + 16;
+constexpr uint32_t kLs = kKc + 2;
+static_assert(kKc == kMomentVecChunk, "a chunk of the pass is a chunk of the vectors");
 typedef double v4d __attribute__((ext_vector_type(4)));
 typedef double v2d __attribute__((ext_vector_type(2)));
 }
 
-template <bool DOSE>
+template <bool DOSE, bool VEC>
 __global__ __launch_bounds__(512) void pair_ld_moments_kernel(MomentArgs A) {
-  __shared__ double sE[kKc * kLd];
-  __shared__ double sD[DOSE ? kKc * kLd : 1];
+  static_assert(DOSE || !VEC, "the vectors are there where the dosages are");
+  constexpr uint32_t kK = VEC ? 1u : kLd, kS = VEC ? kLs : 1u, kN = VEC ? kSites * kLs : kKc * kLd;
+  constexpr uint32_t kBuf = DOSE ? 2 * kN + (VEC ? 16 : 0) : kN;
+  __shared__ __attribute__((aligned(16))) double sV[VEC ? 2 * kBuf : kBuf];
+  double *const sE = sV, *const sD = sV + (DOSE ? kN + (VEC ? 16 : 0) : 0);
   __shared__ uint64_t s_ioff[kTR];
   __shared__ uint32_t s_end[kTR];
   __shared__ uint32_t s_cmax;
@@ -47,7 +52,26 @@
   const double *pl = A.planes + site * A.site_stride + half * 8u;
   const double *p0 = pl + (flip ? 2u * A.np : 0u), *p1 = pl + A.np, *p2 = pl + (flip ? 0u : 2u * A.np);
   v2d q0[4], q1[4], q2[4];
+  constexpr int kParts = (int)(kSites * 2 * kKc / (2 * 512));
+  const uint32_t w = t & 15u;
+  const double *vp[kParts];
+  v2d qv[kParts];
+  if (VEC) {
+#pragma unroll
+    for (int j = 0; j < kParts; ++j) {
+      const uint32_t sj = (uint32_t)j * 32u + (t >> 4);
+      uint64_t sv = sj < kTR ? (uint64_t)rb + sj : c0 + (sj - kTR);
+      if (sv >= A.n_sites) sv = A.n_sites - 1;
+      vp[j] = A.vec + sv * (2 * kKc) + w * 2u;
+    }
+  }
+  const uint64_t vec_chunk = A.n_sites * (2 * kKc);
   auto fetch = [&](uint32_t kc) {
+    if (VEC) {
+#pragma unroll
+      for (int j = 0; j < kParts; ++j) qv[j] = *reinterpret_cast<const v2d *>(vp[j] + kc * vec_chunk);
+      return;
+    }
 #pragma unroll
     for (int i = 0; i < 4; ++i) {
       q0[i] = reinterpret_cast<const v2d *>(p0 + kc * kKc)[i];
@@ -56,6 +80,12 @@
     }
   };
   auto stage = [&](uint32_t kc) {
+    if (VEC) {
+      double *const to = (w < 8u ? sE : sD) + (kc & 1u) * kBuf + (t >> 4) * kLs + (w & 7u) * 2u;
+#pragma unroll
+      for (int j = 0; j < kParts; ++j) *reinterpret_cast<v2d *>(to + j * 32 * kLs) = qv[j];
+      return;
+    }
 #pragma unroll
     for (int i = 0; i < 8; ++i) {
       const double a0 = q0[i >> 1][i & 1], a1 = q1[i >> 1][i & 1], a2 = q2[i >> 1][i & 1];
@@ -83,29 +113,41 @@
   for (int ri = 0; ri < 2; ++ri)
 #pragma unroll
     for (int cj = 0; cj < 2; ++cj) totE[ri][cj] = totD[ri][cj] = v4d{0.0, 0.0, 0.0, 0.0};
-  const uint32_t oa = (lane >> 4) * kLd + wr * 32u + (lane & 15u);
-  const uint32_t ob = (lane >> 4) * kLd + kTR + wc * 32u + (lane & 15u);
+  const uint32_t oa = (lane >> 4) * kK + (wr * 32u + (lane & 15u)) * kS;
+  const uint32_t ob = (lane >> 4) * kK + (kTR + wc * 32u + (lane & 15u)) * kS;
 
   const uint32_t nk = A.np / kKc;
-  if (loader) fetch(0);
+  if (VEC) {
+    fetch(0);
+    stage(0);
+    if (nk > 1) fetch(1);
+  } else if (loader) {
+    fetch(0);
+  }
   for (uint32_t kc = 0; kc < nk; ++kc) {
     lds_barrier();
-    if (loader) {
-      stage(kc);
-      if (kc + 1 < nk) fetch(kc + 1);
-    }
-    lds_barrier();
+    if (VEC) {
+      if (kc + 1 < nk) stage(kc + 1);
+      if (kc + 2 < nk) fetch(kc + 2);
+    } else {
+      if (loader) {
+        stage(kc);
+        if (kc + 1 < nk) fetch(kc + 1);
+      }
+      lds_barrier();
+    }
+    const double *const cE = sE + (VEC ? (kc & 1u) * kBuf : 0u), *const cD = sD + (VEC ? (kc & 1u) * kBuf : 0u);
     v4d inE[2][2], inD[2][2];
 #pragma unroll
     for (int ks = 0; ks < 4; ++ks) {
       double ae[2], be[2], ad[2], bd[2];
 #pragma unroll
       for (int x = 0; x < 2; ++x) {
-        ae[x] = sE[ks * 4 * kLd + oa + x * 16];
-        be[x] = sE[ks * 4 * kLd + ob + x * 16];
+        ae[x] = cE[ks * 4 * kK + oa + x * 16 * kS];
+        be[x] = cE[ks * 4 * kK + ob + x * 16 * kS];
         if (DOSE) {
-          ad[x] = sD[ks * 4 * kLd + oa + x * 16];
-          bd[x] = sD[ks * 4 * kLd + ob + x * 16];
+          ad[x] = cD[ks * 4 * kK + oa + x * 16 * kS];
+          bd[x] = cD[ks * 4 * kK + ob + x * 16 * kS];
         }
       }
 #pragma unroll
@@ -164,10 +206,12 @@
     b.row0 = (uint32_t)r0;
     const uint64_t by = std::min<uint64_t>(blocks_y, ((uint64_t)a.row1 - r0 + kTR - 1) / kTR);
     const dim3 grid((unsigned)most, (unsigned)by), block(512);
-    if (a.dose)
-      hipLaunchKernelGGL((pair_ld_moments_kernel<true>), grid, block, 0, stream, b);
+    if (a.dose && a.vec != nullptr)
+      hipLaunchKernelGGL((pair_ld_moments_kernel<true, true>), grid, block, 0, stream, b);
+    else if (a.dose)
+      hipLaunchKernelGGL((pair_ld_moments_kernel<true, false>), grid, block, 0, stream, b);
     else
-      hipLaunchKernelGGL((pair_ld_moments_kernel<false>), grid, block, 0, stream, b);
+      hipLaunchKernelGGL((pair_ld_moments_kernel<false, false>), grid, block, 0, stream, b);
     const hipError_t e = hipGetLastError();
     if (e != hipSuccess) return e;
   }
diff --git a/ngsld_amd/csrc/ld_prep.h b/ngsld_amd/csrc/ld_prep.h
--- a/ngsld_amd/csrc/ld_prep.h
+++ b/ngsld_amd/csrc/ld_prep.h
@@ -41,7 +41,7 @@
 hipError_t launch_site_skip(const double *planes, uint64_t site_stride, uint32_t np, uint32_t n_ind, int ignore_miss, const double *maf,
                             uint64_t n_sites, uint8_t *skip, uint32_t *count, hipStream_t stream);
 hipError_t launch_site_dose(const double *planes, uint64_t site_stride, uint32_t np, uint32_t n_ind, const double *maf, const uint8_t *skip,
-                            uint64_t n_sites, double *dose_sum, hipStream_t stream);
+                            uint64_t n_sites, double *dose_sum, double *vec, hipStream_t stream);
 hipError_t launch_selftest(const double *in, double *out, hipStream_t stream);
 
 }
diff --git a/ngsld_amd/csrc/ld_prep.hip b/ngsld_amd/csrc/ld_prep.hip
--- a/ngsld_amd/csrc/ld_prep.hip
+++ b/ngsld_amd/csrc/ld_prep.hip
@@ -433,7 +433,7 @@
 constexpr double kDoseDenMin = 0x1p-500;
 __global__ __launch_bounds__(256) void site_dose_kernel(const double *__restrict__ planes, uint64_t site_stride, uint32_t np, uint32_t n_ind,
                                                         const double *__restrict__ maf, const uint8_t *__restrict__ skip, uint64_t n_sites,
-                                                        double *__restrict__ dose_sum) {
+                                                        double *__restrict__ dose_sum, double *__restrict__ vec) {
   const int lane = threadIdx.x & 63, wave = threadIdx.x >> 6;
   for (uint64_t site = (uint64_t)blockIdx.x * 4 + wave; site < n_sites; site += (uint64_t)gridDim.x * 4) {
     const double *pl = planes + site * site_stride;
@@ -453,7 +453,18 @@
       ok = ok && den >= kDoseDenMin && den < __builtin_inf() && d >= 0.0 && d < __builtin_inf() && !odd_triple(a0, a1, a2);
       acc += d;
       prod *= den;
-    }
+      if (vec != nullptr) {
+        const uint64_t at = moment_vec_index(n_sites, site, i);
+        vec[at] = fma(2.0, a2, a1);
+        vec[at + kMomentVecChunk] = d;
+      }
+    }
+    if (vec != nullptr)
+      for (uint32_t i = n_ind + (uint32_t)lane; i < np; i += 64) {
+        const uint64_t at = moment_vec_index(n_sites, site, i);
+        vec[at] = fma(2.0, p2[i], p1[i]);
+        vec[at + kMomentVecChunk] = 0.0;
+      }
     ok = ok && prod >= kDoseDenMin * kDoseDenMin;
     const double S = wave_sum1(acc);
     const bool all_ok = __ballot(!ok) == 0 && S >= 0.0 && S < __builtin_inf();
@@ -462,11 +473,11 @@
 }
 
 hipError_t launch_site_dose(const double *planes, uint64_t site_stride, uint32_t np, uint32_t n_ind, const double *maf, const uint8_t *skip,
-                            uint64_t n_sites, double *dose_sum, hipStream_t stream) {
+                            uint64_t n_sites, double *dose_sum, double *vec, hipStream_t stream) {
   if (n_sites == 0) return hipSuccess;
   const uint64_t wgs = (n_sites + 3) / 4;
   hipLaunchKernelGGL(site_dose_kernel, dim3((unsigned)(wgs < 65536 ? wgs : 65536)), dim3(256), 0, stream, planes, site_stride, np, n_ind, maf,
-                     skip, n_sites, dose_sum);
+                     skip, n_sites, dose_sum, vec);
   return hipGetLastError();
 }
 
```
